# amdreallyfast/GpuRadixSort

Measured on AMD Instinct MI355X. Metric: Gkeys/s (uint32) at 1/2/4/8 MI355X; achieved HBM GB/s vs peak, higher is better.
Workload: dtype u32; 1 GPU; C4: 2^30 uint32 keys in total (strong scaling: 2^30 / N per GPU), 8-bit digits (MSD schedule at N = 1); N > 1: one RCCL exchange over xGMI (config.exchange); dist=uniform, keys_per_gpu=1073741824, total_keys=1073741824, key_bits=32, radix_bits=8, passes=4, parallelism=range-shard x1

## Files before the change

### gpuradixsort_amd/_lib.py

```python
from __future__ import annotations

import ctypes
import os
from ctypes import POINTER, c_char_p, c_float, c_int, c_size_t, c_uint32, c_uint64, c_ulonglong, c_void_p

PKG_DIR = os.path.dirname(os.path.abspath(__file__))
LIB_PATH = os.path.join(PKG_DIR, "libgrs.so")

GRS_OK, GRS_EINVAL, GRS_ENOMEM, GRS_EHIP, GRS_ECAPACITY, GRS_ENODEV, GRS_ETIMEOUT, GRS_ERCCL = range(8)
GRS_KEY_U32, GRS_KEY_U64 = 0, 1
GRS_RCCL_ID_BYTES = 128
GRS_MAX_N = (1 << 32) - (1 << 16)


class GrsError(RuntimeError):
    def __init__(self, status: int, what: str, detail: str = ""):
        self.status = status
        names = ["GRS_OK", "GRS_EINVAL", "GRS_ENOMEM", "GRS_EHIP", "GRS_ECAPACITY", "GRS_ENODEV",
                 "GRS_ETIMEOUT", "GRS_ERCCL"]
        name = names[status] if 0 <= status < len(names) else str(status)
        super().__init__(f"{what}: {name}" + (f" ({detail})" if detail else ""))


class grs_timing(ctypes.Structure):
    _fields_ = [("passes", c_int), ("total_ms", c_float), ("hist_ms", c_float),
                ("pass_ms", c_float * 16), ("copy_ms", c_float), ("kind", c_int)]


class grs_sharded_timing(ctypes.Structure):
    _fields_ = [("total_ms", c_float), ("before_ms", c_float), ("exchange_ms", c_float),
                ("after_ms", c_float), ("bytes_sent", c_uint64), ("bytes_received", c_uint64),
                ("presorted", c_int)]


class grs_key_extract(ctypes.Structure):
    _fields_ = [("kind", c_int), ("offset", c_uint32), ("transform", c_int),
                ("lo", c_float * 3), ("hi", c_float * 3)]


GRS_EXTRACT_FIELD, GRS_EXTRACT_MORTON3 = 0, 1

OPTIONS = {
    "tile": (1, {"size": -1, "small": 0, "big": 1}),
    "xl": (2, {"size": -1, "never": 0, "always": 1}),
    "pass": (3, {"auto": 0, "v4": 4, "v6": 6, "fused": 8}),
    "records": (4, {"arrays": 0, "scratch": 1, "split": 2}),
    "rank": (5, {"probe": 0, "match": 1}),
    "sharded_path": (6, {"auto": 0, "general": 1}),
    "sharded_send": (7, {"regions": 0, "contig": 1, "shrunk": 2}),
    "exchange": (8, {"auto": 0, "partition": 1, "presorted": 2, "chunked": 3}),
    "merge": (9, {"rounds": 0, "kway": 1}),
    "fault_tile": (10, {"off": -1}),
    "msd": (11, {"size": -1, "never": 0, "always": 1, "exact_p2": 2}),
    "seg_route": (12, {"shape": 0, "passes": 1, "composite": 2}),
    "h2_chunk": (13, {"size": 0}),
    "h2_piece": (14, {"default": 0}),
    "p3": (15, {"per_segment": 0, "persistent": 1, "whole_keys": 2}),
    "x_chunks": (16, {"default": 0}),
    "p3_shape": (17, {"size": 0, "S": 4, "M": 5, "A": 1, "W": 1, "B": 2, "C2": 7, "C": 3, "D": 6}),
}

SIGNATURES = [
    ("grs_version", c_int, []),
    ("grs_status_string", c_char_p, [c_int]),
    ("grs_last_error", c_char_p, []),
    ("grs_create", c_int, [POINTER(c_void_p), c_size_t, c_int, c_int, c_int, c_int]),
    ("grs_destroy", None, [c_void_p]),
    ("grs_scratch_bytes", c_size_t, [c_void_p]),
    ("grs_debug_check_guards", c_int, [c_void_p, POINTER(c_uint64)]),
    ("grs_debug_msd_flags", c_int, [c_void_p, POINTER(c_uint32)]),
    ("grs_debug_p3_kernel", c_char_p, [c_int, c_int, c_size_t, c_int, c_int]),
    ("grs_rank_mode", c_int, [c_void_p]),
    ("grs_lds_order_check", c_int, [c_int, c_int, c_int, POINTER(c_ulonglong)]),
    ("grs_set_option", c_int, [c_void_p, c_int, c_int]),
    ("grs_get_option", c_int, [c_void_p, c_int, POINTER(c_int)]),
    ("grs_pass_kernel", c_char_p, [c_void_p, c_size_t]),
    ("grs_sort", c_int, [c_void_p, c_void_p, c_void_p, c_size_t, c_void_p]),
    ("grs_sort_bits", c_int, [c_void_p, c_void_p, c_void_p, c_size_t, c_int, c_int, c_void_p]),
    ("grs_set_profiling", c_int, [c_void_p, c_int]),
    ("grs_last_timing", c_int, [c_void_p, POINTER(grs_timing)]),
    ("grs_timing_history", c_int, [c_void_p, c_int, POINTER(grs_timing)]),
    ("grs_check_error", c_int, [c_void_p]),
    ("grs_stream_check_error", c_int, [c_void_p, c_void_p]),
    ("grs_partition", c_int, [c_void_p, c_void_p, c_void_p, c_void_p, c_void_p, c_size_t, c_void_p,
                              c_int, c_void_p, c_void_p]),
    ("grs_partition_ranges", c_int, [c_void_p, c_void_p, c_void_p, c_void_p, c_void_p, c_size_t,
                                     c_void_p, c_void_p, c_int, c_void_p, c_void_p]),
    ("grs_partition_regions", c_int, [c_void_p, c_void_p, c_void_p, c_void_p, c_void_p, c_size_t,
                                      c_void_p, c_void_p, c_int, c_size_t, c_void_p, c_void_p]),
    ("grs_sort_sharded", c_int, [c_void_p, c_void_p, c_void_p, c_size_t, c_void_p, c_void_p,
                                 c_size_t, POINTER(c_size_t), c_void_p, c_void_p]),
    ("grs_sharded_last_timing", c_int, [c_void_p, POINTER(grs_sharded_timing)]),
    ("grs_sharded_redo_count", c_int, [c_void_p, POINTER(c_uint64)]),
    ("grs_rccl_unique_id", c_int, [c_void_p]),
    ("grs_rccl_comm_init", c_int, [POINTER(c_void_p), c_void_p, c_int, c_int, c_int]),
    ("grs_rccl_comm_destroy", None, [c_void_p]),
    ("grs_shard_splitters_host", c_int, [c_void_p, c_void_p, c_void_p, c_int, c_int, c_int, c_int,
                                         c_void_p, c_void_p]),
    ("grs_shard_plan_host", c_int, [c_void_p, c_int, c_int, POINTER(c_uint64), POINTER(c_uint64),
                                    POINTER(c_uint64)]),
    ("grs_shard_bounds_host", c_int, [c_void_p, c_size_t, c_int, c_void_p, c_void_p, c_int,
                                      POINTER(c_uint64)]),
    ("grs_shard_chunk_plan_host", c_int, [c_void_p, c_int, c_int, c_int, c_uint64, POINTER(c_uint64),
                                          POINTER(c_uint64), POINTER(c_uint64)]),
    ("grs_shard_samples_per_rank", c_int, [c_int]),
    ("grs_shard_sample", c_int, [c_void_p, c_size_t, c_int, c_int, c_void_p, c_void_p, c_void_p]),
    ("grs_shard_encode_words_max", c_size_t, [c_size_t, c_int]),
    ("grs_shard_encode", c_int, [c_void_p, c_void_p, c_size_t, c_void_p, c_void_p, c_int, c_int,
                                 c_void_p, c_size_t, c_void_p, c_void_p]),
    ("grs_shard_decode_merge", c_int, [c_void_p, c_void_p, c_int, POINTER(c_uint64),
                                       POINTER(c_uint32), c_void_p, c_size_t, c_void_p]),
    ("grs_copy_u32", c_int, [c_void_p, c_void_p, c_size_t, c_void_p]),
    ("grs_iota_u32", c_int, [c_void_p, c_size_t, c_uint32, c_void_p]),
    ("grs_gather_records", c_int, [c_void_p, c_void_p, c_void_p, c_size_t, c_size_t, c_void_p]),
    ("grs_fill_splitmix", c_int, [c_void_p, c_size_t, c_int, c_uint64, c_uint64, c_void_p]),
    ("grs_fill_permutation", c_int, [c_void_p, c_size_t, c_int, c_uint64, c_uint64, c_uint64, c_void_p]),
    ("grs_count_inversions", c_int, [c_void_p, c_size_t, c_int, POINTER(c_uint64), c_void_p]),
    ("grs_sort_host", c_int, [c_void_p, c_void_p, c_void_p, c_void_p, c_void_p, c_size_t,
                              c_void_p]),
    ("grs_key_transform", c_int, [c_void_p, c_size_t, c_int, c_int, c_int, c_void_p]),
    ("grs_sort_records", c_int, [c_void_p, c_void_p, c_size_t, c_size_t, POINTER(grs_key_extract),
                                 c_void_p]),
    ("grs_records_key_buffers", c_int, [c_void_p, c_size_t, c_size_t, POINTER(c_void_p),
                                        POINTER(c_void_p)]),
    ("grs_sort_records_by_keys", c_int, [c_void_p, c_void_p, c_size_t, c_size_t, c_void_p, c_void_p,
                                         c_void_p]),
    ("grs_scan_scratch_bytes", c_size_t, [c_size_t]),
    ("grs_exclusive_scan_u32", c_int, [c_void_p, c_void_p, c_size_t, c_void_p, c_void_p, c_size_t,
                                       c_void_p]),
    ("grs_scan_check_error", c_int, [c_void_p, c_void_p]),
    ("grs_sort_segmented", c_int, [c_void_p, c_void_p, c_void_p, c_size_t, c_void_p, c_int,
                                   c_void_p]),
]

_LIB = None


def lib() -> ctypes.CDLL:
    global _LIB
    if _LIB is not None:
        return _LIB
    import torch

    if not os.path.exists(LIB_PATH):
        raise ImportError(
            f"{LIB_PATH} is missing: build it with `make -C gpuradixsort_amd/csrc` or "
            "`python -c 'import __graft_entry__ as g; g.build()'` (no CPU fallback exists)")
    L = ctypes.CDLL(LIB_PATH)
    for name, res, args in SIGNATURES:
        f = getattr(L, name)
        f.restype = res
        f.argtypes = args
    _LIB = L
    return L


def check(status: int, what: str) -> None:
    if status != GRS_OK:
        detail = lib().grs_last_error()
        raise GrsError(status, what, detail.decode() if detail else "")
```

### gpuradixsort_amd/csrc/grs_capi.hip

```cpp
#include <hip/hip_runtime.h>

#include <algorithm>
#include <cmath>
#include <cstdio>
#include <cstdlib>
#include <cstring>
#include <mutex>
#include <set>
#include <string>
#include <type_traits>
#include <vector>

#include "../../include/grs.h"
#include "grs_config.h"
#include "grs_kernels.hpp"
#include "grs_pass.hpp"
#include "grs_msd.hpp"
#include "grs_shard.hpp"
#include "grs_codec.hpp"

#include <rccl/rccl.h>

namespace {

// ... 76 lines not shown
        case 1: d = lane % 3; break;
        case 2: d = (lane * 37u + round * 11u) & 255u; break;
        case 3: d = (lane & 1) ? 5u : 37u; break;
        case 4: d = (grs::splitmix64(lane * 131u + round) >> 7) & 15u; break;
        default: d = 255u - lane / 4; break;
      }
      const uint32_t before = cnt[d];
      __syncthreads();
      uint32_t below = 0;
      for (uint32_t l2 = 0; l2 < 64; ++l2) {
        const uint32_t d2 = __shfl(d, l2, 64);
        below += (l2 < lane && d2 == d) ? 1u : 0u;
      }
      const uint32_t old = atomicAdd(&cnt[d], 1u);
      bad += old != before + below;
      __syncthreads();
    }
  }
  if (bad) atomicAdd(out, bad);
}

template <int RB, int PACK>
__global__ __launch_bounds__(512) void grs_lds_order_scale(uint32_t pattern, uint32_t items,
                                                           unsigned long long* bad) {
  constexpr int RADIX = 1 << RB;
  __shared__ uint32_t cnt[8][RADIX / PACK];
  __shared__ uint32_t ref[8][RADIX];
  const uint32_t w = threadIdx.x >> 6, lane = threadIdx.x & 63;
  for (uint32_t i = threadIdx.x; i < 8u * RADIX / PACK; i += 512) (&cnt[0][0])[i] = 0;
  for (uint32_t i = threadIdx.x; i < 8u * RADIX; i += 512) (&ref[0][0])[i] = 0;
  __syncthreads();
  unsigned long long nbad = 0;
  const uint64_t seed = (static_cast<uint64_t>(blockIdx.x) * 8 + w) * 0x9E3779B97F4A7C15ull + pattern;
  for (uint32_t j = 0; j < items; ++j) {
    const uint64_t r = grs::splitmix64(seed ^ (static_cast<uint64_t>(j) * 64 + lane));
    uint32_t d;
    switch (pattern) {
      case 0: d = static_cast<uint32_t>(r) & (RADIX - 1); break;
      case 1: d = 7u & (RADIX - 1); break;
      case 2: d = (static_cast<uint32_t>(r) & 3u) * (RADIX / 4); break;
      case 3: d = lane < 32 ? 3u : static_cast<uint32_t>(r) & (RADIX - 1); break;
      default: d = ((static_cast<uint32_t>(r) & 15u) * 32u) & (RADIX - 1); break;
    }
    const uint64_t m = grs::match_digit<RB>(d);
    const uint32_t below = grs::mbcnt64(m);
    const uint32_t expect = ref[w][d] + below;
    uint32_t got;
    if constexpr (PACK == 2) {
      const uint32_t sh = (d & 1u) << 4;
      got = (atomicAdd(&cnt[w][d >> 1], 1u << sh) >> sh) & 0xFFFFu;
    } else {
      got = atomicAdd(&cnt[w][d], 1u);
    }
    nbad += got != expect;
    if (below == 0) ref[w][d] += static_cast<uint32_t>(__popcll(m));
  }
  if (nbad) atomicAdd(bad, nbad);
}

int device_rank_mode(int device) {
  static std::mutex mu;
  static int mode[64];
  static bool known[64];
  std::lock_guard<std::mutex> lock(mu);
  if (device >= 0 && device < 64 && known[device]) return mode[device];
  int m = 1;
  uint32_t* d = nullptr;
  if (hipMalloc(&d, 4) == hipSuccess) {
    uint32_t h = 1;
    if (hipMemset(d, 0, 4) == hipSuccess) {
      hipLaunchKernelGGL(grs_probe_lds_order, dim3(1), dim3(64), 0, 0, d);
      if (hipGetLastError() == hipSuccess && hipMemcpy(&h, d, 4, hipMemcpyDeviceToHost) == hipSuccess)
        m = h == 0 ? 0 : 1;
    }
    (void)hipFree(d);
  }
  (void)hipGetLastError();
  if (device >= 0 && device < 64) {
    mode[device] = m;
    known[device] = true;
  }
  return m;
}

}

struct grs_sorter {
  int device = 0;
  grs_key_type key_type = GRS_KEY_U32;
  int pairs = 0;
  int radix_bits = 8;
  int rank_mode = 0;
  int cus = 0;
  size_t capacity = 0;
  void* alt_keys = nullptr;
  uint32_t* alt_vals = nullptr;
  bool alt_joint = false;
  int rec_mode = 2;
  uint32_t* status = nullptr;
  size_t status_words = 0;
  size_t status_stride = 0;
  uint32_t* ctrl = nullptr;
  uint32_t* ctrl2 = nullptr;
  int cb_i = 0;
  bool cb_dirty = false;
  uint32_t* h_err = nullptr;
  size_t scratch_bytes = 0;
  static constexpr int EV_PER_CALL = GRS_MAX_PASSES + 3;
  int ring = 0;
  long long calls = 0;
  hipEvent_t* ev = nullptr;
  struct CallInfo { int ev_used; int passes; bool copy; int kind = 0; };
  CallInfo* info = nullptr;
  void* seg_buf = nullptr;
  size_t seg_bytes = 0;
  grs_sorter* seg64 = nullptr;
  void* host_stage = nullptr;
  size_t host_stage_bytes = 0;
  void* shard_buf = nullptr;
  size_t shard_bytes = 0;
  void* rec_buf = nullptr;
  size_t rec_bytes = 0;
  void* rec_kbuf = nullptr;
  uint32_t* shard_host = nullptr;
  void* xbuf = nullptr;
  size_t xbuf_bytes = 0;
  void* xrbuf = nullptr;
  size_t xrbuf_bytes = 0;
  void* codec_buf = nullptr;
  size_t codec_bytes = 0;
  int sharded_exchange = 0;
  int x_chunks = 0;
  hipStream_t xstream = nullptr;
  hipEvent_t xcev[17] = {};
  hipEvent_t xhev = nullptr;
  uint32_t* xchunk_host = nullptr;
  int merge_mode = 0;
  hipEvent_t xev[4] = {};
  bool xev_recorded = false;
  uint64_t x_sent = 0, x_recv = 0;
  int x_presorted = 0;
  uint64_t x_region_redo = 0;
  int tile_mode = -1;
  int pass_mode = 0;
  bool sharded_general = false;
  int sharded_send = 0;
  int xl_mode = 0;
  int probe_rank_mode = 0;
  int fault_tile = -1;
  uint32_t h2_chunk = 0;
  uint32_t h2_piece = 0;
  int p3_shape = 0;
  int p3_mode = 0;
  int seg_route = 0;
  int msd_mode = -1;
  void* msd_buf = nullptr;
  void* alt2_keys = nullptr;
  uint32_t* alt2_vals = nullptr;
  size_t msd_bytes = 0;
  size_t alt_words = 0;
  struct ScratchBuf {
    void** owner;
    size_t bytes;
    std::vector<size_t> bands;
  };
  std::vector<ScratchBuf> bufs;
  int last_msd_cb = -1;
  uint32_t* last_msd_spill2 = nullptr;
  size_t alt_inner_band = 0;
  bool alt_band_dirty = false;
};

namespace {

constexpr size_t kGuardBytes = 16384;
constexpr uint32_t kGuardWord = 0x6A7DBA5Eu;

hipError_t fill_band(void* at) {
  static const std::vector<uint32_t> pattern(kGuardBytes / 4, kGuardWord);
  return hipMemcpy(at, pattern.data(), kGuardBytes, hipMemcpyHostToDevice);
}

void sbuf_free(grs_sorter* s, void** p) {
  for (size_t i = 0; i < s->bufs.size(); ++i)
    if (s->bufs[i].owner == p) {
      s->scratch_bytes -= s->bufs[i].bytes;
      s->bufs.erase(s->bufs.begin() + static_cast<long>(i));
      break;
    }
  if (*p) (void)hipFree(*p);
  *p = nullptr;
}

grs_status sbuf_alloc(grs_sorter* s, void** p, size_t bytes, const char* what,
                      std::vector<size_t> inner = {}) {
  sbuf_free(s, p);
  void* d = nullptr;
  if (hipMalloc(&d, bytes + kGuardBytes) != hipSuccess) {
    (void)hipGetLastError();
    return set_err(GRS_ENOMEM, std::string(what) + ": hipMalloc of " + std::to_string(bytes + kGuardBytes) +
                                   " bytes failed");
  }
  inner.push_back(bytes);
  for (size_t o : inner)
    if (fill_band(static_cast<char*>(d) + o) != hipSuccess) {
      (void)hipFree(d);
      return set_err(GRS_EHIP, std::string(what) + ": guard band fill failed");
    }
  *p = d;
  s->bufs.push_back({p, bytes + kGuardBytes, inner});
  s->scratch_bytes += bytes + kGuardBytes;
  return GRS_OK;
}

grs_status grow_buf(grs_sorter* s, void** p, size_t* have, size_t need, const char* what) {
  if (*have >= need && *p) return GRS_OK;
  *have = 0;
  const grs_status r = sbuf_alloc(s, p, need, what);
  if (r == GRS_OK) *have = need;
  return r;
}

}

extern "C" {

int grs_version(void) { return GRS_VERSION; }

const char* grs_status_string(grs_status s) {
  switch (s) {
    case GRS_OK: return "GRS_OK";
    case GRS_EINVAL: return "GRS_EINVAL";
    case GRS_ENOMEM: return "GRS_ENOMEM";
    case GRS_EHIP: return "GRS_EHIP";
    case GRS_ECAPACITY: return "GRS_ECAPACITY";
    case GRS_ENODEV: return "GRS_ENODEV";
    case GRS_ETIMEOUT: return "GRS_ETIMEOUT";
    case GRS_ERCCL: return "GRS_ERCCL";
  }
  return "GRS_UNKNOWN";
}

const char* grs_last_error(void) { return g_last_error.c_str(); }

void grs_destroy(grs_sorter* s) {
  if (!s) return;
  int prev = 0;
  (void)hipGetDevice(&prev);
  (void)hipSetDevice(s->device);
  for (grs_sorter::ScratchBuf& b : s->bufs)
    if (*b.owner) {
      (void)hipFree(*b.owner);
      *b.owner = nullptr;
    }
  s->bufs.clear();
  if (s->h_err) (void)hipHostFree(s->h_err);
  if (s->seg64) grs_destroy(s->seg64);
  if (s->shard_host) (void)hipHostFree(s->shard_host);
  for (int i = 0; s->ev && i < s->ring * grs_sorter::EV_PER_CALL; ++i)
    if (s->ev[i]) (void)hipEventDestroy(s->ev[i]);
  for (hipEvent_t e : s->xev)
    if (e) (void)hipEventDestroy(e);
  for (hipEvent_t e : s->xcev)
    if (e) (void)hipEventDestroy(e);
  if (s->xhev) (void)hipEventDestroy(s->xhev);
  if (s->xstream) (void)hipStreamDestroy(s->xstream);
  if (s->xchunk_host) (void)hipHostFree(s->xchunk_host);
  delete[] s->ev;
  delete[] s->info;
  (void)hipSetDevice(prev);
  delete s;
}

}

namespace {

bool use_big_tiles(const grs_sorter* s, size_t n, size_t big_tile) {
  if (s->tile_mode >= 0) return s->tile_mode == 1;
  return (n + big_tile - 1) / big_tile >= static_cast<size_t>(std::max(1, s->cus));
}

bool use_persistent(const grs_sorter* s, size_t tiles, int rb) {
  if (s->pass_mode != 0) return s->pass_mode == 6 || s->pass_mode == 8;
  return rb == 4 || tiles <= 4u * static_cast<size_t>(std::max(1, s->cus));
}

bool use_xl(const grs_sorter* s, size_t n, size_t xl_tile) {
  if (s->rank_mode != 0 || s->xl_mode == 2) return false;
  return s->xl_mode == 1 ||
         (n + xl_tile - 1) / xl_tile >= 32u * static_cast<size_t>(std::max(1, s->cus));
}

template <int B, int I_, bool C> struct MsdLocal {
  static constexpr int BLOCK = B, I = I_;
  static constexpr bool C16 = C;
  static constexpr uint32_t SMAX = B * I_;
};
using MsdLocalS = MsdLocal<256, 8, false>;
using MsdLocalM = MsdLocal<256, 12, false>;
using MsdLocalA = MsdLocal<256, 20, false>;
using MsdLocalB = MsdLocal<512, 20, false>;
using MsdLocalW = MsdLocal<1024, 5, false>;
using MsdLocalC2 = MsdLocal<768, 23, true>;
using MsdLocalC = MsdLocal<768, 24, true>;
using MsdLocalD = MsdLocal<1024, 36, true>;
constexpr uint32_t kMsdSmaxMin = MsdLocalS::SMAX;
template <typename K, bool PAIRS, typename F>
bool with_msd_shape(int code, F&& f) {
  constexpr bool kKeys32 = sizeof(K) == 4 && !PAIRS;
  switch (code) {
    case 4: f(MsdLocalS{}); return true;
    case 5: f(MsdLocalM{}); return true;
    case 1:
      if constexpr (sizeof(K) == 8) f(MsdLocalW{});
      else f(MsdLocalA{});
      return true;
    case 2: f(MsdLocalB{}); return true;
    case 7:
      if constexpr (kKeys32) f(MsdLocalC2{});
      return kKeys32;
    case 3:
      if constexpr (kKeys32) f(MsdLocalC{});
      return kKeys32;
    case 6:
      if constexpr (kKeys32) f(MsdLocalD{});
      return kKeys32;
    default: return false;
  }
}
constexpr uint32_t kMsdTileMin = 17408;
static_assert(BigTile<uint32_t, true>::TILE == kMsdTileMin && BigTile<uint64_t, false>::TILE == kMsdTileMin &&
              BigTile<uint32_t, false>::TILE > kMsdTileMin, "MSD table sizing");

struct MsdLayout {
  size_t h2, h2x, h2s, big, spill2, mid, clear, dstart, reg, room, len2, in2, out2, tab, hdr2, rec2, hdr2r, rec2r,
      hdrf, recf, bin, bstart, blen, brow, rows, spill, words;
  size_t r2, rf, bl, mr;
  std::vector<size_t> bands;
  static MsdLayout of(size_t cap, size_t nd) {
    MsdLayout L{};
    cap = std::max<size_t>(cap, 1);
    L.r2 = cap / kMsdTileMin + 257;
    L.bl = std::min<size_t>(65536, cap / (kMsdSmaxMin + 1) + 2);
    L.mr = cap / (kMsdTileMin + 1) + 2;
    L.rf = cap / kMsdTileMin + L.bl + 1;
    size_t o = 0;
    auto take = [&](size_t w) {
      if (o != 0) {
        L.bands.push_back(o * 4);
        o += kGuardBytes / 4;
      }
      const size_t at = o;
      o += (w + 63) & ~static_cast<size_t>(63);
      return at;
    };
    L.h2 = take(3 * 65536 + 64 + 2 + 3 * 65536);
    L.h2x = L.h2 + 65536;
    L.h2s = L.h2 + 2 * 65536;
    L.big = L.h2 + 3 * 65536;
    L.spill2 = L.big + 8;
    L.mid = L.big + 64;
    L.clear = 3 * 65536 + 64 + 2;
    L.dstart = take(65536);
    L.reg = take(65536);
    L.room = take(256);
    L.len2 = take(65536);
    L.in2 = take(65536);
    L.out2 = take(65536);
    L.tab = take(4 * 257);
    L.hdr2 = take(4);
    L.rec2 = take(L.r2 * 8);
    L.hdr2r = take(4);
    L.rec2r = take(L.r2 * 8);
    L.hdrf = take(4);
    L.recf = take(L.rf * 8);
    L.bin = take(L.bl);
    L.bstart = take(L.bl);
    L.blen = take(L.bl);
    L.brow = take(L.bl);
    L.rows = take(L.mr * nd * 256);
    L.spill = take(6 * (L.bl + 1));
    L.words = o;
    return L;
  }
  static size_t status_words(size_t cap) {
    cap = std::max<size_t>(cap, 1);
    const size_t t2 = cap / kMsdTileMin + 257;
    const size_t w2 = (t2 + 2 * (t2 / GRS_LB_GROUP + 257)) * 256;
    const size_t tf = 2 * (cap / kMsdTileMin) + 2;
    const size_t gf = tf / GRS_LB_GROUP + cap / (kMsdTileMin + 1) + 2;
    return std::max(w2, (tf + 2 * gf) * 256);
  }
};

size_t msd_alt_words(size_t cap) { return std::max<size_t>(cap, 1) + cap / 8 + 256 * 4096 + 1024; }
size_t msd_alt2_words(size_t cap) { return std::max<size_t>(cap, 1) + cap / 10 * 3 + 65536 * 64 + 1024; }

bool msd_type(const grs_sorter* s) {
  return s->radix_bits == 8 && !(s->key_type == GRS_KEY_U64 && s->pairs);
}
constexpr size_t kMsdMinN = size_t(3) << 24;
size_t msd_digits(const grs_sorter* s) { return s->key_type == GRS_KEY_U64 ? 6 : 2; }

template <typename K, bool PAIRS>
size_t max_status_words(const grs_sorter* s, size_t cap, size_t radix) {
  const size_t big = std::min(BigTile<K, PAIRS>::TILE, BigTile4<K, PAIRS>::TILE);
  const size_t small = SmallTile<K, PAIRS>::TILE;
  size_t w0 = 0;
  const size_t big_max = std::max(BigTile<K, PAIRS>::TILE, BigTile4<K, PAIRS>::TILE);
  const size_t small_cap = s->tile_mode == 0 ? cap : std::min(cap, big_max * std::max(1, s->cus));
  const size_t match = MatchTile<K, PAIRS>::TILE;
  w0 = status_words_for((cap + match - 1) / match, radix);
  size_t w = std::max(std::max(w0, status_words_for((cap + big - 1) / big, radix)),
                      status_words_for((small_cap + small - 1) / small, radix));
  const size_t part = PartTile<K, PAIRS>::TILE;
  return std::max(w, status_words_for((cap + part - 1) / part, 16));
}

size_t needed_status_words(const grs_sorter* s) {
  const size_t cap = std::max<size_t>(s->capacity, 1);
  const size_t radix = std::max<size_t>(size_t(1) << s->radix_bits, 16);
  size_t w;
  if (s->key_type == GRS_KEY_U32)
    w = s->pairs ? max_status_words<uint32_t, true>(s, cap, radix)
                 : max_status_words<uint32_t, false>(s, cap, radix);
  else
    w = s->pairs ? max_status_words<uint64_t, true>(s, cap, radix)
                 : max_status_words<uint64_t, false>(s, cap, radix);
  return msd_type(s) ? std::max(w, MsdLayout::status_words(cap)) : w;
}

grs_status alloc_status(grs_sorter* s, size_t words) {
  const size_t stride = words + kGuardBytes / 4;
  const grs_status r = sbuf_alloc(s, reinterpret_cast<void**>(&s->status), (stride + words) * 4,
                                  "look-back status buffers", {words * 4});
  if (r != GRS_OK) return r;
  s->status_words = words;
  s->status_stride = stride;
  return GRS_OK;
}

grs_status alloc_alt(grs_sorter* s, size_t words) {
  const size_t kb = s->key_type == GRS_KEY_U64 ? 8 : 4;
  grs_status r;
  if (s->pairs && s->key_type == GRS_KEY_U32) {
    r = sbuf_alloc(s, &s->alt_keys, (2 * words) * 4 + kGuardBytes, "second buffer", {words * 4});
    if (r != GRS_OK) return r;
    s->alt_vals = reinterpret_cast<uint32_t*>(static_cast<char*>(s->alt_keys) + words * 4 + kGuardBytes);
    s->alt_joint = true;
    s->alt_inner_band = words * 4;
    s->alt_band_dirty = false;
  } else {
    r = sbuf_alloc(s, &s->alt_keys, words * kb, "second buffer");
    if (r == GRS_OK && s->pairs) r = sbuf_alloc(s, reinterpret_cast<void**>(&s->alt_vals), words * 4, "second buffer");
    if (r != GRS_OK) return r;
  }
  s->alt_words = words;
  return GRS_OK;
}

grs_status msd_scratch(grs_sorter* s, bool on) {
  const size_t cap = std::max<size_t>(s->capacity, 1);
  const size_t kb = s->key_type == GRS_KEY_U64 ? 8 : 4;
  const size_t altw = on ? msd_alt_words(cap) : cap;
  const bool change = (s->msd_buf != nullptr) != on || s->alt_words != altw;
  if (!change) return GRS_OK;
  (void)hipDeviceSynchronize();
  if (!on) {
    sbuf_free(s, &s->msd_buf);
    sbuf_free(s, &s->alt2_keys);
    s->alt2_vals = nullptr;
    s->msd_bytes = 0;
    return s->alt_words == cap && s->alt_keys ? GRS_OK : alloc_alt(s, cap);
  }
  grs_status r = alloc_alt(s, altw);
  if (r != GRS_OK) return r;
  const MsdLayout L = MsdLayout::of(cap, msd_digits(s));
  s->msd_bytes = L.words * 4;
  r = sbuf_alloc(s, &s->msd_buf, s->msd_bytes, "MSD tables", L.bands);
  if (r != GRS_OK) return r;
  const size_t w2 = msd_alt2_words(cap);
  r = sbuf_alloc(s, &s->alt2_keys, w2 * kb + kGuardBytes + (s->pairs ? w2 * 4 : 0), "MSD region buffer",
                 {w2 * kb});
  if (r != GRS_OK) return r;
  if (s->pairs) s->alt2_vals = reinterpret_cast<uint32_t*>(static_cast<char*>(s->alt2_keys) + w2 * kb + kGuardBytes);
  return GRS_OK;
}

}

extern "C" {

grs_status grs_set_option(grs_sorter* s, grs_option opt, int value) {
  if (!s) return set_err(GRS_EINVAL, "grs_set_option: NULL sorter");
  auto bad = [&]() { return set_err(GRS_EINVAL, "grs_set_option: value out of range for option " +
                                                    std::to_string(static_cast<int>(opt))); };
  switch (opt) {
    case GRS_OPT_TILE:
      if (value < -1 || value > 1) return bad();
      s->tile_mode = value;
      break;
    case GRS_OPT_XL:
      if (value < -1 || value > 1) return bad();
      s->xl_mode = value == -1 ? 0 : value == 1 ? 1 : 2;
      break;
    case GRS_OPT_PASS:
      if (value != 0 && value != 4 && value != 6 && value != 8) return bad();
      s->pass_mode = value;
      break;
    case GRS_OPT_RECORDS:
      if (value < 0 || value > 2) return bad();
      s->rec_mode = value;
      break;
    case GRS_OPT_RANK:
      if (value < 0 || value > 1) return bad();
      s->rank_mode = value == 1 ? 1 : s->probe_rank_mode;
      break;
    case GRS_OPT_SHARDED_PATH:
      if (value < 0 || value > 1) return bad();
      s->sharded_general = value == 1;
      break;
    case GRS_OPT_SHARDED_SEND:
      if (value < 0 || value > 2) return bad();
      s->sharded_send = value;
      break;
    case GRS_OPT_EXCHANGE:
      if (value < 0 || value > 3) return bad();
      s->sharded_exchange = value;
      break;
    case GRS_OPT_X_CHUNKS:
      if (value < 0 || value > 16) return bad();
      s->x_chunks = value;
      break;
    case GRS_OPT_FAULT_TILE: {
      if (value < -1) return bad();
      const uint32_t w[2] = {static_cast<uint32_t>(value + 1), value >= 0 ? (1u << 12) : 0u};
      int prev = 0;
      GRS_HIP(hipGetDevice(&prev));
      GRS_HIP(hipSetDevice(s->device));
      const hipError_t e = hipMemcpy(s->ctrl + GRS_CTRL_ERROR + 1, w, sizeof(w), hipMemcpyHostToDevice);
      (void)hipSetDevice(prev);
      if (e != hipSuccess) return set_err(GRS_EHIP, "grs_set_option: hipMemcpy failed");
      s->fault_tile = value;
      break;
    }
    case GRS_OPT_MERGE:
      if (value < 0 || value > 1) return bad();
      s->merge_mode = value;
      break;
    case GRS_OPT_MSD:
      if (value < -1 || value > 2) return bad();
      s->msd_mode = value;
      break;
    case GRS_OPT_SEG_ROUTE:
      if (value < 0 || value > 2) return bad();
      s->seg_route = value;
      break;
    case GRS_OPT_H2_CHUNK:
      if (value != 0 && (value < 4096 || value > (1 << 20) || (value & (value - 1)) != 0)) return bad();
      s->h2_chunk = static_cast<uint32_t>(value);
      break;
    case GRS_OPT_H2_PIECE:
      if (value != 0 && (value < 64 || value > 4096 || (value & (value - 1)) != 0)) return bad();
      s->h2_piece = static_cast<uint32_t>(value);
      break;
    case GRS_OPT_P3:
      if (value < 0 || value > 2) return bad();
      s->p3_mode = value;
      break;
    case GRS_OPT_P3_SHAPE: {
      const auto none = [](auto) {};
      const bool ok = value == 0 || (s->key_type == GRS_KEY_U32
                                         ? (s->pairs ? with_msd_shape<uint32_t, true>(value, none)
                                                     : with_msd_shape<uint32_t, false>(value, none))
                                         : !s->pairs && with_msd_shape<uint64_t, false>(value, none));
      if (!ok) return bad();
      s->p3_shape = value;
      break;
    }
    default:
      return set_err(GRS_EINVAL, "grs_set_option: unknown option");
  }
  const size_t words = needed_status_words(s);
  if (words > s->status_words) {
    int prev = 0;
    GRS_HIP(hipGetDevice(&prev));
    GRS_HIP(hipSetDevice(s->device));
    (void)hipDeviceSynchronize();
    const grs_status r = alloc_status(s, words);
    (void)hipSetDevice(prev);
    if (r != GRS_OK) return r;
  }
  if (opt == GRS_OPT_MSD) {
    int prev = 0;
    GRS_HIP(hipGetDevice(&prev));
    GRS_HIP(hipSetDevice(s->device));
    const grs_status r = msd_scratch(s, value != 0 && msd_type(s) && (value != -1 || s->capacity >= kMsdMinN));
    (void)hipSetDevice(prev);
    if (r != GRS_OK) return r;
  }
  return GRS_OK;
}

grs_status grs_get_option(const grs_sorter* s, grs_option opt, int* value) {
  if (!s || !value) return set_err(GRS_EINVAL, "grs_get_option: NULL argument");
  switch (opt) {
    case GRS_OPT_TILE: *value = s->tile_mode; break;
    case GRS_OPT_XL: *value = s->xl_mode == 0 ? -1 : s->xl_mode == 1 ? 1 : 0; break;
    case GRS_OPT_PASS: *value = s->pass_mode; break;
    case GRS_OPT_RECORDS: *value = s->rec_mode; break;
    case GRS_OPT_RANK: *value = s->rank_mode; break;
    case GRS_OPT_SHARDED_PATH: *value = s->sharded_general ? 1 : 0; break;
    case GRS_OPT_SHARDED_SEND: *value = s->sharded_send; break;
    case GRS_OPT_EXCHANGE: *value = s->sharded_exchange; break;
    case GRS_OPT_X_CHUNKS: *value = s->x_chunks; break;
    case GRS_OPT_MERGE: *value = s->merge_mode; break;
    case GRS_OPT_FAULT_TILE: *value = s->fault_tile; break;
    case GRS_OPT_MSD: *value = s->msd_mode; break;
    case GRS_OPT_SEG_ROUTE: *value = s->seg_route; break;
    case GRS_OPT_H2_CHUNK: *value = static_cast<int>(s->h2_chunk); break;
    case GRS_OPT_H2_PIECE: *value = static_cast<int>(s->h2_piece); break;
    case GRS_OPT_P3: *value = s->p3_mode; break;
    case GRS_OPT_P3_SHAPE: *value = s->p3_shape; break;
    default: return set_err(GRS_EINVAL, "grs_get_option: unknown option");
  }
  return GRS_OK;
}

grs_status grs_create(grs_sorter** out, size_t capacity, grs_key_type key_type,
                      int with_u32_payload, int radix_bits, int device) {
  if (!out) return set_err(GRS_EINVAL, "grs_create: out is NULL");
  *out = nullptr;
  if (key_type != GRS_KEY_U32 && key_type != GRS_KEY_U64)
    return set_err(GRS_EINVAL, "grs_create: bad key type");
  if (radix_bits == 0) radix_bits = 8;
  if (radix_bits != 4 && radix_bits != 8)
    return set_err(GRS_EINVAL, "grs_create: radix_bits must be 4, 8 or 0");
  if (capacity > GRS_MAX_N)
    return set_err(GRS_ECAPACITY, "grs_create: capacity exceeds GRS_MAX_N (2^32 - 2^16) items per device call");
  int ndev = 0;
  if (hipGetDeviceCount(&ndev) != hipSuccess || ndev <= 0)
    return set_err(GRS_ENODEV, "grs_create: no HIP device");
  if (device < 0 || device >= ndev) return set_err(GRS_ENODEV, "grs_create: bad device ordinal");

  int prev = 0;
  GRS_HIP(hipGetDevice(&prev));
  GRS_HIP(hipSetDevice(device));
  grs_sorter* s = new grs_sorter();
  s->device = device;
  s->key_type = key_type;
  s->pairs = with_u32_payload ? 1 : 0;
  s->radix_bits = radix_bits;
  s->capacity = capacity;
  s->rank_mode = s->probe_rank_mode = device_rank_mode(device);
  (void)hipDeviceGetAttribute(&s->cus, hipDeviceAttributeMultiprocessorCount, device);
  const size_t kb = key_type == GRS_KEY_U64 ? 8 : 4;
  const size_t cap = std::max<size_t>(capacity, 1);
  (void)kb;
  grs_status st = alloc_status(s, needed_status_words(s));
  if (st == GRS_OK) st = sbuf_alloc(s, reinterpret_cast<void**>(&s->ctrl), GRS_CTRL_WORDS * 4, "grs_create: control block");
  if (st == GRS_OK) st = sbuf_alloc(s, reinterpret_cast<void**>(&s->ctrl2), GRS_CTRL_ERROR * 4, "grs_create: control block");
  if (st == GRS_OK && (hipMemset(s->ctrl, 0, GRS_CTRL_WORDS * 4) != hipSuccess ||
                       hipMemset(s->ctrl2, 0, GRS_CTRL_ERROR * 4) != hipSuccess))
    st = set_err(GRS_EHIP, "grs_create: hipMemset failed");
  if (st == GRS_OK) {
    if (msd_type(s) && cap >= kMsdMinN && msd_scratch(s, true) != GRS_OK) (void)msd_scratch(s, false);
    if (!s->alt_keys) st = alloc_alt(s, cap);
  }
  if (st == GRS_OK && hipHostMalloc(reinterpret_cast<void**>(&s->h_err), 4, hipHostMallocDefault) != hipSuccess) {
    (void)hipGetLastError();
    st = set_err(GRS_ENOMEM, "grs_create: hipHostMalloc failed");
  }
  (void)hipSetDevice(prev);
  if (st != GRS_OK) {
    grs_destroy(s);
    return st;
  }
  *out = s;
  return GRS_OK;
}

size_t grs_scratch_bytes(const grs_sorter* s) { return s ? s->scratch_bytes : 0; }

grs_status grs_debug_check_guards(grs_sorter* s, uint64_t* bad_words) {
  if (!s || !bad_words) return set_err(GRS_EINVAL, "grs_debug_check_guards: NULL argument");
  *bad_words = 0;
  int prev = 0;
  GRS_HIP(hipGetDevice(&prev));
  GRS_HIP(hipSetDevice(s->device));
  grs_status r = GRS_OK;
  if (hipDeviceSynchronize() != hipSuccess) r = set_err(GRS_EHIP, "grs_debug_check_guards: synchronise");
  std::vector<uint32_t> h(kGuardBytes / 4);
  uint64_t bad = 0;
  for (const grs_sorter::ScratchBuf& b : s->bufs) {
    if (r != GRS_OK || !*b.owner) continue;
    for (size_t o : b.bands) {
      char* at = static_cast<char*>(*b.owner) + o;
      const bool records = b.owner == &s->alt_keys && o == s->alt_inner_band && s->alt_band_dirty;
      if (hipMemcpy(h.data(), at, kGuardBytes, hipMemcpyDeviceToHost) != hipSuccess) {
        r = set_err(GRS_EHIP, "grs_debug_check_guards: read-back");
        break;
      }
      uint64_t c = 0;
      for (uint32_t w : h) c += w != kGuardWord;
      if (!records) bad += c;
      if (c != 0 && fill_band(at) != hipSuccess) r = set_err(GRS_EHIP, "grs_debug_check_guards: restore");
    }
  }
  if (r == GRS_OK) s->alt_band_dirty = false;
  *bad_words = bad;
  (void)hipSetDevice(prev);
  return r;
}

grs_status grs_debug_msd_flags(grs_sorter* s, uint32_t* flags) {
  if (!s || !flags) return set_err(GRS_EINVAL, "grs_debug_msd_flags: NULL argument");
  if (s->last_msd_cb < 0) return set_err(GRS_EINVAL, "grs_debug_msd_flags: the last sort did not run the MSD schedule");
  int prev = 0;
  GRS_HIP(hipGetDevice(&prev));
  GRS_HIP(hipSetDevice(s->device));
  grs_status r = GRS_OK;
  const uint32_t* hist = s->last_msd_cb == 0 ? s->ctrl : s->ctrl2;
  uint32_t w[3] = {};
  if (hipDeviceSynchronize() != hipSuccess ||
      hipMemcpy(&w[0], hist + 512 + 256, 4, hipMemcpyDeviceToHost) != hipSuccess ||
      hipMemcpy(&w[1], s->last_msd_spill2, 4, hipMemcpyDeviceToHost) != hipSuccess ||
      hipMemcpy(&w[2], hist + GRS_MSD_SPAN + 4, 4, hipMemcpyDeviceToHost) != hipSuccess)
    r = set_err(GRS_EHIP, "grs_debug_msd_flags: read-back");
  flags[0] = w[0] != 0u;
  flags[1] = w[1] != 0u;
  flags[2] = w[2];
  (void)hipSetDevice(prev);
  return r;
}

int grs_rank_mode(const grs_sorter* s) { return s ? s->rank_mode : -1; }

grs_status grs_set_profiling(grs_sorter* s, int ring) {
  if (!s) return set_err(GRS_EINVAL, "grs_set_profiling: NULL sorter");
  if (ring < 0 || ring > 4096) return set_err(GRS_EINVAL, "grs_set_profiling: ring out of range");
  int prev = 0;
  GRS_HIP(hipGetDevice(&prev));
  GRS_HIP(hipSetDevice(s->device));
  for (int i = 0; s->ev && i < s->ring * grs_sorter::EV_PER_CALL; ++i)
    if (s->ev[i]) (void)hipEventDestroy(s->ev[i]);
  delete[] s->ev;
  delete[] s->info;
  s->ev = nullptr;
  s->info = nullptr;
  s->ring = 0;
  s->calls = 0;
  grs_status st = GRS_OK;
  if (ring > 0) {
    s->ev = new hipEvent_t[ring * grs_sorter::EV_PER_CALL]();
    s->info = new grs_sorter::CallInfo[ring]();
    s->ring = ring;
    for (int i = 0; i < ring * grs_sorter::EV_PER_CALL && st == GRS_OK; ++i)
      if (hipEventCreate(&s->ev[i]) != hipSuccess)
        st = set_err(GRS_EHIP, "grs_set_profiling: hipEventCreate failed");
    for (hipEvent_t& e : s->xev)
      if (st == GRS_OK && !e && hipEventCreate(&e) != hipSuccess)
        st = set_err(GRS_EHIP, "grs_set_profiling: hipEventCreate failed");
  }
  s->xev_recorded = false;
  (void)hipSetDevice(prev);
  return st;
}

}

namespace {

template <typename K, bool PAIRS, int RB, typename Tile, uint32_t OPT, bool PERSIST = false,
          typename DigitF>
grs_status launch_pass(grs_sorter* s, const K* src, K* dst, const uint32_t* vsrc, uint32_t* vdst,
                       uint32_t n, const DigitF& dig, const DigitF* dig_dev, const uint32_t* hist,
                       uint32_t* ticket, uint32_t* st_cur, uint32_t* st_nxt, hipStream_t stream,
                       uint32_t expect_tile = 0, const uint32_t* plan = nullptr) {
  const uint32_t tiles = (n + Tile::TILE - 1) / Tile::TILE;
  if (status_words_for(tiles, 1u << RB) > s->status_words)
    return set_err(GRS_ECAPACITY, "status buffer too small (pass: " + std::to_string(tiles) + " tiles, have " +
                                      std::to_string(s->status_words) + " words)");
  if (expect_tile != 0 && expect_tile != static_cast<uint32_t>(Tile::TILE))
    return set_err(GRS_EINVAL, "internal: pass tile differs from the zeroed status layout");
  if constexpr (PERSIST) {
    const uint32_t grid = std::min<uint32_t>(tiles, static_cast<uint32_t>(s->cus * Tile::MINW));
    hipLaunchKernelGGL((grs::grs_onesweep_v6<K, PAIRS, RB, Tile::BLOCK, Tile::ITEMS, Tile::MINW,
                                             OPT, DigitF>),
                       dim3(grid), dim3(Tile::BLOCK), 0, stream, src, dst, vsrc, vdst, n, dig, hist,
                       ticket, st_cur, st_nxt, s->ctrl + GRS_CTRL_ERROR, dig_dev, plan);
  } else {
    hipLaunchKernelGGL((grs::grs_onesweep_v4<K, PAIRS, RB, Tile::BLOCK, Tile::ITEMS, Tile::MINW,
                                             OPT, DigitF>),
                       dim3(tiles), dim3(Tile::BLOCK), 0, stream, src, dst, vsrc, vdst, n, dig, hist,
                       ticket, st_cur, st_nxt, s->ctrl + GRS_CTRL_ERROR, dig_dev, plan);
  }
  GRS_HIP(hipGetLastError());
  return GRS_OK;
}

template <typename K, bool PAIRS, int RB, typename Tile, uint32_t OPT, bool PERSIST>
grs_status launch_rec(int kind, grs_sorter* s, const K* src, K* dst, const uint32_t* vsrc,
                      uint32_t* vdst, uint32_t n, const grs::RadixDigit<K>& dig,
                      const uint32_t* hist, uint32_t* ticket, uint32_t* st_cur, uint32_t* st_nxt,
                      hipStream_t stream, uint32_t expect_tile, const uint32_t* plan = nullptr) {
  using Dig = grs::RadixDigit<K>;
  constexpr bool R = sizeof(K) == 4 && PAIRS && RB == 8;
  constexpr uint32_t W = R ? 8192u : 0u, Rd = R ? 4096u : 0u, RS = R ? 16384u : 0u, WS = R ? 32768u : 0u;
  switch (R ? kind : 0) {
    case 1: return launch_pass<K, PAIRS, RB, Tile, OPT | W, PERSIST>(s, src, dst, vsrc, vdst, n, dig, (const Dig*)nullptr, hist, ticket, st_cur, st_nxt, stream, expect_tile);
    case 2: return launch_pass<K, PAIRS, RB, Tile, OPT | Rd, PERSIST>(s, src, dst, vsrc, vdst, n, dig, (const Dig*)nullptr, hist, ticket, st_cur, st_nxt, stream, expect_tile);
    case 3: return launch_pass<K, PAIRS, RB, Tile, OPT | Rd | RS | W, PERSIST>(s, src, dst, vsrc, vdst, n, dig, (const Dig*)nullptr, hist, ticket, st_cur, st_nxt, stream, expect_tile);
    case 4: return launch_pass<K, PAIRS, RB, Tile, OPT | Rd | W | WS, PERSIST>(s, src, dst, vsrc, vdst, n, dig, (const Dig*)nullptr, hist, ticket, st_cur, st_nxt, stream, expect_tile);
    default: return launch_pass<K, PAIRS, RB, Tile, OPT, PERSIST>(s, src, dst, vsrc, vdst, n, dig, (const Dig*)nullptr, hist, ticket, st_cur, st_nxt, stream, expect_tile, plan);
  }
}

template <typename K, bool PAIRS, int RB>
grs_status run_sort(grs_sorter* s, K* keys, uint32_t* vals, uint32_t n, int begin_bit,
                    int end_bit, hipStream_t stream, const K* src_in = nullptr,
                    const uint32_t* vsrc_in = nullptr) {
  using Big = std::conditional_t<RB == 8, BigTile<K, PAIRS>, BigTile4<K, PAIRS>>;
  using Small = SmallTile<K, PAIRS>;
  constexpr uint32_t kBig = RB == 8 ? BigTile<K, PAIRS>::OPT : kBig4Opt;
  constexpr int RADIX = 1 << RB;
  const bool big = use_big_tiles(s, n, Big::TILE);
  const int passes = (end_bit - begin_bit + RB - 1) / RB;
  uint32_t tile = big ? Big::TILE : Small::TILE;
  if (s->rank_mode != 0 && big) tile = MatchTile<K, PAIRS>::TILE;
  using XL = XLTile<K, PAIRS>;
  constexpr bool kXlType = RB == 8 && !(sizeof(K) == 8 && PAIRS);
  const bool xl = kXlType && big && use_xl(s, n, XL::TILE);
  if (xl) tile = XL::TILE;
  const uint32_t tiles = (n + tile - 1) / tile;
  const bool persist = !xl && !Big::TWO_ROUNDS && use_persistent(s, tiles, RB);
  const size_t words = status_words_for(tiles, RADIX);
  if (words > s->status_words)
    return set_err(GRS_ECAPACITY, "status buffer too small (LSD: n " + std::to_string(n) + ", " +
                                      std::to_string(words) + " words, have " + std::to_string(s->status_words) + ")");
  uint32_t* st0 = s->status;
  uint32_t* st1 = s->status + s->status_stride;
  uint32_t* const cb[2] = {s->ctrl, s->ctrl2};
  uint32_t* hist = cb[s->cb_i];
  uint32_t* tickets = hist + GRS_CTRL_TICKETS;
  uint32_t* hist_next = cb[s->cb_i ^ 1];
  int ev = 0;
  hipEvent_t* evs = s->ring ? s->ev + (s->calls % s->ring) * grs_sorter::EV_PER_CALL : nullptr;
  auto mark = [&]() -> grs_status {
    if (evs) GRS_HIP(hipEventRecord(evs[ev++], stream));
    return GRS_OK;
  };

  grs_status r;
  if ((r = mark()) != GRS_OK) return r;
  if (s->cb_dirty && s->cb_i == 0) GRS_HIP(hipMemsetAsync(hist, 0, GRS_CTRL_ERROR * 4, stream));
  s->cb_dirty = false;
  {
    const int slots = grs::Hist2Layout<K>::PER_CU * s->cus;
    const int need = static_cast<int>(n >> grs::kHist2GridShift<K>) + 1;
    int grid = n <= (1u << 25) ? s->cus : slots;
    if (grid < need) grid = (need + slots - 1) / slots * slots;
    const bool full = begin_bit == 0 && end_bit == static_cast<int>(8 * sizeof(K));
    auto kern = full ? grs::grs_upfront_hist2<K, RB, true> : grs::grs_upfront_hist2<K, RB, false>;
    hipLaunchKernelGGL(kern, dim3(grid), dim3(grs::Hist2Layout<K>::BLOCK), 0, stream,
                       src_in ? src_in : keys, n, begin_bit, end_bit, passes, hist, st0,
                       static_cast<uint32_t>(words), hist_next, (uint32_t*)nullptr, 0u);
    GRS_HIP(hipGetLastError());
  }
  s->cb_i ^= 1;
  if ((r = mark()) != GRS_OK) return r;

  K* src = keys;
  K* dst = static_cast<K*>(s->alt_keys);
  uint32_t* vsrc = vals;
  uint32_t* vdst = s->alt_vals;
  if (src_in) {
    src = const_cast<K*>(src_in);
    vsrc = const_cast<uint32_t*>(vsrc_in);
    if ((passes & 1) != 0) {
      dst = keys;
      vdst = vals;
    }
  }
  constexpr bool kRecType = sizeof(K) == 4 && PAIRS && RB == 8;
// ... 109 lines not shown
  if (need <= MsdLocalM::SMAX) return 5;
  if (need <= MsdLocalA::SMAX) return 1;
  if (need <= MsdLocalB::SMAX) return 2;
  if (elem == 4 && need <= MsdLocalC2::SMAX) return 7;
  if (elem == 4 && need <= MsdLocalC::SMAX) return 3;
  if (elem == 4 && need <= MsdLocalD::SMAX) return 6;
  return 0;
}

struct MsdP3Kernel {
  enum Family { kLocal, kLocalPf, kLocal16 } family;
  int block, items;
  uint32_t smax;
  uint32_t mid_max;
  bool list;
};
template <typename K, bool PAIRS, typename P3C>
MsdP3Kernel msd_p3_kernel(size_t n, int p3_mode) {
  using P3L = std::conditional_t<sizeof(K) == 4 && !PAIRS, MsdLocalC, MsdLocalB>;
  const uint32_t mid_max = P3L::SMAX > P3C::SMAX ? P3L::SMAX : P3C::SMAX;
  const bool list = P3L::SMAX > P3C::SMAX;
  const MsdP3Kernel whole{MsdP3Kernel::kLocal, P3C::BLOCK, P3C::I, P3C::SMAX, mid_max, list};
  if constexpr (sizeof(K) == 4) {
    if (p3_mode == 1) return {MsdP3Kernel::kLocalPf, P3C::BLOCK, P3C::I, P3C::SMAX, mid_max, list};
    if constexpr (!PAIRS && P3C::SMAX == MsdLocalC2::SMAX) {
      if (p3_mode == 0) return {MsdP3Kernel::kLocal16, 512, 34, 512u * 34u, mid_max, list};
    }
    if constexpr (!PAIRS && P3C::SMAX == MsdLocalD::SMAX) {
      if (p3_mode == 0 && msd_segment_need(n) <= 1024 * 34)
        return {MsdP3Kernel::kLocal16, 1024, 34, 1024u * 34u, 1024u * 34u, list};
    }
  }
  return whole;
}

const char* msd_p3_kernel_name(const MsdP3Kernel& k) {
  static const char* const family[] = {"grs_msd_local", "grs_msd_local_pf", "grs_msd_local16"};
  static std::mutex mu;
  static std::set<std::string> names;
  const std::string name =
      std::string(family[k.family]) + "<" + std::to_string(k.block) + "," + std::to_string(k.items) + ">";
  std::lock_guard<std::mutex> lock(mu);
  return names.insert(name).first->c_str();
}

int msd_shape_code(int pinned, size_t n, size_t elem) { return pinned != 0 ? pinned : msd_local_shape(n, elem); }

bool use_msd(const grs_sorter* s, size_t n, int begin_bit, int end_bit) {
  if (!msd_type(s) || s->msd_mode == 0 || s->msd_buf == nullptr || s->rank_mode != 0) return false;
  const int kbits = s->key_type == GRS_KEY_U64 ? 64 : 32;
  const size_t elem = kbits / 8 + (s->pairs ? 4 : 0);
  if (begin_bit != 0 || end_bit != kbits || msd_local_shape(n, elem) == 0) return false;
  return s->msd_mode >= 1 || n >= kMsdMinN;
}

template <typename K, bool PAIRS, typename P3C>
grs_status run_msd(grs_sorter* s, K* keys, uint32_t* vals, uint32_t n, hipStream_t stream,
                   const K* src_in, const uint32_t* vsrc_in) {
  using Big = BigTile<K, PAIRS>;
  using XL = XLTile<K, PAIRS>;
  using Small = SmallTile<K, PAIRS>;
  using FT = BigTile<K, PAIRS>;
  using Dig = grs::RadixDigit<K>;
  constexpr int KB = 8 * static_cast<int>(sizeof(K));
  constexpr int ND = (KB - 16) / 8;
  static_assert(!Big::TWO_ROUNDS, "u64 pairs take the LSD sort");
  constexpr uint32_t G = GRS_LB_GROUP;
  const bool big = use_big_tiles(s, n, Big::TILE);
  const bool xl = big && use_xl(s, n, XL::TILE);
  const uint32_t tile1 = xl ? XL::TILE : big ? Big::TILE : Small::TILE;
  const size_t words1 = status_words_for((n + tile1 - 1) / tile1, 256);
  const uint32_t tile2 = xl ? XL::TILE : Big::TILE;
  const size_t t2 = n / tile2 + 257;
  const size_t words2 = (t2 + 2 * (t2 / G + 257)) * 256;
  if (words1 > s->status_words || words2 > s->status_words)
    return set_err(GRS_ECAPACITY, "status buffer too small (MSD: n " + std::to_string(n) + ", P1 " +
                                      std::to_string(words1) + " / P2 " + std::to_string(words2) + " words, have " +
                                      std::to_string(s->status_words) + ")");
  const MsdLayout L = MsdLayout::of(s->capacity, ND);
  if (t2 > L.r2) return set_err(GRS_ECAPACITY, "internal: MSD plan capacity");
  uint32_t* const mb = static_cast<uint32_t*>(s->msd_buf);
  uint32_t* const h2 = mb + L.h2;
  uint32_t* const bigc = mb + L.big;
  uint32_t* const dstart = mb + L.dstart;
  uint32_t* const hdr2 = mb + L.hdr2;
  auto* const rec2 = reinterpret_cast<grs::SegTile*>(mb + L.rec2);
  uint32_t* const hdrf = mb + L.hdrf;
  auto* const recf = reinterpret_cast<grs::SegTile*>(mb + L.recf);
  uint32_t* const rows = mb + L.rows;
  uint32_t* const st[2] = {s->status, s->status + s->status_stride};
  uint32_t* const err = s->ctrl + GRS_CTRL_ERROR;
  uint32_t* const cb[2] = {s->ctrl, s->ctrl2};
  uint32_t* const hist = cb[s->cb_i];
  uint32_t* const tickets = hist + GRS_CTRL_TICKETS;
  uint32_t* const hist_next = cb[s->cb_i ^ 1];
  const K* src = src_in ? src_in : keys;
  const uint32_t* vsrc = src_in ? vsrc_in : vals;
  K* const alt = static_cast<K*>(s->alt_keys);
  uint32_t* const valt = PAIRS ? s->alt_vals : nullptr;
  int ev = 0;
  hipEvent_t* evs = s->ring ? s->ev + (s->calls % s->ring) * grs_sorter::EV_PER_CALL : nullptr;
  auto mark = [&]() -> grs_status {
    if (evs) GRS_HIP(hipEventRecord(evs[ev++], stream));
    return GRS_OK;
  };
  uint32_t* const samp = hist;
  uint32_t* const exact = hist + 256;
  uint32_t* const totals = hist + 512;
  uint32_t* const span = hist + GRS_MSD_SPAN;
  const uint32_t* const top = span + 4;
  const uint64_t sampled = std::min<uint64_t>(n, uint64_t(GRS_MSD_SAMPLE_CHUNKS) * GRS_WAVE);
  const unsigned long long mult =
      static_cast<unsigned long long>((static_cast<uint64_t>(n) * 9 * (uint64_t(1) << 20) + 8 * sampled - 1) /
                                      (8 * sampled));
  const uint32_t pad = n > sampled ? 4096u : 0u;
  const uint64_t region_len = static_cast<uint64_t>(n) + n / 8 + 256u * pad + 256u;
  if (region_len > msd_alt_words(s->capacity)) return set_err(GRS_ECAPACITY, "internal: MSD regions");
  grs_status r;
#ifdef GRS_DIAG
  auto diag_set = [&](uint64_t out_lim, uint64_t in_lim) -> grs_status {
    const uint32_t lim[4] = {static_cast<uint32_t>(std::min<uint64_t>(out_lim, 0xFFFFFFFFu)),
                             static_cast<uint32_t>(std::min<uint64_t>(in_lim, 0xFFFFFFFFu)),
                             static_cast<uint32_t>(std::min<size_t>(s->status_words, 0xFFFFFFFFu)), 0u};
    GRS_HIP(hipMemcpyToSymbolAsync(HIP_SYMBOL(grs::diag_lim), lim, sizeof(lim), 0, hipMemcpyHostToDevice, stream));
    return GRS_OK;
  };
  auto diag_check = [&](const char* what) -> grs_status {
    GRS_HIP(hipStreamSynchronize(stream));
    uint32_t hit[24];
    GRS_HIP(hipMemcpyFromSymbol(hit, HIP_SYMBOL(grs::diag_hit), sizeof(hit)));
    if (hit[8] != 0u)
      fprintf(stderr, "diag %-12s first run past the bound: tile %u digit %u start %u gstart %u prefix %u seg_start %u "
              "seg_len %u publish %u gh %u base %u valid %u lstart %u\n", what, hit[9], hit[10], hit[11], hit[12],
              hit[13], hit[14], hit[15], hit[16], hit[17], hit[18], hit[19], hit[20]);
    uint32_t host_err[4] = {};
    GRS_HIP(hipMemcpy(host_err, err, sizeof(host_err), hipMemcpyDeviceToHost));
    fprintf(stderr, "diag %-12s bad stores %u (max %u)  bad loads %u (max %u)  status %u (tile row %u)  error word %u\n",
            what, hit[0], hit[1], hit[2], hit[3], hit[4], hit[5], host_err[0]);
    const uint32_t zero[24] = {};
    GRS_HIP(hipMemcpyToSymbol(HIP_SYMBOL(grs::diag_hit), zero, sizeof(zero)));
    const char* stop = getenv("GRS_DIAG_STOP");
    if (stop != nullptr && strcmp(stop, what) == 0) return set_err(GRS_EINVAL, std::string("diag stop after ") + what);
    return GRS_OK;
  };
#define GRS_DIAG_SET(o, i) if ((r = diag_set(o, i)) != GRS_OK) return r
#define GRS_DIAG_CHECK(w) if ((r = diag_check(w)) != GRS_OK) return r
#else
#define GRS_DIAG_SET(o, i)
#define GRS_DIAG_CHECK(w)
#endif
  if ((r = mark()) != GRS_OK) return r;
  s->last_msd_cb = s->cb_i;
  s->last_msd_spill2 = mb + L.spill2;
  if (s->cb_dirty && s->cb_i == 0) GRS_HIP(hipMemsetAsync(hist, 0, GRS_CTRL_ERROR * 4, stream));
  s->cb_dirty = false;
  if (s->alt_band_dirty) {
    GRS_HIP(hipMemsetD32Async(reinterpret_cast<hipDeviceptr_t>(static_cast<char*>(s->alt_keys) + s->alt_inner_band),
                              static_cast<int>(kGuardWord), kGuardBytes / 4, stream));
    s->alt_band_dirty = false;
  }
  hipLaunchKernelGGL((grs::grs_msd_sample<K>), dim3(std::max(1, s->cus)), dim3(256), 0, stream, src, n, samp, st[0],
                     static_cast<uint32_t>(words1), hist_next, h2, static_cast<uint32_t>(L.clear), span);
  GRS_HIP(hipGetLastError());
  s->cb_i ^= 1;
  if ((r = mark()) != GRS_OK) return r;
  const Dig d1{0, 255u};
  GRS_DIAG_SET(region_len, n);
  {
    const uint32_t tiles = (n + tile1 - 1) / tile1;
    auto go = [&](auto tshape, auto optc) {
      using T = decltype(tshape);
      constexpr uint32_t opt = decltype(optc)::value;
      hipLaunchKernelGGL((grs::grs_onesweep_region<K, PAIRS, 8, T::BLOCK, T::ITEMS, T::MINW, opt>),
                         dim3(tiles), dim3(T::BLOCK), 0, stream, src, alt, vsrc, valt, n, d1, samp, mult,
                         pad, static_cast<uint32_t>(region_len), tickets, st[0], st[1], err, totals, span);
    };
    if (xl) go(XL{}, std::integral_constant<uint32_t, XL::OPT>{});
    else if (big) go(Big{}, std::integral_constant<uint32_t, Big::OPT>{});
    else go(Small{}, std::integral_constant<uint32_t, kSmallOpt>{});
    GRS_HIP(hipGetLastError());
  }
  if ((r = mark()) != GRS_OK) return r;
  hipLaunchKernelGGL((grs::grs_msd_span<K, FT::TILE>), dim3(1), dim3(256), 0, stream, n, span, totals, recf, hdrf);
  GRS_HIP(hipGetLastError());
  hipLaunchKernelGGL((grs::grs_seg_hist<K, 1, true>), dim3(2 * s->cus), dim3(256), 0, stream, src, recf, hdrf,
                     0, exact, st[0], 256u, top);
  GRS_HIP(hipGetLastError());
  hipLaunchKernelGGL((grs::grs_onesweep_seg<K, PAIRS, 8, FT::BLOCK, FT::ITEMS, FT::MINW, FT::OPT, true>),
                     dim3(s->cus), dim3(FT::BLOCK), 0, stream, src, alt, vsrc, valt, d1, recf, hdrf,
                     exact, 256u, tickets + 15 * GRS_XCDS, st[0], st[1], err, nullptr, nullptr, nullptr,
                     nullptr, top);
  GRS_HIP(hipGetLastError());
  GRS_DIAG_CHECK("P1");
  if ((r = mark()) != GRS_OK) return r;
  uint32_t* const tab = mb + L.tab;
  uint32_t* const spill2 = mb + L.spill2;
  uint32_t* const h2x = mb + L.h2x;
  uint32_t* const reg = mb + L.reg;
  uint32_t* const hdr2r = mb + L.hdr2r;
  auto* const rec2r = reinterpret_cast<grs::SegTile*>(mb + L.rec2r);
  K* const rk = static_cast<K*>(s->alt2_keys);
  uint32_t* const rv = PAIRS ? s->alt2_vals : nullptr;
  uint32_t chunk = GRS_H2_CHUNK;
  while (chunk > 32768u && static_cast<uint64_t>(n) / chunk < 16u * static_cast<uint64_t>(std::max(1, s->cus)))
    chunk >>= 1;
  uint32_t shift = 0;
  while (shift < 6 && (static_cast<uint64_t>(n) >> (shift + 1)) >= 65536ull * 512) ++shift;
  chunk = std::min<uint32_t>(chunk << shift, 1u << 20);
  if (s->h2_chunk != 0) chunk = s->h2_chunk;
  const uint32_t piece_log = s->h2_piece != 0 ? static_cast<uint32_t>(__builtin_ctz(s->h2_piece)) : GRS_H2_PIECE_LOG;
  const uint64_t cap2 = s->msd_mode == 2 ? 0 : static_cast<uint64_t>(msd_alt2_words(s->capacity));
  {
    if (xl)
      hipLaunchKernelGGL((grs::grs_msd_plan2<XL::TILE>), dim3(1), dim3(1024), 0, stream, samp, mult, pad,
                         totals, exact, chunk, tab, rec2, hdr2, shift == 0 ? 1u : 0u);
    else
      hipLaunchKernelGGL((grs::grs_msd_plan2<Big::TILE>), dim3(1), dim3(1024), 0, stream, samp, mult, pad,
                         totals, exact, chunk, tab, rec2, hdr2, shift == 0 ? 1u : 0u);
    GRS_HIP(hipGetLastError());
    hipLaunchKernelGGL((grs::grs_msd_hist2<K>), dim3(n / chunk + 257), dim3(1024), 0, stream, alt,
                       shift ? mb + L.h2s : h2x, st[1], static_cast<uint32_t>(words2), tab, chunk, shift,
                       (const uint32_t*)nullptr, top, piece_log);
    GRS_HIP(hipGetLastError());
    if (shift) {
      uint32_t* const room = mb + L.room;
      hipLaunchKernelGGL(grs::grs_msd_regions, dim3(256), dim3(256), 0, stream, tab, mb + L.h2s, reg, room);
      GRS_HIP(hipGetLastError());
      if (xl)
        hipLaunchKernelGGL((grs::grs_msd_plan3<XL::TILE>), dim3(1), dim3(1024), 0, stream, tab, room, cap2,
                           rec2r, hdr2r, spill2);
      else
        hipLaunchKernelGGL((grs::grs_msd_plan3<Big::TILE>), dim3(1), dim3(1024), 0, stream, tab, room, cap2,
                           rec2r, hdr2r, spill2);
      GRS_HIP(hipGetLastError());
    }
  }
  if ((r = mark()) != GRS_OK) return r;
  {
    const Dig d2{-8, 255u};
    const dim3 grid(static_cast<uint32_t>(t2));
    constexpr uint32_t RG = 131072;
    auto go = [&](auto tshape) -> grs_status {
      using T = decltype(tshape);
      if (shift) {
        GRS_DIAG_CHECK("plans");
        GRS_DIAG_SET(cap2, region_len);
        hipLaunchKernelGGL((grs::grs_onesweep_seg<K, PAIRS, 8, T::BLOCK, T::ITEMS, T::MINW, T::OPT | RG, false>),
                           grid, dim3(T::BLOCK), 0, stream, alt, rk, valt, rv, d2, rec2r, hdr2r, reg, 256u,
                           tickets + GRS_XCDS, st[1], st[0], err, dstart, h2, spill2, (const uint32_t*)nullptr, top);
        GRS_HIP(hipGetLastError());
        GRS_DIAG_CHECK("P2region");
        GRS_DIAG_SET(n, region_len);
        hipLaunchKernelGGL((grs::grs_msd_hist2<K, T::TILE>), dim3(n / chunk + 257), dim3(1024), 0, stream, alt,
                           h2x, st[0], static_cast<uint32_t>(words2), tab, chunk, 0u, spill2, top, 8u, rec2, hdr2);
        GRS_HIP(hipGetLastError());
        hipLaunchKernelGGL((grs::grs_onesweep_seg<K, PAIRS, 8, T::BLOCK, T::ITEMS, T::MINW, T::OPT, true>),
                           dim3(s->cus), dim3(T::BLOCK), 0, stream, alt, keys, valt, vals, d2, rec2, hdr2, h2x,
                           256u, tickets + 14 * GRS_XCDS, st[0], st[1], err, (uint32_t*)nullptr,
                           (uint32_t*)nullptr, (uint32_t*)nullptr, spill2, top);
        GRS_HIP(hipGetLastError());
      } else {
        GRS_HIP(hipMemsetD32Async(reinterpret_cast<hipDeviceptr_t>(spill2), 1, 1, stream));
        hipLaunchKernelGGL((grs::grs_onesweep_seg<K, PAIRS, 8, T::BLOCK, T::ITEMS, T::MINW, T::OPT, false>), grid,
                           dim3(T::BLOCK), 0, stream, alt, keys, valt, vals, d2, rec2, hdr2, h2x, 256u,
                           tickets + GRS_XCDS, st[1], st[0], err, (uint32_t*)nullptr, (uint32_t*)nullptr,
                           (uint32_t*)nullptr, (const uint32_t*)nullptr, top);
        GRS_HIP(hipGetLastError());
      }
      return GRS_OK;
    };
    if ((r = xl ? go(XL{}) : go(Big{})) != GRS_OK) return r;
    GRS_DIAG_CHECK("P2exact");
    hipLaunchKernelGGL(grs::grs_msd_starts, dim3(256), dim3(256), 0, stream, spill2, tab, h2, h2x, dstart,
                       mb + L.len2, mb + L.in2, mb + L.out2);
    GRS_HIP(hipGetLastError());
  }
  if ((r = mark()) != GRS_OK) return r;
  using P3L = std::conditional_t<sizeof(K) == 4 && !PAIRS, MsdLocalC, MsdLocalB>;
  const MsdP3Kernel pk = msd_p3_kernel<K, PAIRS, P3C>(n, s->p3_mode);
  const uint32_t mid_max = pk.mid_max;
  bool launched = false;
  if constexpr (sizeof(K) == 4) {
    if (pk.family == MsdP3Kernel::kLocalPf) {
      using LS = grs::LocalSort<K, PAIRS, P3C::BLOCK, P3C::I, P3C::C16>;
      constexpr int lds_per_cu = 160 * 1024 / static_cast<int>(sizeof(typename LS::Smem) + 16);
      constexpr int per_cu = std::min(std::min(lds_per_cu, 2048 / P3C::BLOCK), P3C::BLOCK == 512 && !PAIRS ? 2 : 8);
      constexpr int minw = std::max(1, per_cu * P3C::BLOCK / GRS_WAVE / 4);
      hipLaunchKernelGGL((grs::grs_msd_local_pf<K, PAIRS, P3C::BLOCK, P3C::I, P3C::C16, FT::TILE, minw>),
                         dim3(per_cu * std::max(1, s->cus)), dim3(P3C::BLOCK), 0, stream, keys, vals, rk, rv, spill2,
                         mb + L.len2, mb + L.in2, mb + L.out2, mid_max, mb + L.mid, bigc, mb + L.bin, mb + L.bstart,
                         mb + L.blen, mb + L.brow, rows, top, bigc + 16);
      launched = true;
    } else if (pk.family == MsdP3Kernel::kLocal16 && pk.block == 512) {
      hipLaunchKernelGGL((grs::grs_msd_local16<512, 34, 6, FT::TILE>), dim3(65536), dim3(512), 0, stream,
                         (uint32_t*)keys, vals, (const uint32_t*)rk, rv, spill2, mb + L.len2, mb + L.in2, mb + L.out2,
                         mid_max, mb + L.mid, bigc, mb + L.bin, mb + L.bstart, mb + L.blen, mb + L.brow, rows, top);
      launched = true;
    } else if (pk.family == MsdP3Kernel::kLocal16) {
      hipLaunchKernelGGL((grs::grs_msd_local16<1024, 34, 8, FT::TILE>), dim3(65536), dim3(1024), 0, stream,
                         (uint32_t*)keys, vals, (const uint32_t*)rk, rv, spill2, mb + L.len2, mb + L.in2, mb + L.out2,
                         mid_max, mb + L.mid, bigc, mb + L.bin, mb + L.bstart, mb + L.blen, mb + L.brow, rows, top);
      launched = true;
    }
  }
  if (!launched) {
    if (pk.family != MsdP3Kernel::kLocal) return set_err(GRS_EINVAL, "internal: no P3 kernel of that family for this type");
    hipLaunchKernelGGL((grs::grs_msd_local<K, PAIRS, P3C::BLOCK, P3C::I, P3C::C16, FT::TILE>), dim3(65536),
                       dim3(P3C::BLOCK), 0, stream, keys, vals, rk, rv, spill2, mb + L.len2, mb + L.in2, mb + L.out2,
                       mid_max, mb + L.mid, bigc, mb + L.bin, mb + L.bstart, mb + L.blen, mb + L.brow, rows, top);
  }
  GRS_HIP(hipGetLastError());
  if (pk.list) {
    constexpr int per_cu = P3L::SMAX * (sizeof(K) + (PAIRS ? 4 : 0)) <= 80 * 1024 ? 2 : 1;
    constexpr int minw = per_cu * P3L::BLOCK / GRS_WAVE / 4;
    hipLaunchKernelGGL((grs::grs_msd_local_list<K, PAIRS, P3L::BLOCK, P3L::I, P3L::C16, minw>),
                       dim3(per_cu * s->cus), dim3(P3L::BLOCK), 0, stream, keys, vals, rk, rv, spill2, mb + L.mid,
                       top, (const uint32_t*)bigc, (const uint32_t*)(mb + L.bin), (const uint32_t*)(mb + L.bstart),
                       (const uint32_t*)(mb + L.blen));
    GRS_HIP(hipGetLastError());
  } else {
    hipLaunchKernelGGL((grs::grs_msd_copy_big<K, PAIRS>), dim3(4 * s->cus), dim3(256), 0, stream, rk, rv, keys, vals,
                       spill2, bigc, mb + L.bin, mb + L.bstart, mb + L.blen);
    GRS_HIP(hipGetLastError());
  }
  GRS_DIAG_CHECK("P3");
  GRS_DIAG_SET(n, n);
  if ((r = mark()) != GRS_OK) return r;
  static_assert(ND % 2 == 0, "the fallback ends in keys");
  hipLaunchKernelGGL((grs::grs_seg_plan<FT::TILE, grs::kSegList>), dim3(1), dim3(1024), 0, stream,
                     mb + L.bstart, mb + L.blen, mb + L.brow, 0u, bigc, mb + L.spill, recf, hdrf);
  GRS_HIP(hipGetLastError());
  hipLaunchKernelGGL((grs::grs_seg_hist<K, ND>), dim3(2 * s->cus), dim3(256), 0, stream, keys, recf, hdrf,
                     0, rows, st[0], 256u);
  GRS_HIP(hipGetLastError());
  for (int p = 0; p < ND; ++p) {
    K* const ik = (p & 1) ? alt : keys;
    K* const ok = (p & 1) ? keys : alt;
    uint32_t* const iv = (p & 1) ? valt : vals;
    uint32_t* const ov = (p & 1) ? vals : valt;
    hipLaunchKernelGGL((grs::grs_onesweep_seg<K, PAIRS, 8, FT::BLOCK, FT::ITEMS, FT::MINW, FT::OPT, true>),
                       dim3(s->cus), dim3(FT::BLOCK), 0, stream, ik, ok, iv, ov, Dig{8 * p, 255u}, recf, hdrf,
                       rows + 256 * p, static_cast<uint32_t>(ND * 256), tickets + (2 + p) * GRS_XCDS,
                       st[p & 1], st[(p + 1) & 1], err, nullptr);
    GRS_HIP(hipGetLastError());
  }
  GRS_DIAG_CHECK("fallback");
  GRS_DIAG_SET(0, 0);
  if ((r = mark()) != GRS_OK) return r;
  if (evs) {
    s->info[s->calls % s->ring] = {ev, 6, false, 1};
    ++s->calls;
  }
  return GRS_OK;
}

template <typename K, bool PAIRS>
grs_status run_sort_msd(grs_sorter* s, K* keys, uint32_t* vals, uint32_t n, hipStream_t stream,
                        const K* src_in = nullptr, const uint32_t* vsrc_in = nullptr) {
  grs_status r = GRS_OK;
  const bool known = with_msd_shape<K, PAIRS>(msd_shape_code(s->p3_shape, n, sizeof(K) + (PAIRS ? 4 : 0)), [&](auto shape) {
    r = run_msd<K, PAIRS, decltype(shape)>(s, keys, vals, n, stream, src_in, vsrc_in);
  });
  return known ? r : set_err(GRS_EINVAL, "internal: no MSD shape for this n");
}

template <typename K, bool PAIRS, int N>
grs_status run_partition_n(grs_sorter* s, const K* keys, const uint32_t* vals, K* keys_out,
                           uint32_t* vals_out, uint32_t n, const grs::SplitterIdxDigit<K, N>& dig,
                           const grs::SplitterIdxDigit<K, N>* dig_dev, int count,
                           uint32_t* d_counts, hipStream_t stream, uint32_t region = 0) {
  using T = PartTile<K, PAIRS>;
  using Dig = grs::SplitterIdxDigit<K, N>;
  const uint32_t tiles = (n + T::TILE - 1) / T::TILE;
  const size_t words = status_words_for(tiles, 16);
  if (words > s->status_words) return set_err(GRS_ECAPACITY, "status buffer too small");
  uint32_t* hist = s->ctrl;
  s->cb_dirty = true;
  if (region) {
    hipLaunchKernelGGL(grs::grs_part_init, dim3(std::max<uint32_t>(1u, std::min<uint32_t>(256u, static_cast<uint32_t>(words / 1024 + 1)))),
                       dim3(256), 0, stream, hist, static_cast<uint32_t>(GRS_CTRL_ERROR), region,
                       static_cast<uint32_t>(count + 1), s->status, static_cast<uint32_t>(words));
    GRS_HIP(hipGetLastError());
  } else {
    GRS_HIP(hipMemsetAsync(s->ctrl, 0, GRS_CTRL_ERROR * 4, stream));
    static const int per_cu = [] {
      int b = 0;
      if (hipOccupancyMaxActiveBlocksPerMultiprocessor(&b, grs::grs_digit_hist<K, Dig>, GRS_HIST_BLOCK,
                                                       0) != hipSuccess || b < 1)
        b = 4;
      return b;
    }();
    const int grid = std::max(1, std::min<int>(per_cu * std::max(1, s->cus), (n + 4095) / 4096));
    hipLaunchKernelGGL((grs::grs_digit_hist<K, Dig>), dim3(grid), dim3(GRS_HIST_BLOCK), 0, stream,
                       keys, n, dig, dig_dev, hist, s->status, static_cast<uint32_t>(words));
    GRS_HIP(hipGetLastError());
  }
  grs_status r;
  if (s->rank_mode == 0)
    r = launch_pass<K, PAIRS, 4, T, kSmallOpt>(s, keys, keys_out, vals, vals_out, n, dig, dig_dev, hist,
                                             s->ctrl + GRS_CTRL_TICKETS, s->status,
                                             s->status + s->status_stride, stream);
  else
    r = launch_pass<K, PAIRS, 4, T, kMatchOpt>(s, keys, keys_out, vals, vals_out, n, dig, dig_dev, hist,
                                              s->ctrl + GRS_CTRL_TICKETS, s->status,
                                              s->status + s->status_stride, stream);
  if (r != GRS_OK) return r;
  if (region) {
    const uint32_t groups = (tiles + GRS_LB_GROUP - 1) / GRS_LB_GROUP;
    hipLaunchKernelGGL(grs::grs_lb_totals, dim3(1), dim3(256), 0, stream,
                       s->status + static_cast<size_t>(tiles) * 16, groups, 16u,
                       static_cast<uint32_t>(count + 1), d_counts);
    GRS_HIP(hipGetLastError());
  } else {
    GRS_HIP(hipMemcpyAsync(d_counts, hist, (count + 1) * 4, hipMemcpyDeviceToDevice, stream));
  }
  return GRS_OK;
}

template <typename K, bool PAIRS>
grs_status run_partition(grs_sorter* s, const K* keys, const uint32_t* vals, K* keys_out,
                         uint32_t* vals_out, uint32_t n, const K* splitters, const uint32_t* th,
                         int count, uint32_t* d_counts, hipStream_t stream, uint32_t region = 0) {
  auto go = [&](auto nconst) {
    constexpr int N = decltype(nconst)::value;
    grs::SplitterIdxDigit<K, N> d{};
    d.count = N;
    for (int i = 0; i < GRS_MAX_SPLITTERS; ++i) {
      d.s[i] = i < count ? splitters[i] : static_cast<K>(~static_cast<K>(0));
      d.th[i] = i < count ? (th ? th[i] : 0u) : 0xFFFFFFFFu;
    }
    return run_partition_n<K, PAIRS, N>(s, keys, vals, keys_out, vals_out, n, d, nullptr, count,
                                        d_counts, stream, region);
  };
  if (count <= 1) return go(std::integral_constant<int, 1>{});
  if (count <= 3) return go(std::integral_constant<int, 3>{});
  if (count <= 7) return go(std::integral_constant<int, 7>{});
  return go(std::integral_constant<int, 15>{});
}

}

extern "C" {

static grs_status partition_impl(grs_sorter* s, const void* d_keys, const uint32_t* d_vals,
                                 void* d_keys_out, uint32_t* d_vals_out, size_t n,
                                 const void* splitters, const uint32_t* thresholds,
                                 int n_splitters, uint32_t* d_counts, void* stream,
                                 uint32_t region = 0) {
  if (!s) return set_err(GRS_EINVAL, "grs_partition: NULL sorter");
  if (n_splitters < 0 || n_splitters > GRS_MAX_SPLITTERS || (n_splitters > 0 && !splitters))
    return set_err(GRS_EINVAL, "grs_partition: 0..15 splitters required");
  if (!d_counts) return set_err(GRS_EINVAL, "grs_partition: d_counts is NULL");
  if (n > s->capacity) return set_err(GRS_ECAPACITY, "grs_partition: n exceeds sorter capacity");
  hipStream_t st = static_cast<hipStream_t>(stream);
  if (n == 0) {
    GRS_HIP(hipMemsetAsync(d_counts, 0, (n_splitters + 1) * 4, st));
    return GRS_OK;
  }
  if (!d_keys || !d_keys_out) return set_err(GRS_EINVAL, "grs_partition: NULL keys");
  if (s->pairs && (!d_vals || !d_vals_out))
    return set_err(GRS_EINVAL, "grs_partition: payload sorter needs d_vals / d_vals_out");
  int prev = 0;
  GRS_HIP(hipGetDevice(&prev));
  if (prev != s->device) GRS_HIP(hipSetDevice(s->device));
  const uint32_t n32 = static_cast<uint32_t>(n);
  grs_status r;
  if (s->key_type == GRS_KEY_U32) {
    if (s->pairs)
      r = run_partition<uint32_t, true>(s, (const uint32_t*)d_keys, d_vals, (uint32_t*)d_keys_out,
                                        d_vals_out, n32, (const uint32_t*)splitters, thresholds,
                                        n_splitters, d_counts, st, region);
    else
      r = run_partition<uint32_t, false>(s, (const uint32_t*)d_keys, nullptr, (uint32_t*)d_keys_out,
                                         nullptr, n32, (const uint32_t*)splitters, thresholds,
                                         n_splitters, d_counts, st, region);
// ... 1648 lines not shown
  for (int c = 0; c < nchunks; ++c)
    base += grs::shard_chunk_plan(count_matrices + c * gg, nranks, rank, static_cast<uint64_t>(c) * chunk_len, base,
                                  send_off + static_cast<size_t>(c) * nranks, recv_off + static_cast<size_t>(c) * nranks);
  *n_out = base;
  return GRS_OK;
}

static grs_status records_key_scratch(grs_sorter* s, void** keys, uint32_t** idx) {
  const size_t kb = s->key_type == GRS_KEY_U64 ? 8 : 4;
  const size_t cap = std::max<size_t>(s->capacity, 1);
  const size_t koff = (cap * kb + 255) & ~static_cast<size_t>(255);
  if (!s->rec_kbuf) {
    const grs_status r = sbuf_alloc(s, &s->rec_kbuf, koff + cap * 4, "grs_records_key_buffers: scratch");
    if (r != GRS_OK) return r;
  }
  *keys = s->rec_kbuf;
  *idx = reinterpret_cast<uint32_t*>(static_cast<char*>(s->rec_kbuf) + koff);
  return GRS_OK;
}

static grs_status records_call_scratch(grs_sorter* s, size_t need) {
  return grow_buf(s, &s->rec_buf, &s->rec_bytes, need, "grs_sort_records: scratch");
}

grs_status grs_records_key_buffers(grs_sorter* s, size_t n, size_t record_bytes, void** d_keys,
                                   uint32_t** d_idx) {
  if (!s || !d_keys || !d_idx) return set_err(GRS_EINVAL, "grs_records_key_buffers: NULL argument");
  if (!s->pairs) return set_err(GRS_EINVAL, "grs_records_key_buffers: needs a sorter created with a payload");
  if (n > s->capacity) return set_err(GRS_ECAPACITY, "grs_records_key_buffers: n exceeds capacity");
  if (record_bytes == 0 || record_bytes > 0xFFFFFFFFull)
    return set_err(GRS_EINVAL, "grs_records_key_buffers: bad record size");
  int prev = 0;
  GRS_HIP(hipGetDevice(&prev));
  if (prev != s->device) GRS_HIP(hipSetDevice(s->device));
  const grs_status r = records_key_scratch(s, d_keys, d_idx);
  if (prev != s->device) (void)hipSetDevice(prev);
  return r;
}

grs_status grs_sort_records_by_keys(grs_sorter* s, void* d_records, size_t n, size_t record_bytes,
                                    void* d_keys, uint32_t* d_idx, void* stream) {
  if (!s) return set_err(GRS_EINVAL, "grs_sort_records_by_keys: NULL sorter");
  if (!s->pairs) return set_err(GRS_EINVAL, "grs_sort_records_by_keys: needs a sorter created with a payload");
  if (n > s->capacity) return set_err(GRS_ECAPACITY, "grs_sort_records_by_keys: n exceeds capacity");
  if (record_bytes == 0 || record_bytes > 0xFFFFFFFFull)
    return set_err(GRS_EINVAL, "grs_sort_records_by_keys: bad record size");
  if (n == 0) return GRS_OK;
  if (!d_records || !d_keys || !d_idx) return set_err(GRS_EINVAL, "grs_sort_records_by_keys: NULL buffer");
  int prev = 0;
  GRS_HIP(hipGetDevice(&prev));
  if (prev != s->device) GRS_HIP(hipSetDevice(s->device));
  hipStream_t st = static_cast<hipStream_t>(stream);
  grs_status r = records_call_scratch(s, n * record_bytes);
  void* copy = s->rec_buf;
  if (r == GRS_OK) r = grs_sort(s, d_keys, d_idx, n, stream);
  if (r == GRS_OK) r = gather_records(d_records, copy, d_idx, n, record_bytes, stream,
                                      static_cast<uint32_t>(n - 1));
  if (r == GRS_OK && hipMemcpyAsync(d_records, copy, n * record_bytes, hipMemcpyDeviceToDevice, st) != hipSuccess)
    r = set_err(GRS_EHIP, "grs_sort_records_by_keys: copy back");
  if (prev != s->device) (void)hipSetDevice(prev);
  return r;
}

grs_status grs_sort_records(grs_sorter* s, void* d_records, size_t n, size_t record_bytes,
                            const grs_key_extract* key, void* stream) {
  if (!s || !key) return set_err(GRS_EINVAL, "grs_sort_records: NULL argument");
  if (!s->pairs) return set_err(GRS_EINVAL, "grs_sort_records: needs a sorter created with a payload");
  if (n > s->capacity) return set_err(GRS_ECAPACITY, "grs_sort_records: n exceeds capacity");
  const size_t kb = s->key_type == GRS_KEY_U64 ? 8 : 4;
  if (record_bytes == 0 || record_bytes > 0xFFFFFFFFull ||
      (key->kind != GRS_EXTRACT_FIELD && key->kind != GRS_EXTRACT_MORTON3) ||
      (key->kind == GRS_EXTRACT_FIELD && (key->offset + kb > record_bytes || key->transform < 0 ||
                                          key->transform > 2)) ||
      (key->kind == GRS_EXTRACT_MORTON3 && static_cast<size_t>(key->offset) + 12 > record_bytes))
    return set_err(GRS_EINVAL, "grs_sort_records: key field outside the record or bad kind");
  if (n == 0) return GRS_OK;
  if (!d_records) return set_err(GRS_EINVAL, "grs_sort_records: NULL records");
  int prev = 0;
  GRS_HIP(hipGetDevice(&prev));
  if (prev != s->device) GRS_HIP(hipSetDevice(s->device));
  hipStream_t st = static_cast<hipStream_t>(stream);
  auto al = [](size_t b) { return (b + 255) & ~static_cast<size_t>(255); };
  grs_status r = records_call_scratch(s, al(n * kb) + al(n * 4) + n * record_bytes);
  char* rb = static_cast<char*>(s->rec_buf);
  void* keys = rb;
  uint32_t* idx = reinterpret_cast<uint32_t*>(rb + al(n * kb));
  void* copy = rb + al(n * kb) + al(n * 4);
  const grs::KeyExtract kx{key->kind, key->offset, key->transform,
                           {key->lo[0], key->lo[1], key->lo[2]}, {key->hi[0], key->hi[1], key->hi[2]}};
  if (r == GRS_OK) {
    if (kb == 4)
      hipLaunchKernelGGL(grs::grs_extract_keys<uint32_t>, dim3(grid_for(n, 256)), dim3(256), 0, st,
                         static_cast<const uint8_t*>(d_records), static_cast<uint64_t>(n),
                         static_cast<uint32_t>(record_bytes), kx, static_cast<uint32_t*>(keys), idx);
    else
      hipLaunchKernelGGL(grs::grs_extract_keys<uint64_t>, dim3(grid_for(n, 256)), dim3(256), 0, st,
                         static_cast<const uint8_t*>(d_records), static_cast<uint64_t>(n),
                         static_cast<uint32_t>(record_bytes), kx, static_cast<uint64_t*>(keys), idx);
    if (hipGetLastError() != hipSuccess) r = set_err(GRS_EHIP, "grs_sort_records: launch");
  }
  if (r == GRS_OK) r = grs_sort(s, keys, idx, n, stream);
  if (r == GRS_OK) r = gather_records(d_records, copy, idx, n, record_bytes, stream,
                                      static_cast<uint32_t>(n - 1));
  if (r == GRS_OK && hipMemcpyAsync(d_records, copy, n * record_bytes, hipMemcpyDeviceToDevice, st) != hipSuccess)
    r = set_err(GRS_EHIP, "grs_sort_records: copy back");
  if (prev != s->device) (void)hipSetDevice(prev);
  return r;
}

grs_status grs_lds_order_check(int device, int blocks, int items, unsigned long long* mismatches) {
  if (!mismatches || blocks < 1 || items < 1 || items > 512)
    return set_err(GRS_EINVAL, "grs_lds_order_check: blocks >= 1, 1 <= items <= 512, non-NULL out");
  int prev = 0;
  GRS_HIP(hipGetDevice(&prev));
  if (prev != device) GRS_HIP(hipSetDevice(device));
  unsigned long long* d = nullptr;
  grs_status r = GRS_OK;
  if (hipMalloc(&d, 8) != hipSuccess) {
    (void)hipGetLastError();
    r = set_err(GRS_ENOMEM, "grs_lds_order_check: allocation");
  }
  if (r == GRS_OK && hipMemset(d, 0, 8) != hipSuccess) r = set_err(GRS_EHIP, "grs_lds_order_check: memset");
  for (uint32_t p = 0; r == GRS_OK && p < 5; ++p) {
    const uint32_t it = static_cast<uint32_t>(items);
    hipLaunchKernelGGL((grs_lds_order_scale<4, 1>), dim3(blocks), dim3(512), 0, 0, p, it, d);
    hipLaunchKernelGGL((grs_lds_order_scale<8, 1>), dim3(blocks), dim3(512), 0, 0, p, it, d);
    hipLaunchKernelGGL((grs_lds_order_scale<8, 2>), dim3(blocks), dim3(512), 0, 0, p, it, d);
    hipLaunchKernelGGL((grs_lds_order_scale<11, 1>), dim3(blocks), dim3(512), 0, 0, p, it, d);
    if (hipGetLastError() != hipSuccess) r = set_err(GRS_EHIP, "grs_lds_order_check: launch");
  }
  if (r == GRS_OK && hipMemcpy(mismatches, d, 8, hipMemcpyDeviceToHost) != hipSuccess)
    r = set_err(GRS_EHIP, "grs_lds_order_check: copy");
  if (d) (void)hipFree(d);
  if (prev != device) (void)hipSetDevice(prev);
  return r;
}

const char* grs_debug_p3_kernel(grs_key_type key_type, int pairs, size_t n, int p3_mode, int p3_shape) {
  if (n == 0 || n > GRS_MAX_N || p3_mode < 0 || p3_mode > 2) return nullptr;
  const char* name = nullptr;
  auto pick = [&](auto key, auto with_payload) {
    using K = decltype(key);
    constexpr bool PAIRS = decltype(with_payload)::value;
    (void)with_msd_shape<K, PAIRS>(msd_shape_code(p3_shape, n, sizeof(K) + (PAIRS ? 4 : 0)), [&](auto shape) {
      name = msd_p3_kernel_name(msd_p3_kernel<K, PAIRS, decltype(shape)>(n, p3_mode));
    });
  };
  if (key_type == GRS_KEY_U32 && pairs) pick(uint32_t{}, std::true_type{});
  else if (key_type == GRS_KEY_U32) pick(uint32_t{}, std::false_type{});
  else if (key_type == GRS_KEY_U64 && !pairs) pick(uint64_t{}, std::false_type{});
  return name;
}

const char* grs_pass_kernel(const grs_sorter* s, size_t n) {
  if (!s || n == 0) return "";
  if (use_msd(s, n, 0, s->key_type == GRS_KEY_U64 ? 64 : 32)) return "grs_onesweep_region";
  auto pick = [&](size_t big_tile, bool two_rounds = false) -> const char* {
    if (s->rank_mode != 0 || !use_big_tiles(s, n, big_tile) || two_rounds) return "grs_onesweep_v4";
    if (!use_persistent(s, (n + big_tile - 1) / big_tile, s->radix_bits)) return "grs_onesweep_v4";
    const bool rec = s->key_type == GRS_KEY_U32 && s->pairs && s->radix_bits == 8 && s->rec_mode != 0;
    const bool fused = !rec && s->pass_mode == 8;
    return fused ? "grs_onesweep_fused" : "grs_onesweep_v6";
  };
  const bool u32 = s->key_type == GRS_KEY_U32;
  if (s->radix_bits == 4)
    return u32 ? (s->pairs ? pick(BigTile4<uint32_t, true>::TILE) : pick(BigTile4<uint32_t, false>::TILE))
               : (s->pairs ? pick(BigTile4<uint64_t, true>::TILE) : pick(BigTile4<uint64_t, false>::TILE));
  return u32 ? (s->pairs ? pick(BigTile<uint32_t, true>::TILE, use_xl(s, n, XLTile<uint32_t, true>::TILE))
                         : pick(BigTile<uint32_t, false>::TILE, use_xl(s, n, XLTile<uint32_t, false>::TILE)))
             : (s->pairs ? pick(BigTile<uint64_t, true>::TILE, BigTile<uint64_t, true>::TWO_ROUNDS)
                         : pick(BigTile<uint64_t, false>::TILE, use_xl(s, n, XLTile<uint64_t, false>::TILE)));
}

}
```

### gpuradixsort_amd/csrc/grs_msd.hpp

```cpp
#pragma once

#include "grs_kernels.hpp"
#include "grs_pass.hpp"

namespace grs {

enum SegSource : int { kSegSizes = 0, kSegList = 1, kSegOffsets = 2, kSegMoved = 3, kSegOffsetsAll = 4 };

#define GRS_PLAN_LDS_SEGS 2048
#define GRS_H2_PIECE_LOG 8
#ifndef GRS_P3_LDS_LAYOUT
#define GRS_P3_LDS_LAYOUT 1
#endif
#define GRS_PLAN_LDS_WORDS (6 * GRS_PLAN_LDS_SEGS + 5 * 16)

template <int BLOCK, int NV>
__device__ __forceinline__ void block_scan(uint32_t (&v)[NV], uint32_t* wsum, uint32_t (&tot)[NV]) {
  constexpr int W = BLOCK / GRS_WAVE;
  const uint32_t t = threadIdx.x, lane = t & (GRS_WAVE - 1), w = t >> 6;
  uint32_t inc[NV];
#pragma unroll
  for (int q = 0; q < NV; ++q) {
    inc[q] = wave_scan_dpp(v[q]);
    if (lane == GRS_WAVE - 1) wsum[q * W + w] = inc[q];
// ... 22 lines not shown
                               const uint32_t* __restrict__ room = nullptr) {
  constexpr uint32_t G = GRS_LB_GROUP;
  const uint32_t t = threadIdx.x;
  const bool in_lds = nseg < GRS_PLAN_LDS_SEGS;
  uint32_t* const tpre = in_lds ? lds : spill;
  const uint32_t cap = in_lds ? GRS_PLAN_LDS_SEGS : nseg + 1;
  uint32_t* const rpre = tpre + cap;
  uint32_t* const gpre = rpre + cap;
  uint32_t* const sst = gpre + cap;
  uint32_t* const sln = sst + cap;
  uint32_t* const shr = sln + cap;
  uint32_t* const wsum = lds + 6 * GRS_PLAN_LDS_SEGS;
  uint32_t carry[5] = {0, 0, 0, 0, 0};
  for (uint32_t c0 = 0; c0 < nseg; c0 += BLOCK) {
    const uint32_t i = c0 + t;
    uint32_t len = 0, st = 0, hr = i;
    if (i < nseg) {
      if constexpr (SRC == kSegSizes) {
        len = a[i];
      } else if constexpr (SRC == kSegList || SRC == kSegMoved) {
        st = a[i];
        len = b[i];
        hr = c[i];
      } else {
        st = a[i];
        len = a[i + 1] - st;
      }
    }
    const uint32_t tl = len / TILE + (len % TILE != 0u ? 1u : 0u);
    const uint32_t multi = tl > 1 ? tl : 0u;
    uint32_t v[5] = {tl, multi, (multi + G - 1) / G, len, multi ? 1u : 0u}, tot[5];
    block_scan<BLOCK, 5>(v, wsum, tot);
    if (i < nseg) {
      tpre[i] = carry[0] + v[0];
      rpre[i] = carry[1] + v[1];
      gpre[i] = carry[2] + v[2];
      sst[i] = SRC == kSegSizes ? carry[3] + v[3] : st;
      sln[i] = len;
      shr[i] = SRC == kSegOffsets ? carry[4] + v[4] : hr;
    }
#pragma unroll
    for (int q = 0; q < 5; ++q) carry[q] += tot[q];
  }
  if (t == 0) tpre[nseg] = carry[0];
  __syncthreads();
  const uint32_t tiles = carry[0];
  for (uint32_t tk = t; tk < tiles; tk += BLOCK) {
    uint32_t lo = 0, hi = nseg;
    while (hi - lo > 1) {
      const uint32_t mid = (lo + hi) >> 1;
      if (tpre[mid] <= tk) lo = mid; else hi = mid;
    }
    const uint32_t j = tk - tpre[lo];
    const uint32_t tl = tpre[lo + 1] - tpre[lo];
    const uint32_t len = sln[lo];
    const uint32_t q = j / G;
    const uint32_t flags = (j % G) | (min(G, tl - q * G) << 4) | ((tl == 1 ? 1u : 0u) << 8) | (q << 9) |
                           (j + 1 == tl ? 0x80000000u : 0u);
    const uint32_t out = SRC == kSegMoved ? shr[lo] : sst[lo];
    rec[tk] = SegTile{rpre[lo] + j, gpre[lo] + q, flags, sst[lo] + j * TILE, min(TILE, len - j * TILE),
                      out, room != nullptr ? room[lo] : len, SRC == kSegMoved ? lo : shr[lo]};
  }
  if (t == 0) {
    hdr[0] = tiles;
    hdr[1] = carry[2];
    hdr[2] = carry[1];
  }
}

template <uint32_t TILE, int SRC>
__global__ __launch_bounds__(1024) void grs_seg_plan(const uint32_t* __restrict__ a,
                                                     const uint32_t* __restrict__ b,
                                                     const uint32_t* __restrict__ c,
                                                     uint32_t nseg_host,
                                                     const uint32_t* __restrict__ nseg_dev,
                                                     uint32_t* __restrict__ spill,
                                                     SegTile* __restrict__ rec,
                                                     uint32_t* __restrict__ hdr) {
  __shared__ uint32_t lds[GRS_PLAN_LDS_WORDS];
  const uint32_t nseg = nseg_dev != nullptr ? *nseg_dev : nseg_host;
  seg_plan_block<TILE, 1024, SRC>(a, b, c, nseg, spill, rec, hdr, lds);
}

template <typename K, int ND, bool SOLO = false>
__global__ __launch_bounds__(256) void grs_seg_hist(const K* __restrict__ keys,
                                                    const SegTile* __restrict__ rec,
                                                    const uint32_t* __restrict__ hdr, int shift0,
                                                    uint32_t* __restrict__ rows,
                                                    uint32_t* __restrict__ zero, uint32_t radix,
                                                    const uint32_t* __restrict__ shift_dev = nullptr) {
  __shared__ uint32_t h[ND * 256];
  const uint32_t t = threadIdx.x;
  const uint32_t tiles = hdr[0];
  if (shift_dev != nullptr) shift0 += static_cast<int>(__builtin_amdgcn_readfirstlane(*shift_dev));
  const size_t zw = static_cast<size_t>(hdr[2] + 2 * hdr[1]) * radix;
  for (size_t i = static_cast<size_t>(blockIdx.x) * 256 + t; i < zw; i += static_cast<size_t>(gridDim.x) * 256)
    zero[i] = 0;
  for (uint32_t k = blockIdx.x; k < tiles; k += gridDim.x) {
    const SegTile r = rec[k];
    if (!SOLO && ((r.flags >> 8) & 1u)) continue;
    for (uint32_t i = t; i < ND * 256; i += 256) h[i] = 0;
    __syncthreads();
    constexpr uint32_t U = 8;
    for (uint32_t i0 = t; i0 < r.valid; i0 += 256 * U) {
      K x[U];
#pragma unroll
      for (uint32_t u = 0; u < U; ++u) {
        const uint32_t i = i0 + u * 256;
        x[u] = i < r.valid ? keys[r.base + i] : K(0);
      }
#pragma unroll
      for (uint32_t u = 0; u < U; ++u) {
        if (i0 + u * 256 < r.valid) {
#pragma unroll
          for (int p = 0; p < ND; ++p)
            atomicAdd(&h[p * 256 + static_cast<uint32_t>((x[u] >> (shift0 + 8 * p)) & 255u)], 1u);
        }
      }
    }
    __syncthreads();
    for (uint32_t i = t; i < ND * 256; i += 256)
      if (h[i] != 0u) atomicAdd(&rows[static_cast<size_t>(r.seg) * ND * 256 + i], h[i]);
    __syncthreads();
  }
}

#define GRS_H2_CHUNK 262144
#define GRS_H2_COPIES 32
#ifndef GRS_H2_INFLIGHT
#define GRS_H2_INFLIGHT 8
#endif
#define GRS_MSD_SAMPLE_CHUNKS 16384
#define GRS_MSD_GUESS_CHUNKS 64

#define GRS_MSD_SPAN 1024

template <typename K>
__host__ __device__ inline uint32_t msd_top_shift(K varying) {
  constexpr int KB = 8 * static_cast<int>(sizeof(K));
  int hb = -1;
  for (int b = KB - 1; b >= 0; --b)
    if ((varying >> b) & K(1)) {
      hb = b;
      break;
    }
  const int s = hb - 7;
  return static_cast<uint32_t>(s < 8 ? 8 : s > KB - 8 ? KB - 8 : s);
}
template <typename K>
__device__ __forceinline__ K span_join(uint32_t lo, uint32_t hi) {
  if constexpr (sizeof(K) == 8) return (static_cast<K>(hi) << 32) | lo;
  else return static_cast<K>(lo);
}
template <int RMAX>
__device__ __forceinline__ int msd_p3_rounds(uint32_t s) {
  const int r = (static_cast<int>(s) - 8 + 7) / 8;
  return r < 1 ? 1 : r > RMAX ? RMAX : r;
}

template <typename K>
__global__ __launch_bounds__(256) void grs_msd_sample(const K* __restrict__ keys, uint32_t n,
                                                      uint32_t* __restrict__ samp,
                                                      uint32_t* __restrict__ clear, uint32_t clear_words,
                                                      uint32_t* __restrict__ clear_ctrl,
                                                      uint32_t* __restrict__ clear2, uint32_t clear2_words,
                                                      uint32_t* __restrict__ span) {
  __shared__ uint32_t h[256];
  __shared__ uint32_t sv[4];
  const uint32_t t = threadIdx.x, lane = t & (GRS_WAVE - 1);
  h[t] = 0;
  if (t < 4) sv[t] = 0;
  constexpr uint32_t GC = GRS_MSD_GUESS_CHUNKS, GK = GC * GRS_WAVE / 256;
  K g[GK];
#pragma unroll
  for (uint32_t u = 0; u < GK; ++u) {
    const uint32_t i = u * 256 + t;
    const uint32_t pos = n <= GC * GRS_WAVE
                             ? i
                             : static_cast<uint32_t>(static_cast<uint64_t>(i >> 6) * (n - GRS_WAVE) / (GC - 1)) + (i & 63u);
    g[u] = i < n ? keys[pos] : K(0);
  }
  const uint32_t gs = gridDim.x * 256;
  auto zero16 = [&](uint32_t* p, uint32_t words) {
    uint4* const q = reinterpret_cast<uint4*>(p);
    const uint32_t nv = words / 4;
    for (uint32_t i = blockIdx.x * 256 + t; i < nv; i += gs) q[i] = make_uint4(0u, 0u, 0u, 0u);
    for (uint32_t i = nv * 4 + blockIdx.x * 256 + t; i < words; i += gs) p[i] = 0;
  };
  zero16(clear, clear_words);
  zero16(clear2, clear2_words);
  constexpr uint32_t H = GRS_CTRL_HIST_WORDS, TK = GRS_MAX_PASSES * GRS_XCDS;
  zero16(clear_ctrl, H + TK);
  K o = 0, no = 0;
#pragma unroll
  for (uint32_t u = 0; u < GK; ++u)
    if (u * 256 + t < n) {
      o |= g[u];
      no |= static_cast<K>(~g[u]);
    }
  uint32_t v[4] = {static_cast<uint32_t>(o), static_cast<uint32_t>(static_cast<uint64_t>(o) >> 32),
                   static_cast<uint32_t>(no), static_cast<uint32_t>(static_cast<uint64_t>(no) >> 32)};
#pragma unroll
  for (int q = 0; q < 4; ++q) {
#pragma unroll
    for (int s = 32; s > 0; s >>= 1) v[q] |= __shfl_xor(v[q], s);
  }
  __syncthreads();
  if (lane == 0)
    for (int q = 0; q < 4; ++q) atomicOr(&sv[q], v[q]);
  __syncthreads();
  const uint32_t top = msd_top_shift<K>(span_join<K>(sv[0], sv[1]) & span_join<K>(sv[2], sv[3]));
  if (blockIdx.x == 0 && t == 0) span[4] = top;
  auto bin = [&](K k) { return static_cast<uint32_t>(k >> top) & 255u; };
  constexpr uint32_t C = GRS_MSD_SAMPLE_CHUNKS;
  if (n <= C * GRS_WAVE) {
    for (uint32_t i0 = blockIdx.x * 256 + t; i0 < n; i0 += 4 * gs) {
      K x[4];
#pragma unroll
      for (uint32_t u = 0; u < 4; ++u) x[u] = i0 + u * gs < n ? keys[i0 + u * gs] : K(0);
#pragma unroll
      for (uint32_t u = 0; u < 4; ++u)
        if (i0 + u * gs < n) atomicAdd(&h[bin(x[u])], 1u);
    }
  } else {
    constexpr uint32_t U = 16;
    const uint32_t waves = gridDim.x * 4;
    for (uint32_t c0 = blockIdx.x * 4 + (t >> 6); c0 < C; c0 += U * waves) {
      K k[U];
#pragma unroll
      for (uint32_t u = 0; u < U; ++u) {
        const uint32_t c = c0 + u * waves;
        const uint32_t pos = static_cast<uint32_t>(static_cast<uint64_t>(c) * (n - GRS_WAVE) / (C - 1));
        k[u] = c < C ? keys[pos + lane] : K(0);
      }
#pragma unroll
      for (uint32_t u = 0; u < U; ++u)
        if (c0 + u * waves < C) atomicAdd(&h[bin(k[u])], 1u);
    }
  }
  __syncthreads();
  if (h[t] != 0u) atomicAdd(&samp[t], h[t]);
}

template <typename K, uint32_t TILEF>
__global__ __launch_bounds__(256) void grs_msd_span(uint32_t n, uint32_t* __restrict__ span,
                                                    uint32_t* __restrict__ totals,
                                                    SegTile* __restrict__ rec, uint32_t* __restrict__ hdr) {
  __shared__ uint32_t tiles;
  const uint32_t t = threadIdx.x;
  if (t == 0) {
    const uint32_t sx = msd_top_shift<K>(span_join<K>(span[0], span[1]) & span_join<K>(span[2], span[3]));
    bool redo = totals[256] != 0u;
    if (sx != span[4]) {
      span[4] = sx;
      totals[256] = 1u;
      redo = true;
    }
    tiles = redo ? n / TILEF + (n % TILEF != 0u ? 1u : 0u) : 0u;
  }
  __syncthreads();
  constexpr uint32_t G = GRS_LB_GROUP;
  const uint32_t T = tiles;
  for (uint32_t k = t; k < T; k += 256) {
    const uint32_t q = k / G;
    const uint32_t flags = (k % G) | (min(G, T - q * G) << 4) | ((T == 1 ? 1u : 0u) << 8) | (q << 9) |
                           (k + 1 == T ? 0x80000000u : 0u);
    rec[k] = SegTile{k, q, flags, k * TILEF, min(TILEF, n - k * TILEF), 0u, n, 0u};
  }
  if (t == 0) {
    hdr[0] = T;
    hdr[1] = T > 1 ? (T + G - 1) / G : 0u;
    hdr[2] = T > 1 ? T : 0u;
  }
}

__device__ void msd_bucket_table(const uint32_t* __restrict__ samp, unsigned long long mult,
                                 uint32_t pad, const uint32_t* __restrict__ totals,
                                 const uint32_t* __restrict__ exact, uint32_t chunk, uint32_t* in,
                                 uint32_t* len, uint32_t* out, uint32_t* cpre, uint32_t* wsum) {
  const uint32_t t = threadIdx.x;
  const bool redo = totals[256] != 0u;
  uint32_t v[3] = {0, 0, 0}, tot[3];
  if (t < 256) {
    const uint32_t l = redo ? exact[t] : totals[t];
    const uint32_t r = redo ? l : static_cast<uint32_t>((static_cast<unsigned long long>(samp[t]) * mult) >> 20) + pad;
    v[0] = l;
    v[1] = r;
    v[2] = (l + chunk - 1) / chunk;
    len[t] = l;
  }
  block_scan<1024, 3>(v, wsum, tot);
  if (t < 256) {
    out[t] = v[0];
    in[t] = v[1];
    cpre[t] = v[2];
  }
  if (t == 0) cpre[256] = tot[2];
  __syncthreads();
}

template <uint32_t TILE2>
__global__ __launch_bounds__(1024) void grs_msd_plan2(const uint32_t* __restrict__ samp,
                                                      unsigned long long mult, uint32_t pad,
                                                      const uint32_t* __restrict__ totals,
                                                      const uint32_t* __restrict__ exact,
                                                      uint32_t chunk, uint32_t* __restrict__ tab,
// ... 71 lines not shown
  const uint32_t head = min(cl, (VEC - mis) % VEC);
  const uint32_t nv = (cl - head) / VEC;
  const uint4* kv = reinterpret_cast<const uint4*>(kc + head);
  auto count4 = [&](const uint4& x) {
    const K* e = reinterpret_cast<const K*>(&x);
#pragma unroll
    for (uint32_t q = 0; q < VEC; ++q) count(e[q]);
  };
  if (sample_shift != 0) {
    constexpr uint32_t VL = VEC == 4 ? 2 : 1;
    const uint32_t pul = piece_log - VL, PU = 1u << pul;
    const uint32_t np = (nv + PU - 1) >> pul;
    const uint32_t ns = ((np + (1u << sample_shift) - 1) >> sample_shift) << pul;
    auto at = [&](uint32_t m) { return ((m >> pul) << (sample_shift + pul)) + (m & (PU - 1u)); };
    uint32_t m = t;
    constexpr int U = GRS_H2_INFLIGHT;
    for (; m + (U - 1) * B < ns; m += U * B) {
      uint4 x[U];
      bool ok[U];
#pragma unroll
      for (int u = 0; u < U; ++u) {
        const uint32_t v = at(m + u * B);
        ok[u] = v < nv;
        x[u] = kv[ok[u] ? v : 0u];
      }
#pragma unroll
      for (int u = 0; u < U; ++u) asm volatile("" ::"v"(x[u].x), "v"(x[u].y), "v"(x[u].z), "v"(x[u].w));
#pragma unroll
      for (int u = 0; u < U; ++u) {
        const K* e = reinterpret_cast<const K*>(&x[u]);
        const uint32_t one = ok[u] ? 1u : 0u;
#pragma unroll
        for (uint32_t q = 0; q < VEC; ++q)
          atomicAdd(base + (static_cast<uint32_t>(e[q] >> SH) & 255u) * GRS_H2_COPIES, one);
      }
    }
    for (; m < ns; m += B) {
      const uint32_t v = at(m);
      if (v < nv) count4(kv[v]);
    }
    flush();
    return;
  }
  if (t < head) count(kc[t]);
  uint32_t i = t;
  constexpr int U = GRS_H2_INFLIGHT;
  for (; i + (U - 1) * B < nv; i += U * B) {
    uint4 x[U];
#pragma unroll
    for (int u = 0; u < U; ++u) x[u] = kv[i + u * B];
#pragma unroll
    for (int u = 0; u < U; ++u) asm volatile("" ::"v"(x[u].x), "v"(x[u].y), "v"(x[u].z), "v"(x[u].w));
#pragma unroll
    for (int u = 0; u < U; ++u) count4(x[u]);
  }
  for (; i < nv; i += B) count4(kv[i]);
  for (uint32_t r = head + nv * VEC + t; r < cl; r += B) count(kc[r]);
  flush();
}

__global__ __launch_bounds__(256) void grs_msd_regions(const uint32_t* __restrict__ tab,
                                                       const uint32_t* __restrict__ hs,
                                                       uint32_t* __restrict__ reg, uint32_t* __restrict__ room) {
  __shared__ uint32_t wsum[4];
  const uint32_t s = blockIdx.x, t = threadIdx.x;
  const uint32_t c = hs[s * 256 + t];
  uint32_t v[1] = {c}, ts[1];
  block_scan<256, 1>(v, wsum, ts);
  const uint32_t L = tab[257 + s];
  uint32_t r = L;
  if (ts[0] != 0u) {
    const float scale = static_cast<float>(L) / static_cast<float>(ts[0]);
    const float e = static_cast<float>(c) * scale + 6.0f * scale * sqrtf(static_cast<float>(c) + 1.0f) + 64.0f;
    r = e < static_cast<float>(L) ? static_cast<uint32_t>(e) : L;
  }
  reg[s * 256 + t] = r;
  __shared__ uint64_t part[4];
  uint64_t r64 = r;
  for (int o = 32; o > 0; o >>= 1) r64 += __shfl_xor(r64, o);
  if ((t & 63u) == 0) part[t >> 6] = r64;
  __syncthreads();
  if (t == 0) {
    const uint64_t all = part[0] + part[1] + part[2] + part[3];
    room[s] = all >= (uint64_t(1) << 31) ? 0xFFFFFFFFu : static_cast<uint32_t>(all);
  }
}

template <uint32_t TILE2>
__global__ __launch_bounds__(1024) void grs_msd_plan3(const uint32_t* __restrict__ tab,
                                                      const uint32_t* __restrict__ room_g, uint64_t cap2,
                                                      SegTile* __restrict__ rec, uint32_t* __restrict__ hdr,
                                                      uint32_t* __restrict__ spill) {
  __shared__ uint32_t lds[GRS_PLAN_LDS_WORDS + 4 * 257 + 64];
  uint32_t* const in = lds + GRS_PLAN_LDS_WORDS;
  uint32_t* const len = in + 257;
  uint32_t* const out = len + 257;
  uint32_t* const room = out + 257;
  uint32_t* const wsum = room + 257;
  const uint32_t t = threadIdx.x;
  uint64_t r64 = 0;
  if (t < 256) {
    in[t] = tab[t];
    len[t] = tab[257 + t];
    room[t] = room_g[t];
    r64 = room[t];
  }
  for (int o = 32; o > 0; o >>= 1) r64 += __shfl_xor(r64, o);
  __shared__ uint64_t wtot[16];
  if ((t & 63u) == 0) wtot[t >> 6] = r64;
  uint32_t v[1] = {t < 256 ? room[t] : 0u}, tot[1];
  block_scan<1024, 1>(v, wsum, tot);
  if (t < 256) out[t] = v[0];
  uint64_t all = 0;
  for (int k = 0; k < 16; ++k) all += wtot[k];
  __syncthreads();
  if (all > cap2 || all >= (uint64_t(1) << 32)) {
    if (t == 0) {
      hdr[0] = 0;
      hdr[1] = 0;
      hdr[2] = 0;
      *spill = 1u;
    }
    return;
  }
  seg_plan_block<TILE2, 1024, kSegMoved>(in, len, out, 256u, nullptr, rec, hdr, lds, room);
}

__global__ __launch_bounds__(256) void grs_msd_starts(const uint32_t* __restrict__ spill,
                                                      const uint32_t* __restrict__ tab,
                                                      const uint32_t* __restrict__ rtot,
                                                      const uint32_t* __restrict__ xcnt,
                                                      const uint32_t* __restrict__ rstart,
                                                      uint32_t* __restrict__ len2, uint32_t* __restrict__ in2,
                                                      uint32_t* __restrict__ out2) {
  __shared__ uint32_t wsum[4];
  const bool sp = *spill != 0u;
  const uint32_t s = blockIdx.x, t = threadIdx.x, b = s * 256 + t;
  const uint32_t l = sp ? xcnt[b] : rtot[b];
  uint32_t v[1] = {l}, tot[1];
  block_scan<256, 1>(v, wsum, tot);
  const uint32_t o = tab[2 * 257 + s] + v[0];
  len2[b] = l;
  out2[b] = o;
  in2[b] = sp ? o : rstart[b];
}

template <typename K, bool PAIRS>
__global__ __launch_bounds__(256) void grs_msd_copy_big(const K* __restrict__ rk, const uint32_t* __restrict__ rv,
                                                        K* __restrict__ keys, uint32_t* __restrict__ vals,
                                                        const uint32_t* __restrict__ spill,
                                                        const uint32_t* __restrict__ big,
                                                        const uint32_t* __restrict__ big_in,
                                                        const uint32_t* __restrict__ big_out,
                                                        const uint32_t* __restrict__ big_len) {
  if (*spill != 0u) return;
  const uint32_t count = big[0];
  for (uint32_t e = 0; e < count; ++e) {
    const uint32_t a = big_in[e], o = big_out[e], n = big_len[e];
    for (uint32_t i = blockIdx.x * 256 + threadIdx.x; i < n; i += gridDim.x * 256) {
      keys[o + i] = rk[a + i];
      if constexpr (PAIRS) vals[o + i] = rv[a + i];
    }
  }
}

template <typename K, bool PAIRS, int BLOCK, int I, bool C16, int RMAX = (8 * static_cast<int>(sizeof(K)) - 16) / 8>
struct LocalSort {
  static constexpr uint32_t W = BLOCK / GRS_WAVE, SMAX = BLOCK * I;
  static constexpr int ROUNDS = RMAX;
  static_assert(W <= 16 && BLOCK >= 256, "digit threads: waves 0..3");
  static_assert(!C16 || SMAX < 65536, "16-bit positions");
  static constexpr uint32_t KV = 16 / sizeof(K), VV = 4;
  template <uint32_t V>
  __device__ __forceinline__ static uint32_t swz_t(uint32_t x) {
#if GRS_P3_LDS_LAYOUT == 0
    return x;
#elif GRS_P3_LDS_LAYOUT == 2
    return x + ((x >> 8) * V);
#else
    return x ^ (((x >> 8) & 15u) << (V == 4 ? 2 : V == 2 ? 1 : 0));
#endif
  }
  __device__ __forceinline__ static uint32_t swz(uint32_t x) { return swz_t<KV>(x); }
  __device__ __forceinline__ static uint32_t swzv(uint32_t x) { return swz_t<VV>(x); }
  template <uint32_t V>
  __device__ __forceinline__ static uint32_t swz_row(uint32_t base, uint32_t lane) {
#if GRS_P3_LDS_LAYOUT == 0
    return base + lane;
#elif GRS_P3_LDS_LAYOUT == 2
    return base + (base >> 8) * V + lane;
#else
    return base + (lane ^ (((base >> 8) & 15u) << (V == 4 ? 2 : V == 2 ? 1 : 0)));
#endif
  }
  template <uint32_t V>
  static constexpr uint32_t lds_len(uint32_t n) {
    return GRS_P3_LDS_LAYOUT == 2 ? (n + (n >> 8) * V + 63) / 64 * 64 : (n + 63) / 64 * 64;
  }
  static constexpr uint32_t SK = lds_len<KV>(SMAX + KV);
  struct Smem {
    alignas(16) K sk[SK];
    alignas(16) uint32_t sv[PAIRS ? lds_len<VV>(SMAX + VV) : 4];
    uint32_t cnt[W * 256 / (C16 ? 2 : 1)];
    uint32_t wtot[4];
    uint32_t slot;
  };
  using Vals = uint32_t[PAIRS ? I : 1];
  __device__ __forceinline__ static void run(Smem& sm, K* __restrict__ keys, uint32_t* __restrict__ vals,
                                             uint32_t lo, uint32_t len) {
    run(sm, keys, vals, keys, vals, lo, len, ROUNDS);
  }
  __device__ __forceinline__ static void run(Smem& sm, const K* kin, const uint32_t* vin, K* kout,
                                             uint32_t* vout, uint32_t lo, uint32_t len, int rounds) {
    K k[I];
    Vals v;
    load(k, v, kin, vin, lo, len);
    sort_rounds(sm, k, v, len, rounds);
    store(sm, kout, vout, lo, len);
  }
  __device__ __forceinline__ static void load(K (&k)[I], Vals& v, const K* kin, const uint32_t* vin,
                                              uint32_t lo, uint32_t len, uint32_t t = threadIdx.x) {
    const uint32_t lane = t & (GRS_WAVE - 1), w = t >> 6;
#pragma unroll
    for (uint32_t j = 0; j < I; ++j) {
      const uint32_t i = w * GRS_WAVE * I + j * GRS_WAVE + lane;
      k[j] = i < len ? kin[lo + i] : K(0);
      if constexpr (PAIRS) v[j] = i < len ? vin[lo + i] : 0u;
    }
  }
  __device__ __forceinline__ static void sort_rounds(Smem& sm, K (&k)[I], Vals& v, uint32_t len, int rounds,
                                                     uint32_t ak = 0, uint32_t av = 0, int shift0 = 0,
                                                     uint32_t t = threadIdx.x) {
    uint16_t* const c16 = reinterpret_cast<uint16_t*>(sm.cnt);
    auto cld = [&](uint32_t a) -> uint32_t { if constexpr (C16) return c16[a]; else return sm.cnt[a]; };
    auto cst = [&](uint32_t a, uint32_t x) {
      if constexpr (C16) c16[a] = static_cast<uint16_t>(x); else sm.cnt[a] = x;
    };
    const uint32_t lane = t & (GRS_WAVE - 1), w = t >> 6;
#pragma unroll
    for (int pass = 0; pass < ROUNDS; ++pass) {
      if (pass >= rounds) break;
      const int shift = shift0 + 8 * pass;
      auto digit = [&](K x) { return static_cast<uint32_t>(x >> shift) & 255u; };
      for (uint32_t c = t; c < W * 256 / (C16 ? 2 : 1); c += BLOCK) sm.cnt[c] = 0;
      __syncthreads();
      uint32_t r[I];
#pragma unroll
      for (uint32_t j = 0; j < I; ++j) {
        const uint32_t i = w * GRS_WAVE * I + j * GRS_WAVE + lane;
        const uint32_t d = digit(k[j]);
        if constexpr (C16) {
          const uint32_t sh = (d & 1u) << 4;
          r[j] = i < len ? (atomicAdd(&sm.cnt[(w * 256 + d) >> 1], 1u << sh) >> sh) & 0xFFFFu : 0u;
        } else {
          r[j] = i < len ? atomicAdd(&sm.cnt[w * 256 + d], 1u) : 0u;
        }
      }
      __syncthreads();
      uint32_t c[W], tot = 0, incl = 0;
      if (t < 256) {
#pragma unroll
        for (uint32_t ww = 0; ww < W; ++ww) {
          c[ww] = cld(ww * 256 + t);
          tot += c[ww];
        }
        incl = wave_scan_dpp(tot);
        if (lane == GRS_WAVE - 1) sm.wtot[w] = incl;
      }
      __syncthreads();
      if (t < 256) {
        uint32_t b = incl - tot;
#pragma unroll
        for (uint32_t ww = 0; ww < 4; ++ww) b += ww < w ? sm.wtot[ww] : 0u;
#pragma unroll
        for (uint32_t ww = 0; ww < W; ++ww) {
          cst(ww * 256 + t, b);
          b += c[ww];
        }
      }
      __syncthreads();
      const bool last = pass + 1 >= rounds;
      const uint32_t sk_off = last ? ak : 0u, sv_off = last ? av : 0u;
#pragma unroll
      for (uint32_t j = 0; j < I; ++j) {
        const uint32_t i = w * GRS_WAVE * I + j * GRS_WAVE + lane;
        if (i < len) {
          const uint32_t dst = cld(w * 256 + digit(k[j])) + r[j];
          sm.sk[swz(dst + sk_off)] = k[j];
          if constexpr (PAIRS) sm.sv[swzv(dst + sv_off)] = v[j];
        }
      }
      __syncthreads();
      if (pass + 1 < rounds) {
        const uint32_t ws = __builtin_amdgcn_readfirstlane(w);
#pragma unroll
        for (uint32_t j = 0; j < I; ++j) {
          const uint32_t base = ws * GRS_WAVE * I + j * GRS_WAVE;
          if (base + lane < len) {
            k[j] = sm.sk[swz_row<KV>(base, lane)];
            if constexpr (PAIRS) v[j] = sm.sv[swz_row<VV>(base, lane)];
          }
        }
      }
    }
  }
  __device__ __forceinline__ static void store(Smem& sm, K* kout, uint32_t* vout, uint32_t lo, uint32_t len) {
    for (uint32_t i = threadIdx.x; i < len; i += BLOCK) {
      kout[lo + i] = sm.sk[swz(i)];
      if constexpr (PAIRS) vout[lo + i] = sm.sv[swzv(i)];
    }
  }

  template <typename T, uint32_t V>
  __device__ __forceinline__ static uint32_t mis(const T* at) {
    return static_cast<uint32_t>(reinterpret_cast<uintptr_t>(at) / sizeof(T)) % V;
  }
  template <typename T, uint32_t V, bool ROT = true>
  __device__ __forceinline__ static void copy_out(T* run, const T* lds, uint32_t len, uint32_t seed = blockIdx.x) {
    const uint32_t t = threadIdx.x, a = mis<T, V>(run);
    const uint32_t head = min(len, (V - a) % V);
    const uint32_t nv = (len - head) / V;
    if (t < head) run[t] = lds[swz_t<V>(a + t)];
    uint4* dst = reinterpret_cast<uint4*>(run + head);
    const uint32_t rot = ROT && nv != 0u ? ((seed * 97u & 255u) * 16u) % nv : 0u;
    for (uint32_t c = t; c < nv; c += BLOCK) {
      uint32_t r = c + rot;
      if (r >= nv) r -= nv;
      dst[r] = *reinterpret_cast<const uint4*>(lds + swz_t<V>(a + head + r * V));
    }
    const uint32_t r = head + nv * V + t;
    if (r < len) run[r] = lds[swz_t<V>(a + r)];
  }
  template <bool ROT = true>
  __device__ __forceinline__ static void run_vec(Smem& sm, const K* kin, const uint32_t* vin, K* kout,
                                                 uint32_t* vout, uint32_t len, int rounds) {
    K k[I];
    Vals v;
    auto ld = [&]() { load(k, v, kin, vin, 0u, len); };
    ld();
    const uint32_t ak = mis<K, KV>(kout), av = PAIRS ? mis<uint32_t, VV>(vout) : 0u;
    if (ROUNDS > 2 && rounds > 2) {
      if constexpr (ROUNDS > 2) {
        sort_rounds(sm, k, v, len, 2, ak, av, 8 * rounds - 16);
        if (finish_runs(sm, len, 8 * rounds - 16, ak, av)) {
          ld();
          sort_rounds(sm, k, v, len, rounds, ak, av);
        }
      }
    } else {
      sort_rounds(sm, k, v, len, rounds, ak, av);
    }
    copy_out<K, KV, ROT>(kout, sm.sk, len);
    if constexpr (PAIRS) copy_out<uint32_t, VV, ROT>(vout, sm.sv, len);
  }
  static constexpr uint32_t kRunMax = 48;
  __device__ __forceinline__ static bool finish_runs(Smem& sm, uint32_t len, int hb, uint32_t ak, uint32_t av) {
    __syncthreads();
    if (threadIdx.x == 0) sm.slot = 0;
    __syncthreads();
    auto A = [&](uint32_t p) -> K& { return sm.sk[swz(ak + p)]; };
    auto B = [&](uint32_t p) -> uint32_t& { return sm.sv[swzv(av + p)]; };
    for (uint32_t p = threadIdx.x; p < len; p += BLOCK) {
      const K hi = A(p) >> hb;
      if (p != 0 && (A(p - 1) >> hb) == hi) continue;
      uint32_t e = p + 1;
      while (e < len && (A(e) >> hb) == hi && e - p <= kRunMax) ++e;
      if (e - p > kRunMax) {
        sm.slot = 1;
        continue;
      }
      for (uint32_t q = p + 1; q < e; ++q) {
        const K x = A(q);
        uint32_t y = 0;
        if constexpr (PAIRS) y = B(q);
        uint32_t r = q;
        while (r > p && A(r - 1) > x) {
          A(r) = A(r - 1);
          if constexpr (PAIRS) B(r) = B(r - 1);
          --r;
        }
        A(r) = x;
        if constexpr (PAIRS) B(r) = y;
      }
    }
    __syncthreads();
    return sm.slot != 0u;
  }
};

#ifndef GRS_P3H_GROUP
#define GRS_P3H_GROUP 8
#endif
template <int BLOCK, int I>
struct LocalSort16 {
  static_assert(I % 2 == 0, "two keys a register");
  static constexpr uint32_t W = BLOCK / GRS_WAVE, SMAX = BLOCK * I, IP = I / 2;
  static constexpr uint32_t G = GRS_P3H_GROUP;
  static_assert(W <= 16 && BLOCK >= 256 && SMAX < 65536, "digit threads: waves 0..3; 16-bit counters");
  __device__ __forceinline__ static uint32_t swz(uint32_t x) { return x ^ (((x >> 8) & 15u) << 2); }
  __device__ __forceinline__ static uint32_t swz_row(uint32_t base, uint32_t lane) {
    return base + (lane ^ (((base >> 8) & 15u) << 2));
  }
  static constexpr uint32_t SK = (SMAX + 4 + 63) / 64 * 64;
  struct Smem {
    alignas(16) uint16_t sk[SK];
    uint32_t cnt[W * 128];
    uint32_t spare[GRS_WAVE];
    uint32_t wtot[4];
    uint32_t slot;
  };
  __device__ __forceinline__ static uint32_t half(const uint32_t (&p)[IP], uint32_t j) {
    return (p[j >> 1] >> (16 * (j & 1))) & 0xFFFFu;
  }
  __device__ __forceinline__ static void run(Smem& sm, const uint32_t* kin, uint32_t* kout, uint32_t len,
                                             int rounds) {
    const uint32_t t = threadIdx.x, lane = t & (GRS_WAVE - 1), w = t >> 6;
    const uint32_t hi = __builtin_amdgcn_readfirstlane(kin[0]) & 0xFFFF0000u;
    const auto rsrc = __builtin_amdgcn_make_buffer_rsrc(const_cast<uint32_t*>(kin), 0, static_cast<int>(4u * len),
                                                        0x00020000);
    const uint32_t ws = __builtin_amdgcn_readfirstlane(w), wbase = ws * GRS_WAVE * I;
    const uint32_t wlen = len > wbase ? len - wbase : 0u;
    uint32_t kp[IP];
#pragma unroll
    for (uint32_t j = 0; j < IP; ++j) {
      const uint32_t a = __builtin_amdgcn_raw_buffer_load_b16(rsrc, 4u * lane, 4u * (wbase + 2u * j * GRS_WAVE), 0);
      const uint32_t b = __builtin_amdgcn_raw_buffer_load_b16(rsrc, 4u * lane, 4u * (wbase + (2u * j + 1u) * GRS_WAVE), 0);
      kp[j] = (a & 0xFFFFu) | (b << 16);
    }
    const uint32_t ak = static_cast<uint32_t>(reinterpret_cast<uintptr_t>(kout) / 4u) % 4u;
    uint16_t* const c16 = reinterpret_cast<uint16_t*>(sm.cnt);
#pragma unroll
    for (int pass = 0; pass < 2; ++pass) {
      if (pass >= rounds) break;
      const uint32_t shift = 8u * static_cast<uint32_t>(pass);
      for (uint32_t c = t; c < W * 128; c += BLOCK) sm.cnt[c] = 0;
      __syncthreads();
      uint32_t rp[IP];
#pragma unroll
      for (uint32_t j = 0; j < I; ++j) {
        const uint32_t d = (half(kp, j) >> shift) & 255u, sh = (d & 1u) << 4;
        const bool ok = lane + j * GRS_WAVE < wlen;
        const uint32_t r = (atomicAdd(ok ? &sm.cnt[(w * 256 + d) >> 1] : &sm.spare[lane], 1u << sh) >> sh) & 0xFFFFu;
        if (j & 1) rp[j >> 1] |= r << 16;
        else rp[j >> 1] = r;
        if (j % G == G - 1) __builtin_amdgcn_sched_barrier(0);
      }
#pragma unroll
      for (uint32_t j = 0; j < IP; ++j) asm volatile("" : "+v"(kp[j]), "+v"(rp[j]));
      __syncthreads();
      uint32_t c[W], tot = 0, incl = 0;
      if (t < 256) {
#pragma unroll
        for (uint32_t ww = 0; ww < W; ++ww) {
          c[ww] = c16[ww * 256 + t];
          tot += c[ww];
        }
        incl = wave_scan_dpp(tot);
        if (lane == GRS_WAVE - 1) sm.wtot[w] = incl;
      }
      __syncthreads();
      if (t < 256) {
        uint32_t b = incl - tot;
#pragma unroll
        for (uint32_t ww = 0; ww < 4; ++ww) b += ww < w ? sm.wtot[ww] : 0u;
#pragma unroll
        for (uint32_t ww = 0; ww < W; ++ww) {
          c16[ww * 256 + t] = static_cast<uint16_t>(b);
          b += c[ww];
        }
      }
      __syncthreads();
      const uint32_t off = pass + 1 >= rounds ? ak : 0u;
#pragma unroll
      for (uint32_t j = 0; j < I; ++j) {
        const uint32_t x = half(kp, j);
        const uint32_t dst = lane + j * GRS_WAVE < wlen ? c16[w * 256 + ((x >> shift) & 255u)] + half(rp, j)
                                                        : wbase + j * GRS_WAVE + lane;
        sm.sk[swz(dst + off)] = static_cast<uint16_t>(x);
        if (j % G == G - 1) __builtin_amdgcn_sched_barrier(0);
      }
      __syncthreads();
      if (pass + 1 < rounds) {
#pragma unroll
        for (uint32_t j = 0; j < IP; ++j) {
          const uint32_t b0 = wbase + 2u * j * GRS_WAVE, b1 = b0 + GRS_WAVE;
          kp[j] = static_cast<uint32_t>(sm.sk[swz_row(b0, lane)]) | (static_cast<uint32_t>(sm.sk[swz_row(b1, lane)]) << 16);
        }
      }
    }
    const uint32_t head = min(len, (4u - ak) % 4u), nv = (len - head) / 4u;
    if (t < head) kout[t] = hi | sm.sk[swz(ak + t)];
    uint4* const dst = reinterpret_cast<uint4*>(kout + head);
    const uint32_t rot = nv != 0u ? ((blockIdx.x * 97u & 255u) * 16u) % nv : 0u;
    for (uint32_t c = t; c < nv; c += BLOCK) {
      uint32_t r = c + rot;
      if (r >= nv) r -= nv;
      const uint2 g = *reinterpret_cast<const uint2*>(sm.sk + swz(ak + head + r * 4u));
      dst[r] = make_uint4(hi | (g.x & 0xFFFFu), hi | (g.x >> 16), hi | (g.y & 0xFFFFu), hi | (g.y >> 16));
    }
    const uint32_t r = head + nv * 4u + t;
    if (r < len) kout[r] = hi | sm.sk[swz(ak + r)];
  }
};

template <typename K, bool PAIRS, int BLOCK, uint32_t SMAX, uint32_t ND, uint32_t TILEF>
__device__ __forceinline__ void msd_local_other(uint32_t len, uint32_t lo, uint32_t o, bool inplace, const K* kin,
                                                const uint32_t* vin, K* keys, uint32_t* vals, uint32_t mid_max,
                                                uint32_t* mid, uint32_t* big, uint32_t* big_in,
                                                uint32_t* big_start, uint32_t* big_len, uint32_t* big_row,
                                                uint32_t* rows, uint32_t& slot) {
  const uint32_t t = threadIdx.x;
  if (len == 1u) {
    if (!inplace && t == 0) {
      keys[o] = kin[lo];
      if constexpr (PAIRS) vals[o] = vin[lo];
    }
    return;
  }
  if (len <= SMAX) return;
  if (len <= mid_max) {
    if (t == 0) {
      const uint32_t e = atomicAdd(&mid[0], 1u);
      mid[2 + 3 * e] = lo;
      mid[3 + 3 * e] = o;
      mid[4 + 3 * e] = len;
    }
    return;
  }
  if (t == 0) {
    const uint32_t e = atomicAdd(&big[0], 1u);
    const uint32_t row = len > TILEF ? atomicAdd(&big[1], 1u) : 0xFFFFFFFFu;
    big_in[e] = lo;
    big_start[e] = o;
    big_len[e] = len;
    big_row[e] = row;
    slot = row;
  }
  __syncthreads();
  const uint32_t row = slot;
  if (row != 0xFFFFFFFFu)
    for (uint32_t i = t; i < ND * 256; i += BLOCK) rows[static_cast<size_t>(row) * ND * 256 + i] = 0;
}

template <typename K, bool PAIRS, int BLOCK, int I, bool C16, uint32_t TILEF>
__global__ __launch_bounds__(BLOCK) void grs_msd_local(K* __restrict__ keys, uint32_t* __restrict__ vals,
                                                       const K* __restrict__ rk, const uint32_t* __restrict__ rv,
                                                       const uint32_t* __restrict__ spill,
                                                       const uint32_t* __restrict__ len2,
                                                       const uint32_t* __restrict__ in2,
                                                       const uint32_t* __restrict__ out2,
                                                       uint32_t mid_max, uint32_t* __restrict__ mid,
                                                       uint32_t* __restrict__ big,
                                                       uint32_t* __restrict__ big_in,
                                                       uint32_t* __restrict__ big_start,
                                                       uint32_t* __restrict__ big_len,
                                                       uint32_t* __restrict__ big_row,
                                                       uint32_t* __restrict__ rows,
                                                       const uint32_t* __restrict__ top_shift) {
  using LS = LocalSort<K, PAIRS, BLOCK, I, C16>;
  constexpr uint32_t ND = LS::ROUNDS;
  __shared__ typename LS::Smem sm;
  const uint32_t len = len2[blockIdx.x];
  if (len == 0u) return;
  const bool inplace = __builtin_amdgcn_readfirstlane(*spill) != 0u;
  const uint32_t lo = in2[blockIdx.x], o = out2[blockIdx.x];
  const K* const kin = inplace ? keys : rk;
  const uint32_t* const vin = inplace ? vals : rv;
  if (len == 1u || len > LS::SMAX) {
    msd_local_other<K, PAIRS, BLOCK, LS::SMAX, ND, TILEF>(len, lo, o, inplace, kin, vin, keys, vals, mid_max, mid,
                                                          big, big_in, big_start, big_len, big_row, rows, sm.slot);
    return;
  }
  const int rounds = msd_p3_rounds<LS::ROUNDS>(__builtin_amdgcn_readfirstlane(*top_shift));
  LS::template run_vec<>(sm, kin + lo, PAIRS ? vin + lo : nullptr, keys + o, PAIRS ? vals + o : nullptr, len,
                         rounds);
}

template <int BLOCK, int I, int MINW, uint32_t TILEF>
__global__ __launch_bounds__(BLOCK, MINW) void grs_msd_local16(
    uint32_t* __restrict__ keys, uint32_t* __restrict__ vals, const uint32_t* __restrict__ rk,
    const uint32_t* __restrict__ rv, const uint32_t* __restrict__ spill, const uint32_t* __restrict__ len2,
    const uint32_t* __restrict__ in2, const uint32_t* __restrict__ out2, uint32_t mid_max, uint32_t* __restrict__ mid,
    uint32_t* __restrict__ big, uint32_t* __restrict__ big_in, uint32_t* __restrict__ big_start,
    uint32_t* __restrict__ big_len, uint32_t* __restrict__ big_row, uint32_t* __restrict__ rows,
    const uint32_t* __restrict__ top_shift) {
  using LS = LocalSort16<BLOCK, I>;
  __shared__ typename LS::Smem sm;
  const uint32_t len = len2[blockIdx.x];
  if (len == 0u) return;
  const bool inplace = __builtin_amdgcn_readfirstlane(*spill) != 0u;
  const uint32_t lo = in2[blockIdx.x], o = out2[blockIdx.x];
  const uint32_t* const kin = inplace ? keys : rk;
  if (len == 1u || len > LS::SMAX) {
    msd_local_other<uint32_t, false, BLOCK, LS::SMAX, 2, TILEF>(len, lo, o, inplace, kin, nullptr, keys, vals, mid_max,
                                                                mid, big, big_in, big_start, big_len, big_row, rows,
                                                                sm.slot);
    return;
  }
  LS::run(sm, kin + lo, keys + o, len, msd_p3_rounds<2>(__builtin_amdgcn_readfirstlane(*top_shift)));
}

template <typename K, bool PAIRS, int BLOCK, int I, bool C16, uint32_t TILEF, int MINW>
__global__ __launch_bounds__(BLOCK, MINW) void grs_msd_local_pf(
    K* __restrict__ keys, uint32_t* __restrict__ vals, const K* __restrict__ rk, const uint32_t* __restrict__ rv,
    const uint32_t* __restrict__ spill, const uint32_t* __restrict__ len2, const uint32_t* __restrict__ in2,
    const uint32_t* __restrict__ out2, uint32_t mid_max, uint32_t* __restrict__ mid, uint32_t* __restrict__ big,
    uint32_t* __restrict__ big_in, uint32_t* __restrict__ big_start, uint32_t* __restrict__ big_len,
    uint32_t* __restrict__ big_row, uint32_t* __restrict__ rows, const uint32_t* __restrict__ top_shift,
    uint32_t* __restrict__ ticket) {
  using LS = LocalSort<K, PAIRS, BLOCK, I, C16>;
  static_assert(LS::ROUNDS <= 2, "u64 keys: grs_msd_local (its run finish may reload the keys)");
  constexpr uint32_t ND = LS::ROUNDS, NSEG = 65536;
  __shared__ typename LS::Smem sm;
  __shared__ uint32_t nxt;
  const uint32_t t = threadIdx.x;
  const bool inplace = __builtin_amdgcn_readfirstlane(*spill) != 0u;
  const K* const kin = inplace ? keys : rk;
  const uint32_t* const vin = inplace ? vals : rv;
  const int rounds = msd_p3_rounds<LS::ROUNDS>(__builtin_amdgcn_readfirstlane(*top_shift));
  auto sorted_here = [](uint32_t l) { return l >= 2u && l <= LS::SMAX; };
  if (t == 0) nxt = atomicAdd(ticket, 1u);
  __syncthreads();
  uint32_t b = __builtin_amdgcn_readfirstlane(nxt);
  K k[I];
  typename LS::Vals v;
  uint32_t len = b < NSEG ? len2[b] : 0u;
  if (b < NSEG && sorted_here(len)) LS::load(k, v, kin, vin, in2[b], len);
  while (b < NSEG) {
    __syncthreads();
    if (t == 0) nxt = atomicAdd(ticket, 1u);
    const uint32_t lo = in2[b], o = out2[b];
    const bool here = sorted_here(len);
    if (here) {
      const uint32_t ak = LS::template mis<K, LS::KV>(keys + o);
      const uint32_t av = PAIRS ? LS::template mis<uint32_t, LS::VV>(vals + o) : 0u;
      uint32_t tt = t;
      asm volatile("" : "+v"(tt));
      LS::sort_rounds(sm, k, v, len, rounds, ak, av, 0, tt);
    } else {
      if (len != 0u)
        msd_local_other<K, PAIRS, BLOCK, LS::SMAX, ND, TILEF>(len, lo, o, inplace, kin, vin, keys, vals, mid_max,
                                                              mid, big, big_in, big_start, big_len, big_row, rows,
                                                              sm.slot);
      __syncthreads();
    }
    const uint32_t nb = __builtin_amdgcn_readfirstlane(nxt);
    const uint32_t nlen = nb < NSEG ? len2[nb] : 0u;
    if (nb < NSEG && sorted_here(nlen)) {
      uint32_t tt = t;
      asm volatile("" : "+v"(tt));
      LS::load(k, v, kin, vin, in2[nb], nlen, tt);
    }
    if (here) {
      LS::template copy_out<K, LS::KV>(keys + o, sm.sk, len, b);
      if constexpr (PAIRS) LS::template copy_out<uint32_t, LS::VV>(vals + o, sm.sv, len, b);
    }
    b = nb;
    len = nlen;
  }
}

template <typename K, bool PAIRS, int BLOCK, int I, bool C16, int MINW>
__global__ __launch_bounds__(BLOCK, MINW) void grs_msd_local_list(K* __restrict__ keys,
                                                            uint32_t* __restrict__ vals,
                                                            const K* __restrict__ rk,
                                                            const uint32_t* __restrict__ rv,
                                                            const uint32_t* __restrict__ spill,
                                                            const uint32_t* __restrict__ mid,
                                                            const uint32_t* __restrict__ top_shift,
                                                            const uint32_t* __restrict__ big = nullptr,
                                                            const uint32_t* __restrict__ big_in = nullptr,
                                                            const uint32_t* __restrict__ big_out = nullptr,
                                                            const uint32_t* __restrict__ big_len = nullptr) {
  using LS = LocalSort<K, PAIRS, BLOCK, I, C16>;
  __shared__ typename LS::Smem sm;
  const bool inplace = *spill != 0u;
  if (big != nullptr && !inplace) {
    const uint32_t nb = big[0];
    for (uint32_t e = 0; e < nb; ++e) {
      const uint32_t a = big_in[e], o = big_out[e], n = big_len[e];
      for (uint32_t i = blockIdx.x * BLOCK + threadIdx.x; i < n; i += gridDim.x * BLOCK) {
        keys[o + i] = rk[a + i];
        if constexpr (PAIRS) vals[o + i] = rv[a + i];
      }
    }
  }
  const uint32_t count = mid[0];
  if (count == 0u) return;
  const K* const kin = inplace ? keys : rk;
  const uint32_t* const vin = inplace ? vals : rv;
  const int rounds = msd_p3_rounds<LS::ROUNDS>(__builtin_amdgcn_readfirstlane(*top_shift));
  for (uint32_t e = blockIdx.x; e < count; e += gridDim.x) {
    const uint32_t lo = mid[2 + 3 * e], o = mid[3 + 3 * e], len = mid[4 + 3 * e];
    LS::template run_vec<>(sm, kin + lo, PAIRS ? vin + lo : nullptr, keys + o, PAIRS ? vals + o : nullptr,
                           len, rounds);
    __syncthreads();
  }
}

template <uint32_t CP, uint32_t CL, uint32_t TILEF, int ND>
__global__ __launch_bounds__(256) void grs_seg_runs(const uint32_t* __restrict__ off,
                                                    const uint32_t* __restrict__ ds, uint32_t* __restrict__ cnt,
                                                    uint32_t* __restrict__ prim, uint32_t* __restrict__ mid,
                                                    uint32_t* __restrict__ bstart,
                                                    uint32_t* __restrict__ blen, uint32_t* __restrict__ brow,
                                                    uint32_t* __restrict__ rows) {
  constexpr uint32_t NONE = 0xFFFFFFFFu;
  __shared__ uint32_t es[257], eb[257], rl[256], wsum[3 * 4], base[3];
  const uint32_t s = blockIdx.x, t = threadIdx.x;
  const uint32_t lo = off[s], hi = off[s + 1];
  if (hi <= lo) return;
  const uint32_t st = ds[static_cast<size_t>(s) * 256 + t];
  const uint32_t en = t < 255u ? ds[static_cast<size_t>(s) * 256 + t + 1] : hi;
  rl[t] = en - st;
  __syncthreads();
  if (t < GRS_WAVE) {
    uint32_t cur = CP + 1;
    uint32_t q4[4];
#pragma unroll
    for (int q = 0; q < 4; ++q) q4[q] = rl[q * GRS_WAVE + t];
#pragma unroll
    for (int q = 0; q < 4; ++q) {
      uint64_t m = 0;
#pragma unroll
      for (int j = 0; j < GRS_WAVE; ++j) {
        const uint32_t l = __builtin_amdgcn_readlane(q4[q], j);
        const bool open = cur > CP || l > CP - cur;
        cur = open ? l : cur + l;
        if (l > CP) cur = CP + 1;
        m |= static_cast<uint64_t>(open) << j;
      }
      rl[q * GRS_WAVE + t] = static_cast<uint32_t>(m >> t) & 1u;
    }
  }
  __syncthreads();
  uint32_t f[1] = {rl[t]}, ne[1];
  const uint32_t is_first = f[0];
  block_scan<256, 1>(f, wsum, ne);
  const uint32_t E = ne[0];
  if (is_first) {
    es[f[0]] = st;
    eb[f[0]] = t;
  }
  if (t == 0) {
    es[E] = hi;
    eb[E] = 256;
  }
  __syncthreads();
  uint32_t s0 = 0, l = 0, nb = 0;
  if (t < E) {
    s0 = es[t];
    l = es[t + 1] - s0;
    nb = eb[t + 1] - eb[t];
  }
  uint32_t cls[3] = {l != 0u && l <= CP ? 1u : 0u, l > CP && l <= CL ? 1u : 0u, l > CL ? 1u : 0u}, tot[3];
  const uint32_t k0 = cls[0], k1 = cls[1], k2 = cls[2];
  block_scan<256, 3>(cls, wsum, tot);
  if (t == 0) {
    base[0] = tot[0] ? atomicAdd(&cnt[0], tot[0]) : 0u;
    base[1] = tot[1] ? atomicAdd(&cnt[1], tot[1]) : 0u;
    base[2] = tot[2] ? atomicAdd(&cnt[2], tot[2]) : 0u;
  }
  __syncthreads();
  const uint32_t lw = l | (nb > 1u ? 0x80000000u : 0u);
  if (k0) {
    const uint32_t e = base[0] + cls[0];
    prim[2 * e] = s0;
    prim[2 * e + 1] = lw;
  } else if (k1) {
    const uint32_t e = base[1] + cls[1];
    mid[2 * e] = s0;
    mid[2 * e + 1] = lw;
  } else if (k2) {
    const uint32_t e = base[2] + cls[2];
    const uint32_t row = l > TILEF ? atomicAdd(&cnt[3], 1u) : NONE;
    bstart[e] = s0;
    blen[e] = l;
    brow[e] = row;
    if (row != NONE)
      for (uint32_t i = 0; i < ND * 256; ++i) rows[static_cast<size_t>(row) * ND * 256 + i] = 0;
  }
}

template <typename K, bool PAIRS, int BLOCK, int I, bool C16, int MINW>
__global__ __launch_bounds__(BLOCK, MINW) void grs_seg_local_list(const K* __restrict__ kin,
                                                                  const uint32_t* __restrict__ vin,
                                                                  K* __restrict__ kout,
                                                                  uint32_t* __restrict__ vout,
                                                                  const uint32_t* __restrict__ count_p,
                                                                  const uint32_t* __restrict__ list) {
  constexpr int KR = static_cast<int>(sizeof(K));
  using LS = LocalSort<K, PAIRS, BLOCK, I, C16, KR>;
  __shared__ typename LS::Smem sm;
  const uint32_t count = *count_p;
  for (uint32_t e = blockIdx.x; e < count; e += gridDim.x) {
    const uint32_t lw = list[2 * e + 1];
    LS::run(sm, kin, vin, kout, vout, list[2 * e], lw & 0x7FFFFFFFu, (lw >> 31) ? KR : KR - 1);
    __syncthreads();
  }
}

}
```

### gpuradixsort_amd/csrc/grs_pass.hpp

```cpp
#pragma once

#include <type_traits>

#include "grs_kernels.hpp"

namespace grs {

__host__ __device__ constexpr size_t lb3_status_words(size_t tiles, size_t radix) {
  return (tiles + 2 * ((tiles + GRS_LB_GROUP - 1) / GRS_LB_GROUP)) * radix;
}

struct PassDebug {
  uint32_t fault_tile1;
  uint32_t spin_limit;
  __device__ __forceinline__ static PassDebug read(const uint32_t* error_word) {
    const uint32_t lim = error_word[2];
    return PassDebug{error_word[1], lim != 0u ? lim : static_cast<uint32_t>(GRS_SPIN_LIMIT)};
  }
};

template <int RADIX, int GW = GRS_LB_GWIN>
struct Lb3 {
  static constexpr int G = GRS_LB_GROUP;
  uint32_t tw[G - 1];
// ... 325 lines not shown
      const uint32_t c = cnt_ld(ww * RADIX + t);
      cnt_st(ww * RADIX + t, tile_cnt);
      tile_cnt += c;
    }
    publish = (t == dmask) ? tile_cnt - pad : tile_cnt;
    if (solo) {
      gh = publish;
    } else {
      if (tile + 1u != dbg.fault_tile1)
        st_status(status + static_cast<size_t>(tile) * RADIX + t, publish + 1u);
      gold = __hip_atomic_fetch_add(gacc + static_cast<size_t>(sp.group) * RADIX + t,
                                    (1u << 24) | publish, __ATOMIC_RELAXED, __HIP_MEMORY_SCOPE_AGENT);
    }
  }
  if (w < static_cast<uint32_t>(DW)) {
    const uint32_t li = wave_scan_dpp(tile_cnt);
    const uint32_t gi = wave_scan_dpp(gh);
    if (lane == GRS_WAVE - 1) {
      sm.wsum[w] = li;
      sm.wsum[WAVES + w] = gi;
    }
    lstart = li - tile_cnt;
    gstart = gi - gh;
  }
  lds_barrier();

  Lb3<RADIX, (ROUNDS > 1 ? GRS_LB_GWIN_XL : GRS_LB_GWIN)> lb;
  if (t < static_cast<uint32_t>(RADIX)) {
    for (uint32_t ww = 0; ww < w; ++ww) {
      lstart += sm.wsum[ww];
      gstart += sm.wsum[WAVES + ww];
    }
    if (digit_starts != nullptr) digit_starts[t] = sp.seg_start + gstart;
#pragma unroll
    for (int ww = 0; ww < WAVES; ++ww) cnt_st(ww * RADIX + t, cnt_ld(ww * RADIX + t) + lstart);
    if constexpr (IDX) {
      sm.lstart[t] = lstart;
      if (t == static_cast<uint32_t>(RADIX - 1)) sm.lstart[RADIX] = TILE;
    }
    if constexpr (!LATE_LB) {
      if (!solo) lb.issue(status, gacc, ginc, tile, t, sp.jg, sp.group, sp.g0);
    }
  }
  lds_barrier();

  if constexpr (IDX) {
    for (uint32_t c = t; c < static_cast<uint32_t>(TILE / GRS_WAVE); c += BLOCK) {
      uint32_t d0 = 0, d1 = 0;
#pragma unroll
      for (int b = 1; b < RADIX; ++b) {
        const uint32_t ls = sm.lstart[b];
        d0 += ls <= c * GRS_WAVE;
        d1 += ls <= c * GRS_WAVE + GRS_WAVE - 1;
      }
      sm.cdig[c] = static_cast<uint16_t>(d0 | (d1 << 8));
    }
  }
#pragma unroll
  for (int j = 0; j < ITEMS; ++j) asm volatile("" : "+v"(key[j]));
#pragma unroll
  for (int j = 0; j < ITEMS; ++j) {
    uint32_t r = (j & 1) ? rank[j / 2] >> 16 : rank[j / 2] & 0xFFFFu;
    uint32_t d;
    if constexpr (IDX) {
      d = r >> 12;
      r &= 0xFFFu;
    } else {
      d = dig_of(j);
    }
    const uint32_t pos = cnt_ld(w * RADIX + d) + r;
    if (ROUNDS == 1 || pos < static_cast<uint32_t>(LTILE)) {
      sm.keys[pos] = key[j];
      if constexpr (PAIRS) sm.vals[pos] = val[j];
    }
    if constexpr (ROUNDS > 1) {
      if (j & 1)
        rank[j / 2] = (rank[j / 2] & 0xFFFFu) | (pos << 16);
      else
        rank[j / 2] = (rank[j / 2] & 0xFFFF0000u) | pos;
    }
  }
  if constexpr (LATE_LB) {
    if (t < static_cast<uint32_t>(RADIX) && !solo) lb.issue(status, gacc, ginc, tile, t, sp.jg, sp.group, sp.g0);
  }
  uint32_t next = tiles;
  if constexpr (PF && ROUNDS == 1) {
    next = __builtin_amdgcn_readfirstlane(sm.next);
    if (next < tiles) tile_load<K, PAIRS, BLOCK, ITEMS, OPT>(key, val, keys_in, vals_in, n, next, t);
  }
  if (t < static_cast<uint32_t>(RADIX)) {
    const uint32_t prefix =
        solo ? 0u
             : lb.finish(status, gacc, ginc, tile, sp.jg, sp.group, sp.in_group, t, gold, publish,
                         error_word, dbg.spin_limit);
    if constexpr ((OPT & 131072) != 0) {
      if (sp.last) {
        const uint32_t tot = prefix + publish;
        region_totals[t] = tot;
        if (tot > gh) atomicOr(spill_flag != nullptr ? spill_flag : &region_totals[RADIX], 1u);
      }
    }
    uint32_t start = gstart + prefix;
    if constexpr (!IDX) {
      const uint64_t last = sp.seg_len >= publish ? static_cast<uint64_t>(sp.seg_len - publish) : 0u;
      const uint64_t want = static_cast<uint64_t>(gstart) + static_cast<uint64_t>(prefix);
#ifndef GRS_TEST_NO_CLAMP
      start = sp.seg_start + static_cast<uint32_t>(want < last ? want : last);
#else
      (void)last;
      start = sp.seg_start + static_cast<uint32_t>(want);
#endif
    }
#ifdef GRS_DIAG
    if (diag_lim[0] != 0u && publish != 0u && start + publish > diag_lim[0] &&
        atomicCAS(&diag_hit[8], 0u, 1u) == 0u) {
      diag_hit[9] = tile;
      diag_hit[10] = t;
      diag_hit[11] = start;
      diag_hit[12] = gstart;
      diag_hit[13] = prefix;
      diag_hit[14] = sp.seg_start;
      diag_hit[15] = sp.seg_len;
      diag_hit[16] = publish;
      diag_hit[17] = gh;
      diag_hit[18] = sp.base;
      diag_hit[19] = sp.valid;
      diag_hit[20] = lstart;
    }
#endif
    sm.base[t] = start - lstart;
  }
  lds_barrier();

  constexpr bool SPAN = (OPT & 262144) != 0;
  K s_or = 0, s_nor = 0;
  auto put = [&](uint32_t dst, K kk, uint32_t i) {
#ifdef GRS_DIAG
    if (diag_lim[0] != 0u && dst >= diag_lim[0]) {
      atomicAdd(&diag_hit[0], 1u);
      atomicMax(&diag_hit[1], dst);
      return;
    }
#endif
    if constexpr ((OPT & 8192) != 0) {
      static_assert(PAIRS && sizeof(K) == 4, "records: u32 key + u32 value");
      const uint2 r = make_uint2(static_cast<uint32_t>(kk), sm.vals[i]);
      const unsigned long long x = (static_cast<unsigned long long>(r.y) << 32) | r.x;
      if constexpr ((OPT & 32768) != 0) {
        if (dst >= n / 2) reinterpret_cast<unsigned long long*>(vals_out)[dst - n / 2] = x;
        else reinterpret_cast<unsigned long long*>(keys_out)[dst] = x;
      } else {
        reinterpret_cast<unsigned long long*>(keys_out)[dst] = x;
      }
    } else {
      keys_out[dst] = kk;
      if constexpr (PAIRS) vals_out[dst] = sm.vals[i];
    }
  };
  auto dig_at = [&](uint32_t i, K kk) -> uint32_t {
    if constexpr (IDX) {
      const uint32_t c = sm.cdig[i >> 6];
      uint32_t d = c & 255u;
      if (d != (c >> 8))
        while (i >= sm.lstart[d + 1]) ++d;
      return d;
    } else {
      return dig(kk);
    }
  };
#pragma unroll
  for (int rr = 0; rr < ROUNDS; ++rr) {
    if (rr > 0) {
      lds_barrier();
#pragma unroll
      for (int j = 0; j < ITEMS; ++j) {
        const uint32_t pos = (j & 1) ? rank[j / 2] >> 16 : rank[j / 2] & 0xFFFFu;
        const uint32_t lp = pos - static_cast<uint32_t>(rr * LTILE);
        if (lp < static_cast<uint32_t>(LTILE)) {
          sm.keys[lp] = key[j];
          if constexpr (PAIRS) sm.vals[lp] = val[j];
        }
      }
      lds_barrier();
      if constexpr (PF) {
        if (rr == ROUNDS - 1) {
          next = __builtin_amdgcn_readfirstlane(sm.next);
          if (next < tiles) tile_load<K, PAIRS, BLOCK, ITEMS, OPT>(key, val, keys_in, vals_in, n, next, t);
        }
      }
    }
    const uint32_t roff = static_cast<uint32_t>(rr * LTILE);
    if (valid == static_cast<uint32_t>(TILE)) {
#pragma unroll
      for (int k = 0; k < LITEMS; ++k) {
        const uint32_t i = k * BLOCK + t;
        const K kk = sm.keys[i];
        const uint32_t d = dig_at(roff + i, kk);
        put(sm.base[d] + roff + i, kk, i);
        if constexpr (SPAN) {
          s_or |= kk;
          s_nor |= static_cast<K>(~kk);
        }
      }
    } else {
#pragma unroll
      for (int k = 0; k < LITEMS; ++k) {
        const uint32_t i = k * BLOCK + t;
        if (roff + i < valid) {
          const K kk = sm.keys[i];
          const uint32_t d = dig_at(roff + i, kk);
          put(sm.base[d] + roff + i, kk, i);
          if constexpr (SPAN) {
            s_or |= kk;
            s_nor |= static_cast<K>(~kk);
          }
        }
      }
    }
  }
  if constexpr (SPAN) {
    uint32_t v[4] = {static_cast<uint32_t>(s_or), static_cast<uint32_t>(static_cast<uint64_t>(s_or) >> 32),
                     static_cast<uint32_t>(s_nor), static_cast<uint32_t>(static_cast<uint64_t>(s_nor) >> 32)};
#pragma unroll
    for (int q = 0; q < 4; ++q) {
      if (sizeof(K) == 4 && (q & 1)) continue;
#pragma unroll
      for (int o = 32; o > 0; o >>= 1) v[q] |= __shfl_xor(v[q], o);
      if (lane == 0 && v[q] != 0u) atomicOr(&sm.span[q], v[q]);
    }
  }
  return next;
}

template <typename K, bool PAIRS, int RADIX, int BLOCK>
__device__ __forceinline__ void elided_tile(uint32_t mode, const TileSpan& sp, const K* __restrict__ keys_in,
                                            K* __restrict__ keys_out, const uint32_t* __restrict__ vals_in,
                                            uint32_t* __restrict__ vals_out, uint32_t* __restrict__ status_next) {
  const uint32_t t = threadIdx.x;
  if (t < static_cast<uint32_t>(RADIX)) {
    status_next[static_cast<size_t>(sp.tile) * RADIX + t] = 0;
    if (sp.jg == 0) {
      status_next[static_cast<size_t>(sp.tiles + sp.group) * RADIX + t] = 0;
      status_next[static_cast<size_t>(sp.tiles + sp.groups + sp.group) * RADIX + t] = 0;
    }
  }
  if (mode == kPassCopy) {
    for (uint32_t i = t; i < sp.valid; i += BLOCK) {
      keys_out[sp.base + i] = keys_in[sp.base + i];
      if constexpr (PAIRS) vals_out[sp.base + i] = vals_in[sp.base + i];
    }
  }
}

template <typename K, bool PAIRS, int RB, int BLOCK, int ITEMS, int MINW, int OPT = 0,
          typename DigitF = RadixDigit<K>>
__global__ __launch_bounds__(BLOCK, MINW) void grs_onesweep_v4(
    const K* __restrict__ keys_in, K* __restrict__ keys_out, const uint32_t* __restrict__ vals_in,
    uint32_t* __restrict__ vals_out, uint32_t n, const DigitF dig,
    const uint32_t* __restrict__ pass_hist, uint32_t* __restrict__ ticket,
    uint32_t* __restrict__ status, uint32_t* __restrict__ status_next,
    uint32_t* __restrict__ error_word, const DigitF* __restrict__ dig_dev,
    const uint32_t* __restrict__ plan = nullptr) {
  using SM = V4SmemFor<K, PAIRS, RB, BLOCK, ITEMS, OPT, DigitF>;
  __shared__ SM sm;
  const uint32_t t = threadIdx.x;
  uint32_t tt = t;
  asm volatile("" : "+v"(tt));
  K key[ITEMS];
  uint32_t val[ITEMS];
  const uint32_t mode = plan != nullptr ? __builtin_amdgcn_readfirstlane(*plan) : 0u;
  if (t == 0) sm.ticket = atomicAdd(ticket, 1u);
  for (uint32_t i = t; i < sizeof(sm.cnt) / 4; i += BLOCK) sm.cnt[i] = 0;
  const DigitF dg = dig_dev != nullptr ? *dig_dev : dig;
  __syncthreads();
  const uint32_t tile = __builtin_amdgcn_readfirstlane(sm.ticket);
  if (mode != 0u) {
    elided_tile<K, PAIRS, SM::RADIX, BLOCK>(mode, TileSpan::whole(tile, n, SM::TILE), keys_in, keys_out, vals_in,
                                            vals_out, status_next);
    return;
  }
  tile_load<K, PAIRS, BLOCK, ITEMS, OPT>(key, val, keys_in, vals_in, n, tile, tt);
  const uint32_t gh = t < static_cast<uint32_t>(SM::RADIX) ? pass_hist[t] : 0u;
  onesweep_tile<K, PAIRS, RB, BLOCK, ITEMS, OPT>(sm, TileSpan::whole(tile, n, SM::TILE), key, val,
                                                 keys_in, keys_out, vals_in,
                                                 vals_out, n, dg, gh, ticket, status, status_next,
                                                 error_word, PassDebug::read(error_word));
}

template <typename K, bool PAIRS, int RB, int BLOCK, int ITEMS, int MINW, int OPT>
__global__ __launch_bounds__(BLOCK, MINW) void grs_onesweep_region(
    const K* __restrict__ keys_in, K* __restrict__ keys_out, const uint32_t* __restrict__ vals_in,
    uint32_t* __restrict__ vals_out, uint32_t n, const RadixDigit<K> dig,
    const uint32_t* __restrict__ sample, unsigned long long mult, uint32_t pad,
    uint32_t region_len, uint32_t* __restrict__ ticket, uint32_t* __restrict__ status,
    uint32_t* __restrict__ status_next, uint32_t* __restrict__ error_word,
    uint32_t* __restrict__ totals, uint32_t* __restrict__ span) {
  constexpr int ROPT = OPT | 131072 | 262144;
  using SM = V4SmemFor<K, PAIRS, RB, BLOCK, ITEMS, ROPT, RadixDigit<K>>;
  __shared__ SM sm;
  const uint32_t t = threadIdx.x;
  uint32_t tt = t;
  asm volatile("" : "+v"(tt));
  K key[ITEMS];
  uint32_t val[ITEMS];
  if (t == 0) sm.ticket = atomicAdd(ticket, 1u);
  if (t < 4) sm.span[t] = 0;
// ... 177 lines not shown
```

### gpuradixsort_amd/sorter.py

```python
from __future__ import annotations

import ctypes
from typing import Optional

import torch

from ._lib import GRS_KEY_U32, GRS_KEY_U64, OPTIONS, check, grs_timing, lib

_KEY_TYPES = {torch.int32: GRS_KEY_U32, torch.uint32: GRS_KEY_U32,
              torch.int64: GRS_KEY_U64, torch.uint64: GRS_KEY_U64}


def _stream_ptr(stream: Optional[torch.cuda.Stream]) -> ctypes.c_void_p:
    s = stream if stream is not None else torch.cuda.current_stream()
    return ctypes.c_void_p(s.cuda_stream)


def _ptr(t: torch.Tensor) -> ctypes.c_void_p:
    return ctypes.c_void_p(t.data_ptr())


class RadixSorter:

    def __init__(self, capacity: int, key_bits: int = 32, pairs: bool = False,
                 radix_bits: int = 8, device: Optional[int] = None,
                 options: Optional[dict] = None):
        L = lib()
        if device is None:
            device = torch.cuda.current_device()
        self.capacity = int(capacity)
        self.key_bits = int(key_bits)
        self.pairs = bool(pairs)
        self.radix_bits = int(radix_bits)
        self.device = int(device)
        kt = GRS_KEY_U32 if key_bits == 32 else GRS_KEY_U64
        if key_bits not in (32, 64):
            raise ValueError("key_bits must be 32 or 64")
        h = ctypes.c_void_p()
        check(L.grs_create(ctypes.byref(h), self.capacity, kt, int(self.pairs), self.radix_bits,
                           self.device), "grs_create")
        self._h = h
        for name, value in (options or {}).items():
            self.set_option(name, value)

    def set_option(self, name: str, value) -> None:
        opt, names = OPTIONS[name]
        v = names[value] if isinstance(value, str) else int(value)
        check(lib().grs_set_option(self._h, opt, v), f"grs_set_option({name}={value})")

    def get_option(self, name: str) -> int:
        v = ctypes.c_int()
        check(lib().grs_get_option(self._h, OPTIONS[name][0], ctypes.byref(v)), "grs_get_option")
        return v.value

    def close(self) -> None:
        if getattr(self, "_h", None):
            lib().grs_destroy(self._h)
            self._h = None

    def __del__(self):
        try:
            self.close()
        except Exception:
            pass

    @property
    def scratch_bytes(self) -> int:
        return int(lib().grs_scratch_bytes(self._h))

    def check_guards(self) -> int:
        bad = ctypes.c_uint64()
        check(lib().grs_debug_check_guards(self._h, ctypes.byref(bad)), "grs_debug_check_guards")
        return int(bad.value)

    def msd_flags(self) -> dict:
        f = (ctypes.c_uint32 * 3)()
        check(lib().grs_debug_msd_flags(self._h, f), "grs_debug_msd_flags")
        return {"p1_redo": bool(f[0]), "p2_exact": bool(f[1]), "top_shift": int(f[2])}

    def p3_kernel(self, n: int) -> Optional[str]:
        kt = GRS_KEY_U32 if self.key_bits == 32 else GRS_KEY_U64
        name = lib().grs_debug_p3_kernel(kt, int(self.pairs), int(n), self.get_option("p3"),
                                         self.get_option("p3_shape"))
        return name.decode() if name else None

    @property
    def rank_mode(self) -> str:
        return {0: "atomic", 1: "match"}[int(lib().grs_rank_mode(self._h))]

    @property
    def pass_kernel(self) -> str:
        return self.pass_kernel_for(self.capacity)

    def pass_kernel_for(self, n: int) -> str:
        return lib().grs_pass_kernel(self._h, int(n)).decode()

    def _check_keys(self, keys: torch.Tensor, vals: Optional[torch.Tensor]) -> None:
        if not keys.is_cuda or not keys.is_contiguous():
            raise ValueError("keys must be a contiguous device tensor")
        if keys.element_size() * 8 != self.key_bits:
            raise ValueError(f"keys must be {self.key_bits}-bit")
        if self.pairs:
            if vals is None or vals.numel() < keys.numel() or vals.element_size() != 4 \
                    or not vals.is_contiguous() or not vals.is_cuda:
                raise ValueError("pairs sorter needs a contiguous 32-bit device payload tensor")
        elif vals is not None:
            raise ValueError("this sorter was created without a payload")

    @staticmethod
    def _check_n(n: Optional[int], *tensors: Optional[torch.Tensor]) -> int:
        n = tensors[0].numel() if n is None else int(n)
        if n < 0:
            raise ValueError("n must be >= 0")
        for t in tensors:
            if t is not None and t.numel() < n:
                raise ValueError(f"n = {n} exceeds a tensor of {t.numel()} items")
        return n

    def sort(self, keys: torch.Tensor, vals: Optional[torch.Tensor] = None, n: Optional[int] = None,
             begin_bit: int = 0, end_bit: Optional[int] = None,
             stream: Optional[torch.cuda.Stream] = None) -> None:
        self._check_keys(keys, vals)
        n = self._check_n(n, keys, vals)
        end_bit = self.key_bits if end_bit is None else int(end_bit)
        vp = _ptr(vals) if vals is not None else ctypes.c_void_p(0)
        check(lib().grs_sort_bits(self._h, _ptr(keys), vp, n, int(begin_bit), end_bit,
                                  _stream_ptr(stream)), "grs_sort")

    def partition(self, keys: torch.Tensor, keys_out: torch.Tensor, splitters, counts: torch.Tensor,
                  vals: Optional[torch.Tensor] = None, vals_out: Optional[torch.Tensor] = None,
                  n: Optional[int] = None, stream: Optional[torch.cuda.Stream] = None) -> None:
        import numpy as np

        self._check_keys(keys, vals)
        if not keys_out.is_cuda or not keys_out.is_contiguous() or keys_out.element_size() != keys.element_size():
            raise ValueError("keys_out must be a contiguous device tensor of the key width")
        if not counts.is_cuda or counts.element_size() != 4 or not counts.is_contiguous():
            raise ValueError("counts must be a contiguous 32-bit device tensor")
        n = self._check_n(n, keys, vals, keys_out, vals_out)
        sp = np.ascontiguousarray(np.asarray(splitters, dtype=np.uint32 if self.key_bits == 32
                                             else np.uint64))
        if counts.numel() < sp.size + 1:
            raise ValueError("counts needs len(splitters) + 1 entries")
        if self.pairs and (vals_out is None or not vals_out.is_cuda or not vals_out.is_contiguous()
                           or vals_out.element_size() != 4):
            raise ValueError("pairs partition needs a contiguous 32-bit device vals_out")
        vp = _ptr(vals) if vals is not None else ctypes.c_void_p(0)
        vo = _ptr(vals_out) if vals_out is not None else ctypes.c_void_p(0)
        check(lib().grs_partition(self._h, _ptr(keys), vp, _ptr(keys_out), vo, n,
                                  ctypes.c_void_p(sp.ctypes.data), int(sp.size), _ptr(counts),
                                  _stream_ptr(stream)), "grs_partition")

    def partition_regions(self, keys: torch.Tensor, keys_out: torch.Tensor, splitters, counts: torch.Tensor,
                          region: int, thresholds=None, vals: Optional[torch.Tensor] = None,
                          vals_out: Optional[torch.Tensor] = None, n: Optional[int] = None,
                          stream: Optional[torch.cuda.Stream] = None) -> None:
        import numpy as np

        self._check_keys(keys, vals)
        n = keys.numel() if n is None else int(n)
        sp = np.ascontiguousarray(np.asarray(splitters, dtype=np.uint32 if self.key_bits == 32
                                             else np.uint64))
        th = np.ascontiguousarray(np.zeros(sp.size, np.uint32) if thresholds is None
                                  else np.asarray(thresholds, dtype=np.uint32))
        need = sp.size * int(region) + n
        if (not keys_out.is_cuda or not keys_out.is_contiguous() or keys_out.numel() < need
                or keys_out.element_size() != keys.element_size()):
            raise ValueError(f"keys_out must be a contiguous device tensor of >= {need} keys")
        if self.pairs and (vals_out is None or vals_out.numel() < need or not vals_out.is_contiguous()):
            raise ValueError(f"pairs partition needs a contiguous vals_out of >= {need} items")
        if counts.numel() < sp.size + 1 or counts.element_size() != 4:
            raise ValueError("counts needs len(splitters) + 1 32-bit entries")
        vp = _ptr(vals) if vals is not None else ctypes.c_void_p(0)
        vo = _ptr(vals_out) if vals_out is not None else ctypes.c_void_p(0)
        check(lib().grs_partition_regions(self._h, _ptr(keys), vp, _ptr(keys_out), vo, n,
                                          ctypes.c_void_p(sp.ctypes.data), ctypes.c_void_p(th.ctypes.data),
                                          int(sp.size), int(region), _ptr(counts), _stream_ptr(stream)),
              "grs_partition_regions")

    def sort_host(self, keys, vals=None, stream: Optional[torch.cuda.Stream] = None) -> None:
        import numpy as np

        if not isinstance(keys, np.ndarray) or not keys.flags.c_contiguous \
                or keys.dtype.itemsize * 8 != self.key_bits:
            raise ValueError(f"keys must be a contiguous {self.key_bits}-bit numpy array")
        if (vals is not None) != self.pairs:
            raise ValueError("payload presence must match the sorter")
        if vals is not None and (vals.dtype.itemsize != 4 or vals.size < keys.size
                                 or not vals.flags.c_contiguous):
            raise ValueError("vals must be a contiguous 32-bit numpy array")
        kp = ctypes.c_void_p(keys.ctypes.data)
        vp = ctypes.c_void_p(vals.ctypes.data) if vals is not None else ctypes.c_void_p(0)
        check(lib().grs_sort_host(self._h, kp, kp, vp, vp, keys.size, _stream_ptr(stream)),
              "grs_sort_host")

    def sort_segmented(self, keys: torch.Tensor, offsets: torch.Tensor,
                       vals: Optional[torch.Tensor] = None, n: Optional[int] = None,
                       stream: Optional[torch.cuda.Stream] = None) -> None:
        if not self.pairs:
            raise ValueError("sort_segmented needs a sorter created with pairs=True")
        if not keys.is_cuda or not keys.is_contiguous() or keys.element_size() * 8 != self.key_bits:
            raise ValueError(f"keys must be a contiguous {self.key_bits}-bit device tensor")
        if not offsets.is_cuda or not offsets.is_contiguous() or offsets.element_size() != 4:
            raise ValueError("offsets must be a contiguous 32-bit device tensor")
        if vals is not None and (not vals.is_cuda or not vals.is_contiguous()
                                 or vals.element_size() != 4):
            raise ValueError("vals must be a contiguous 32-bit device tensor")
        n = self._check_n(n, keys, vals)
        if offsets.numel() < 2:
            raise ValueError("offsets needs num_segments + 1 >= 2 entries")
        vp = _ptr(vals) if vals is not None else ctypes.c_void_p(0)
        check(lib().grs_sort_segmented(self._h, _ptr(keys), vp, n, _ptr(offsets),
                                       offsets.numel() - 1, _stream_ptr(stream)),
              "grs_sort_segmented")

    def set_profiling(self, ring: int) -> None:
        check(lib().grs_set_profiling(self._h, int(ring)), "grs_set_profiling")

    def timing(self, k: int = 0) -> dict:
        t = grs_timing()
        check(lib().grs_timing_history(self._h, int(k), ctypes.byref(t)), "grs_timing_history")
        return {"passes": t.passes, "total_ms": t.total_ms, "hist_ms": t.hist_ms,
                "pass_ms": list(t.pass_ms)[: t.passes], "copy_ms": t.copy_ms,
                "kind": {1: "msd", 2: "fused"}.get(t.kind, "lsd")}

    def check_error(self, stream: Optional[torch.cuda.Stream] = None, device_wide: bool = False) -> None:
        if device_wide:
            check(lib().grs_check_error(self._h), "grs_check_error")
        else:
            check(lib().grs_stream_check_error(self._h, _stream_ptr(stream)), "grs_stream_check_error")

# ... 68 lines not shown
```

### include/grs.h

```cpp
#ifndef GRS_H_
#define GRS_H_

#include <stddef.h>
#include <stdint.h>

#ifdef __cplusplus
extern "C" {
#endif

#define GRS_VERSION 410

typedef enum grs_status {
  GRS_OK = 0,
  GRS_EINVAL = 1,
  GRS_ENOMEM = 2,
  GRS_EHIP = 3,
  GRS_ECAPACITY = 4,
  GRS_ENODEV = 5,
  GRS_ETIMEOUT = 6,
  GRS_ERCCL = 7
} grs_status;

#define GRS_MAX_N 0xFFFF0000ull

typedef enum grs_key_type { GRS_KEY_U32 = 0, GRS_KEY_U64 = 1 } grs_key_type;

typedef struct grs_sorter grs_sorter;

typedef struct grs_timing {
  int passes;
  float total_ms;
  float hist_ms;
  float pass_ms[16];
  float copy_ms;
  int kind;
} grs_timing;

int grs_version(void);
const char* grs_status_string(grs_status s);
const char* grs_last_error(void);

grs_status grs_create(grs_sorter** out, size_t capacity, grs_key_type key_type,
                      int with_u32_payload, int radix_bits, int device);
void grs_destroy(grs_sorter* s);

size_t grs_scratch_bytes(const grs_sorter* s);

grs_status grs_debug_check_guards(grs_sorter* s, uint64_t* bad_words);

grs_status grs_debug_msd_flags(grs_sorter* s, uint32_t flags[3]);

const char* grs_debug_p3_kernel(grs_key_type key_type, int pairs, size_t n, int p3_mode, int p3_shape);

int grs_rank_mode(const grs_sorter* s);

grs_status grs_lds_order_check(int device, int blocks, int items, unsigned long long* mismatches);

typedef enum grs_option {
  GRS_OPT_TILE = 1,
  GRS_OPT_XL = 2,
  GRS_OPT_PASS = 3,
  GRS_OPT_RECORDS = 4,
  GRS_OPT_RANK = 5,
  GRS_OPT_SHARDED_PATH = 6,
  GRS_OPT_SHARDED_SEND = 7,
  GRS_OPT_EXCHANGE = 8,
  GRS_OPT_MERGE = 9,
  GRS_OPT_FAULT_TILE = 10,
  GRS_OPT_MSD = 11,
  GRS_OPT_SEG_ROUTE = 12,
  GRS_OPT_H2_CHUNK = 13,
  GRS_OPT_H2_PIECE = 14,
  GRS_OPT_P3 = 15,
  GRS_OPT_X_CHUNKS = 16,
  GRS_OPT_P3_SHAPE = 17
} grs_option;
grs_status grs_set_option(grs_sorter* s, grs_option opt, int value);
grs_status grs_get_option(const grs_sorter* s, grs_option opt, int* value);

const char* grs_pass_kernel(const grs_sorter* s, size_t n);

grs_status grs_sort(grs_sorter* s, void* d_keys, uint32_t* d_vals, size_t n, void* stream);

grs_status grs_sort_bits(grs_sorter* s, void* d_keys, uint32_t* d_vals, size_t n,
                         int begin_bit, int end_bit, void* stream);

grs_status grs_set_profiling(grs_sorter* s, int ring);
grs_status grs_last_timing(grs_sorter* s, grs_timing* out);
grs_status grs_timing_history(grs_sorter* s, int k, grs_timing* out);
grs_status grs_check_error(grs_sorter* s);
grs_status grs_stream_check_error(grs_sorter* s, void* stream);

grs_status grs_partition(grs_sorter* s, const void* d_keys, const uint32_t* d_vals,
                         void* d_keys_out, uint32_t* d_vals_out, size_t n,
                         const void* splitters, int n_splitters, uint32_t* d_counts,
                         void* stream);

grs_status grs_partition_ranges(grs_sorter* s, const void* d_keys, const uint32_t* d_vals,
                                void* d_keys_out, uint32_t* d_vals_out, size_t n,
                                const void* splitters, const uint32_t* thresholds,
                                int n_splitters, uint32_t* d_counts, void* stream);

grs_status grs_partition_regions(grs_sorter* s, const void* d_keys, const uint32_t* d_vals,
                                 void* d_keys_out, uint32_t* d_vals_out, size_t n,
                                 const void* splitters, const uint32_t* thresholds,
                                 int n_splitters, size_t region, uint32_t* d_counts, void* stream);

grs_status grs_sort_sharded(grs_sorter* s, const void* d_keys_in, const uint32_t* d_vals_in,
                            size_t n_local, void* d_keys_out, uint32_t* d_vals_out,
                            size_t out_capacity, size_t* n_out, void* nccl_comm, void* stream);

typedef struct grs_sharded_timing {
  float total_ms, before_ms, exchange_ms, after_ms;
  uint64_t bytes_sent, bytes_received;
  int presorted;
} grs_sharded_timing;
grs_status grs_sharded_last_timing(grs_sorter* s, grs_sharded_timing* out);
grs_status grs_sharded_redo_count(const grs_sorter* s, uint64_t* count);

#define GRS_RCCL_ID_BYTES 128
grs_status grs_rccl_unique_id(void* id_out);
grs_status grs_rccl_comm_init(void** comm_out, const void* id, int nranks, int rank, int device);
void grs_rccl_comm_destroy(void* comm);

grs_status grs_shard_splitters_host(const void* sorted_keys, const uint32_t* sorted_idx,
                                    const uint32_t* gathered_pos, int key_bytes, int nranks,
                                    int samples_per_rank, int rank, void* splitters_out,
                                    uint32_t* thresholds_out);
grs_status grs_shard_plan_host(const uint32_t* count_matrix, int nranks, int rank,
                               uint64_t* send_off, uint64_t* recv_off, uint64_t* n_out);
grs_status grs_shard_bounds_host(const void* sorted_keys, size_t n, int key_bytes,
                                 const void* splitters, const uint32_t* thresholds, int nranks,
                                 uint64_t* bounds_out);
grs_status grs_shard_chunk_plan_host(const uint32_t* count_matrices, int nchunks, int nranks, int rank,
                                     uint64_t chunk_len, uint64_t* send_off, uint64_t* recv_off,
                                     uint64_t* n_out);
int grs_shard_samples_per_rank(int nranks);

grs_status grs_shard_sample(const void* d_keys, size_t n, int key_bytes, int samples,
                            void* d_sample_keys, uint32_t* d_sample_pos, void* stream);
size_t grs_shard_encode_words_max(size_t n, int nranks);
grs_status grs_shard_encode(grs_sorter* s, const uint32_t* d_sorted, size_t n,
                            const uint32_t* d_gathered_keys, const uint32_t* d_gathered_pos,
                            int nranks, int rank, uint32_t* d_send, size_t send_capacity_words,
                            uint32_t* d_sizes, void* stream);
grs_status grs_shard_decode_merge(grs_sorter* s, const uint32_t* d_recv, int nranks,
                                  const uint64_t* recv_word_offsets, const uint32_t* recv_keys,
                                  uint32_t* d_keys_out, size_t out_capacity, void* stream);


grs_status grs_iota_u32(uint32_t* d_out, size_t n, uint32_t start, void* stream);

grs_status grs_gather_records(const void* d_src, void* d_dst, const uint32_t* d_idx, size_t n,
                              size_t record_bytes, void* stream);

grs_status grs_copy_u32(const uint32_t* d_src, uint32_t* d_dst, size_t n, void* stream);

grs_status grs_fill_splitmix(void* d_keys, size_t n, int key_bytes, uint64_t seed,
                             uint64_t first_index, void* stream);

grs_status grs_fill_permutation(void* d_keys, size_t n, int key_bytes, uint64_t total, uint64_t seed,
                                uint64_t first_index, void* stream);

grs_status grs_count_inversions(const void* d_keys, size_t n, int key_bytes,
                                uint64_t* out_count, void* stream);

grs_status grs_sort_host(grs_sorter* s, const void* h_keys_in, void* h_keys_out,
                         const uint32_t* h_vals_in, uint32_t* h_vals_out, size_t n, void* stream);


#define GRS_KEYS_UNSIGNED 0
#define GRS_KEYS_SIGNED 1
#define GRS_KEYS_FLOAT 2
grs_status grs_key_transform(void* d_keys, size_t n, int key_bytes, int kind, int inverse,
                             void* stream);

#define GRS_EXTRACT_FIELD 0
#define GRS_EXTRACT_MORTON3 1
typedef struct grs_key_extract {
  int kind;
  uint32_t offset;
  int transform;
  float lo[3];
  float hi[3];
} grs_key_extract;
grs_status grs_sort_records(grs_sorter* s, void* d_records, size_t n, size_t record_bytes,
                            const grs_key_extract* key, void* stream);

grs_status grs_records_key_buffers(grs_sorter* s, size_t n, size_t record_bytes, void** d_keys,
                                   uint32_t** d_idx);
grs_status grs_sort_records_by_keys(grs_sorter* s, void* d_records, size_t n, size_t record_bytes,
                                    void* d_keys, uint32_t* d_idx, void* stream);

#define GRS_SCAN_MAX_N 0xFFFFF000u
size_t grs_scan_scratch_bytes(size_t n);
grs_status grs_exclusive_scan_u32(const uint32_t* d_in, uint32_t* d_out, size_t n,
                                  uint32_t* d_total, void* d_scratch, size_t scratch_bytes,
                                  void* stream);
grs_status grs_scan_check_error(const void* d_scratch, void* stream);

grs_status grs_sort_segmented(grs_sorter* s, void* d_keys, uint32_t* d_vals, size_t n,
                              const uint32_t* d_offsets, int num_segments, void* stream);

#ifdef __cplusplus
}
#endif

#endif
```

Before: 170.1 Gkeys/s.

## Store only low 16-bit key halves between MSD pass 2 and local sort

In the MSD path for u32 keys without payload, the second region pass now writes only the low 16 bits of each key into the scratch buffer. The high 16 bits are rebuilt in pass 3 from the segment index and the OR of the key span, through a new helper, and passed along the mid/big work lists. This halves the write traffic of pass 2 and the read traffic of pass 3, at the cost of wider work-list entries, an extra hi array, and more branches in the local-sort and copy kernels. It is on by default and can be turned off with a new option.

```diff
diff --git a/gpuradixsort_amd/_lib.py b/gpuradixsort_amd/_lib.py
--- a/gpuradixsort_amd/_lib.py
+++ b/gpuradixsort_amd/_lib.py
@@ -57,6 +57,7 @@
     "h2_piece": (14, {"default": 0}),
     "p3": (15, {"per_segment": 0, "persistent": 1, "whole_keys": 2}),
     "x_chunks": (16, {"default": 0}),
+    "p2_half": (18, {"auto": 0, "never": 1}),
     "p3_shape": (17, {"size": 0, "S": 4, "M": 5, "A": 1, "W": 1, "B": 2, "C2": 7, "C": 3, "D": 6}),
 }
 
@@ -69,6 +70,7 @@
     ("grs_scratch_bytes", c_size_t, [c_void_p]),
     ("grs_debug_check_guards", c_int, [c_void_p, POINTER(c_uint64)]),
     ("grs_debug_msd_flags", c_int, [c_void_p, POINTER(c_uint32)]),
+    ("grs_debug_p2_half_hi", c_uint32, [c_uint32, c_int, c_uint32]),
     ("grs_debug_p3_kernel", c_char_p, [c_int, c_int, c_size_t, c_int, c_int]),
     ("grs_rank_mode", c_int, [c_void_p]),
     ("grs_lds_order_check", c_int, [c_int, c_int, c_int, POINTER(c_ulonglong)]),
diff --git a/gpuradixsort_amd/csrc/grs_capi.hip b/gpuradixsort_amd/csrc/grs_capi.hip
--- a/gpuradixsort_amd/csrc/grs_capi.hip
+++ b/gpuradixsort_amd/csrc/grs_capi.hip
@@ -252,6 +252,7 @@
   uint32_t h2_piece = 0;
   int p3_shape = 0;
   int p3_mode = 0;
+  int p2_half = 0;
   int seg_route = 0;
   int msd_mode = -1;
   void* msd_buf = nullptr;
@@ -267,6 +268,7 @@
   std::vector<ScratchBuf> bufs;
   int last_msd_cb = -1;
   uint32_t* last_msd_spill2 = nullptr;
+  bool last_msd_half = false;
   size_t alt_inner_band = 0;
   bool alt_band_dirty = false;
 };
@@ -435,7 +437,7 @@
 
 struct MsdLayout {
   size_t h2, h2x, h2s, big, spill2, mid, clear, dstart, reg, room, len2, in2, out2, tab, hdr2, rec2, hdr2r, rec2r,
-      hdrf, recf, bin, bstart, blen, brow, rows, spill, words;
+      hdrf, recf, bin, bstart, blen, brow, bhi, rows, spill, words;
   size_t r2, rf, bl, mr;
   std::vector<size_t> bands;
   static MsdLayout of(size_t cap, size_t nd) {
@@ -455,7 +457,7 @@
       o += (w + 63) & ~static_cast<size_t>(63);
       return at;
     };
-    L.h2 = take(3 * 65536 + 64 + 2 + 3 * 65536);
+    L.h2 = take(3 * 65536 + 64 + 2 + 4 * 65536);
     L.h2x = L.h2 + 65536;
     L.h2s = L.h2 + 2 * 65536;
     L.big = L.h2 + 3 * 65536;
@@ -479,6 +481,7 @@
     L.bstart = take(L.bl);
     L.blen = take(L.bl);
     L.brow = take(L.bl);
+    L.bhi = take(L.bl);
     L.rows = take(L.mr * nd * 256);
     L.spill = take(6 * (L.bl + 1));
     L.words = o;
@@ -669,6 +672,10 @@
       if (value < 0 || value > 2) return bad();
       s->p3_mode = value;
       break;
+    case GRS_OPT_P2_HALF:
+      if (value < 0 || value > 1) return bad();
+      s->p2_half = value;
+      break;
     case GRS_OPT_P3_SHAPE: {
       const auto none = [](auto) {};
       const bool ok = value == 0 || (s->key_type == GRS_KEY_U32
@@ -723,6 +730,7 @@
     case GRS_OPT_H2_PIECE: *value = static_cast<int>(s->h2_piece); break;
     case GRS_OPT_P3: *value = s->p3_mode; break;
     case GRS_OPT_P3_SHAPE: *value = s->p3_shape; break;
+    case GRS_OPT_P2_HALF: *value = s->p2_half; break;
     default: return set_err(GRS_EINVAL, "grs_get_option: unknown option");
   }
   return GRS_OK;
@@ -823,6 +831,7 @@
   grs_status r = GRS_OK;
   const uint32_t* hist = s->last_msd_cb == 0 ? s->ctrl : s->ctrl2;
   uint32_t w[3] = {};
+  const bool half = s->last_msd_half;
   if (hipDeviceSynchronize() != hipSuccess ||
       hipMemcpy(&w[0], hist + 512 + 256, 4, hipMemcpyDeviceToHost) != hipSuccess ||
       hipMemcpy(&w[1], s->last_msd_spill2, 4, hipMemcpyDeviceToHost) != hipSuccess ||
@@ -831,6 +840,7 @@
   flags[0] = w[0] != 0u;
   flags[1] = w[1] != 0u;
   flags[2] = w[2];
+  flags[3] = half && w[1] == 0u;
   (void)hipSetDevice(prev);
   return r;
 }
@@ -1246,6 +1256,7 @@
   if ((r = mark()) != GRS_OK) return r;
   s->last_msd_cb = s->cb_i;
   s->last_msd_spill2 = mb + L.spill2;
+  s->last_msd_half = false;
   if (s->cb_dirty && s->cb_i == 0) GRS_HIP(hipMemsetAsync(hist, 0, GRS_CTRL_ERROR * 4, stream));
   s->cb_dirty = false;
   if (s->alt_band_dirty) {
@@ -1330,18 +1341,31 @@
     }
   }
   if ((r = mark()) != GRS_OK) return r;
+  const MsdP3Kernel pk = msd_p3_kernel<K, PAIRS, P3C>(n, s->p3_mode);
+  const bool half = sizeof(K) == 4 && !PAIRS && shift != 0 && pk.family == MsdP3Kernel::kLocal16 && s->p2_half == 0;
+  s->last_msd_half = half;
   {
     const Dig d2{-8, 255u};
     const dim3 grid(static_cast<uint32_t>(t2));
-    constexpr uint32_t RG = 131072;
+    constexpr uint32_t RG = 131072, HALF = 524288;
     auto go = [&](auto tshape) -> grs_status {
       using T = decltype(tshape);
       if (shift) {
         GRS_DIAG_CHECK("plans");
         GRS_DIAG_SET(cap2, region_len);
-        hipLaunchKernelGGL((grs::grs_onesweep_seg<K, PAIRS, 8, T::BLOCK, T::ITEMS, T::MINW, T::OPT | RG, false>),
-                           grid, dim3(T::BLOCK), 0, stream, alt, rk, valt, rv, d2, rec2r, hdr2r, reg, 256u,
-                           tickets + GRS_XCDS, st[1], st[0], err, dstart, h2, spill2, (const uint32_t*)nullptr, top);
+        bool launched_half = false;
+        if constexpr (sizeof(K) == 4 && !PAIRS) {
+          if (half) {
+            hipLaunchKernelGGL((grs::grs_onesweep_seg<K, PAIRS, 8, T::BLOCK, T::ITEMS, T::MINW, T::OPT | RG | HALF, false>),
+                               grid, dim3(T::BLOCK), 0, stream, alt, rk, valt, rv, d2, rec2r, hdr2r, reg, 256u,
+                               tickets + GRS_XCDS, st[1], st[0], err, dstart, h2, spill2, (const uint32_t*)nullptr, top);
+            launched_half = true;
+          }
+        }
+        if (!launched_half)
+          hipLaunchKernelGGL((grs::grs_onesweep_seg<K, PAIRS, 8, T::BLOCK, T::ITEMS, T::MINW, T::OPT | RG, false>),
+                             grid, dim3(T::BLOCK), 0, stream, alt, rk, valt, rv, d2, rec2r, hdr2r, reg, 256u,
+                             tickets + GRS_XCDS, st[1], st[0], err, dstart, h2, spill2, (const uint32_t*)nullptr, top);
         GRS_HIP(hipGetLastError());
         GRS_DIAG_CHECK("P2region");
         GRS_DIAG_SET(n, region_len);
@@ -1371,8 +1395,9 @@
   }
   if ((r = mark()) != GRS_OK) return r;
   using P3L = std::conditional_t<sizeof(K) == 4 && !PAIRS, MsdLocalC, MsdLocalB>;
-  const MsdP3Kernel pk = msd_p3_kernel<K, PAIRS, P3C>(n, s->p3_mode);
   const uint32_t mid_max = pk.mid_max;
+  const uint32_t* const span_or = half ? span : nullptr;
+  uint32_t* const bhi = half ? mb + L.bhi : nullptr;
   bool launched = false;
   if constexpr (sizeof(K) == 4) {
     if (pk.family == MsdP3Kernel::kLocalPf) {
@@ -1388,12 +1413,14 @@
     } else if (pk.family == MsdP3Kernel::kLocal16 && pk.block == 512) {
       hipLaunchKernelGGL((grs::grs_msd_local16<512, 34, 6, FT::TILE>), dim3(65536), dim3(512), 0, stream,
                          (uint32_t*)keys, vals, (const uint32_t*)rk, rv, spill2, mb + L.len2, mb + L.in2, mb + L.out2,
-                         mid_max, mb + L.mid, bigc, mb + L.bin, mb + L.bstart, mb + L.blen, mb + L.brow, rows, top);
+                         mid_max, mb + L.mid, bigc, mb + L.bin, mb + L.bstart, mb + L.blen, mb + L.brow, rows, top,
+                         span_or, bhi);
       launched = true;
     } else if (pk.family == MsdP3Kernel::kLocal16) {
       hipLaunchKernelGGL((grs::grs_msd_local16<1024, 34, 8, FT::TILE>), dim3(65536), dim3(1024), 0, stream,
                          (uint32_t*)keys, vals, (const uint32_t*)rk, rv, spill2, mb + L.len2, mb + L.in2, mb + L.out2,
-                         mid_max, mb + L.mid, bigc, mb + L.bin, mb + L.bstart, mb + L.blen, mb + L.brow, rows, top);
+                         mid_max, mb + L.mid, bigc, mb + L.bin, mb + L.bstart, mb + L.blen, mb + L.brow, rows, top,
+                         span_or, bhi);
       launched = true;
     }
   }
@@ -1410,11 +1437,11 @@
     hipLaunchKernelGGL((grs::grs_msd_local_list<K, PAIRS, P3L::BLOCK, P3L::I, P3L::C16, minw>),
                        dim3(per_cu * s->cus), dim3(P3L::BLOCK), 0, stream, keys, vals, rk, rv, spill2, mb + L.mid,
                        top, (const uint32_t*)bigc, (const uint32_t*)(mb + L.bin), (const uint32_t*)(mb + L.bstart),
-                       (const uint32_t*)(mb + L.blen));
+                       (const uint32_t*)(mb + L.blen), (const uint32_t*)bhi);
     GRS_HIP(hipGetLastError());
   } else {
     hipLaunchKernelGGL((grs::grs_msd_copy_big<K, PAIRS>), dim3(4 * s->cus), dim3(256), 0, stream, rk, rv, keys, vals,
-                       spill2, bigc, mb + L.bin, mb + L.bstart, mb + L.blen);
+                       spill2, bigc, mb + L.bin, mb + L.bstart, mb + L.blen, (const uint32_t*)bhi);
     GRS_HIP(hipGetLastError());
   }
   GRS_DIAG_CHECK("P3");
@@ -3369,6 +3396,11 @@
   return name;
 }
 
+uint32_t grs_debug_p2_half_hi(uint32_t or_keys, int top_shift, uint32_t segment) {
+  if (top_shift < 8 || top_shift > 24 || segment > 0xFFFFu) return 0xFFFFFFFFu;
+  return grs::msd_half_hi(or_keys, static_cast<uint32_t>(top_shift), segment);
+}
+
 const char* grs_pass_kernel(const grs_sorter* s, size_t n) {
   if (!s || n == 0) return "";
   if (use_msd(s, n, 0, s->key_type == GRS_KEY_U64 ? 64 : 32)) return "grs_onesweep_region";
diff --git a/gpuradixsort_amd/csrc/grs_msd.hpp b/gpuradixsort_amd/csrc/grs_msd.hpp
--- a/gpuradixsort_amd/csrc/grs_msd.hpp
+++ b/gpuradixsort_amd/csrc/grs_msd.hpp
@@ -198,6 +198,10 @@
   if constexpr (sizeof(K) == 8) return (static_cast<K>(hi) << 32) | lo;
   else return static_cast<K>(lo);
 }
+__host__ __device__ inline uint32_t msd_half_hi(uint32_t or_keys, uint32_t s, uint32_t b) {
+  const uint32_t low_mask = s + 8 >= 32 ? 0xFFFFFFFFu : (1u << (s + 8)) - 1u;
+  return ((or_keys & ~low_mask) | (b << (s - 8))) & 0xFFFF0000u;
+}
 template <int RMAX>
 __device__ __forceinline__ int msd_p3_rounds(uint32_t s) {
   const int r = (static_cast<int>(s) - 8 + 7) / 8;
@@ -575,11 +579,20 @@
                                                         const uint32_t* __restrict__ big,
                                                         const uint32_t* __restrict__ big_in,
                                                         const uint32_t* __restrict__ big_out,
-                                                        const uint32_t* __restrict__ big_len) {
+                                                        const uint32_t* __restrict__ big_len,
+                                                        const uint32_t* __restrict__ big_hi = nullptr) {
   if (*spill != 0u) return;
   const uint32_t count = big[0];
   for (uint32_t e = 0; e < count; ++e) {
     const uint32_t a = big_in[e], o = big_out[e], n = big_len[e];
+    if constexpr (sizeof(K) == 4 && !PAIRS) {
+      if (big_hi != nullptr) {
+        const uint32_t hi = big_hi[e];
+        const uint16_t* const rh = reinterpret_cast<const uint16_t*>(rk);
+        for (uint32_t i = blockIdx.x * 256 + threadIdx.x; i < n; i += gridDim.x * 256) keys[o + i] = hi | rh[a + i];
+        continue;
+      }
+    }
     for (uint32_t i = blockIdx.x * 256 + threadIdx.x; i < n; i += gridDim.x * 256) {
       keys[o + i] = rk[a + i];
       if constexpr (PAIRS) vals[o + i] = rv[a + i];
@@ -651,6 +664,15 @@
       if constexpr (PAIRS) v[j] = i < len ? vin[lo + i] : 0u;
     }
   }
+  __device__ __forceinline__ static void load_half(K (&k)[I], const uint16_t* hin, uint32_t len, uint32_t hi) {
+    static_assert(sizeof(K) == 4 && !PAIRS, "low halves: u32 keys without payload");
+    const uint32_t lane = threadIdx.x & (GRS_WAVE - 1), w = threadIdx.x >> 6;
+#pragma unroll
+    for (uint32_t j = 0; j < I; ++j) {
+      const uint32_t i = w * GRS_WAVE * I + j * GRS_WAVE + lane;
+      k[j] = i < len ? hi | hin[i] : K(0);
+    }
+  }
   __device__ __forceinline__ static void sort_rounds(Smem& sm, K (&k)[I], Vals& v, uint32_t len, int rounds,
                                                      uint32_t ak = 0, uint32_t av = 0, int shift0 = 0,
                                                      uint32_t t = threadIdx.x) {
@@ -835,19 +857,20 @@
   __device__ __forceinline__ static uint32_t half(const uint32_t (&p)[IP], uint32_t j) {
     return (p[j >> 1] >> (16 * (j & 1))) & 0xFFFFu;
   }
-  __device__ __forceinline__ static void run(Smem& sm, const uint32_t* kin, uint32_t* kout, uint32_t len,
-                                             int rounds) {
+  __device__ __forceinline__ static void run(Smem& sm, const void* kin, uint32_t esz, uint32_t hi, uint32_t* kout,
+                                             uint32_t len, int rounds) {
     const uint32_t t = threadIdx.x, lane = t & (GRS_WAVE - 1), w = t >> 6;
-    const uint32_t hi = __builtin_amdgcn_readfirstlane(kin[0]) & 0xFFFF0000u;
-    const auto rsrc = __builtin_amdgcn_make_buffer_rsrc(const_cast<uint32_t*>(kin), 0, static_cast<int>(4u * len),
+    if (esz == 4u) hi = __builtin_amdgcn_readfirstlane(*static_cast<const uint32_t*>(kin)) & 0xFFFF0000u;
+    const auto rsrc = __builtin_amdgcn_make_buffer_rsrc(const_cast<void*>(kin), 0, static_cast<int>(esz * len),
                                                         0x00020000);
     const uint32_t ws = __builtin_amdgcn_readfirstlane(w), wbase = ws * GRS_WAVE * I;
     const uint32_t wlen = len > wbase ? len - wbase : 0u;
+    const uint32_t voff = esz * lane;
     uint32_t kp[IP];
 #pragma unroll
     for (uint32_t j = 0; j < IP; ++j) {
-      const uint32_t a = __builtin_amdgcn_raw_buffer_load_b16(rsrc, 4u * lane, 4u * (wbase + 2u * j * GRS_WAVE), 0);
-      const uint32_t b = __builtin_amdgcn_raw_buffer_load_b16(rsrc, 4u * lane, 4u * (wbase + (2u * j + 1u) * GRS_WAVE), 0);
+      const uint32_t a = __builtin_amdgcn_raw_buffer_load_b16(rsrc, voff, esz * (wbase + 2u * j * GRS_WAVE), 0);
+      const uint32_t b = __builtin_amdgcn_raw_buffer_load_b16(rsrc, voff, esz * (wbase + (2u * j + 1u) * GRS_WAVE), 0);
       kp[j] = (a & 0xFFFFu) | (b << 16);
     }
     const uint32_t ak = static_cast<uint32_t>(reinterpret_cast<uintptr_t>(kout) / 4u) % 4u;
@@ -931,12 +954,17 @@
                                                 const uint32_t* vin, K* keys, uint32_t* vals, uint32_t mid_max,
                                                 uint32_t* mid, uint32_t* big, uint32_t* big_in,
                                                 uint32_t* big_start, uint32_t* big_len, uint32_t* big_row,
-                                                uint32_t* rows, uint32_t& slot) {
+                                                uint32_t* rows, uint32_t& slot, bool half = false, uint32_t hi = 0,
+                                                uint32_t* big_hi = nullptr) {
   const uint32_t t = threadIdx.x;
   if (len == 1u) {
     if (!inplace && t == 0) {
-      keys[o] = kin[lo];
-      if constexpr (PAIRS) vals[o] = vin[lo];
+      if constexpr (sizeof(K) == 4 && !PAIRS) {
+        keys[o] = half ? hi | reinterpret_cast<const uint16_t*>(kin)[lo] : kin[lo];
+      } else {
+        keys[o] = kin[lo];
+        if constexpr (PAIRS) vals[o] = vin[lo];
+      }
     }
     return;
   }
@@ -944,15 +972,17 @@
   if (len <= mid_max) {
     if (t == 0) {
       const uint32_t e = atomicAdd(&mid[0], 1u);
-      mid[2 + 3 * e] = lo;
-      mid[3 + 3 * e] = o;
-      mid[4 + 3 * e] = len;
+      mid[2 + 4 * e] = lo;
+      mid[3 + 4 * e] = o;
+      mid[4 + 4 * e] = len;
+      mid[5 + 4 * e] = hi;
     }
     return;
   }
   if (t == 0) {
     const uint32_t e = atomicAdd(&big[0], 1u);
     const uint32_t row = len > TILEF ? atomicAdd(&big[1], 1u) : 0xFFFFFFFFu;
+    if (big_hi != nullptr) big_hi[e] = hi;
     big_in[e] = lo;
     big_start[e] = o;
     big_len[e] = len;
@@ -1006,7 +1036,8 @@
     const uint32_t* __restrict__ in2, const uint32_t* __restrict__ out2, uint32_t mid_max, uint32_t* __restrict__ mid,
     uint32_t* __restrict__ big, uint32_t* __restrict__ big_in, uint32_t* __restrict__ big_start,
     uint32_t* __restrict__ big_len, uint32_t* __restrict__ big_row, uint32_t* __restrict__ rows,
-    const uint32_t* __restrict__ top_shift) {
+    const uint32_t* __restrict__ top_shift, const uint32_t* __restrict__ span_or = nullptr,
+    uint32_t* __restrict__ big_hi = nullptr) {
   using LS = LocalSort16<BLOCK, I>;
   __shared__ typename LS::Smem sm;
   const uint32_t len = len2[blockIdx.x];
@@ -1014,13 +1045,18 @@
   const bool inplace = __builtin_amdgcn_readfirstlane(*spill) != 0u;
   const uint32_t lo = in2[blockIdx.x], o = out2[blockIdx.x];
   const uint32_t* const kin = inplace ? keys : rk;
+  const uint32_t top = __builtin_amdgcn_readfirstlane(*top_shift);
+  const bool half = span_or != nullptr && !inplace;
+  const uint32_t hi = half ? msd_half_hi(__builtin_amdgcn_readfirstlane(*span_or), top, blockIdx.x) : 0u;
   if (len == 1u || len > LS::SMAX) {
     msd_local_other<uint32_t, false, BLOCK, LS::SMAX, 2, TILEF>(len, lo, o, inplace, kin, nullptr, keys, vals, mid_max,
                                                                 mid, big, big_in, big_start, big_len, big_row, rows,
-                                                                sm.slot);
+                                                                sm.slot, half, hi, big_hi);
     return;
   }
-  LS::run(sm, kin + lo, keys + o, len, msd_p3_rounds<2>(__builtin_amdgcn_readfirstlane(*top_shift)));
+  const void* const src = half ? static_cast<const void*>(reinterpret_cast<const uint16_t*>(kin) + lo)
+                               : static_cast<const void*>(kin + lo);
+  LS::run(sm, src, half ? 2u : 4u, hi, keys + o, len, msd_p3_rounds<2>(top));
 }
 
 template <typename K, bool PAIRS, int BLOCK, int I, bool C16, uint32_t TILEF, int MINW>
@@ -1094,14 +1130,25 @@
                                                             const uint32_t* __restrict__ big = nullptr,
                                                             const uint32_t* __restrict__ big_in = nullptr,
                                                             const uint32_t* __restrict__ big_out = nullptr,
-                                                            const uint32_t* __restrict__ big_len = nullptr) {
+                                                            const uint32_t* __restrict__ big_len = nullptr,
+                                                            const uint32_t* __restrict__ big_hi = nullptr) {
   using LS = LocalSort<K, PAIRS, BLOCK, I, C16>;
   __shared__ typename LS::Smem sm;
   const bool inplace = *spill != 0u;
+  bool half = false;
+  if constexpr (sizeof(K) == 4 && !PAIRS) half = big_hi != nullptr && !inplace;
+  const uint16_t* const rh = reinterpret_cast<const uint16_t*>(rk);
   if (big != nullptr && !inplace) {
     const uint32_t nb = big[0];
     for (uint32_t e = 0; e < nb; ++e) {
       const uint32_t a = big_in[e], o = big_out[e], n = big_len[e];
+      if constexpr (sizeof(K) == 4 && !PAIRS) {
+        if (half) {
+          const uint32_t hi = big_hi[e];
+          for (uint32_t i = blockIdx.x * BLOCK + threadIdx.x; i < n; i += gridDim.x * BLOCK) keys[o + i] = hi | rh[a + i];
+          continue;
+        }
+      }
       for (uint32_t i = blockIdx.x * BLOCK + threadIdx.x; i < n; i += gridDim.x * BLOCK) {
         keys[o + i] = rk[a + i];
         if constexpr (PAIRS) vals[o + i] = rv[a + i];
@@ -1114,7 +1161,18 @@
   const uint32_t* const vin = inplace ? vals : rv;
   const int rounds = msd_p3_rounds<LS::ROUNDS>(__builtin_amdgcn_readfirstlane(*top_shift));
   for (uint32_t e = blockIdx.x; e < count; e += gridDim.x) {
-    const uint32_t lo = mid[2 + 3 * e], o = mid[3 + 3 * e], len = mid[4 + 3 * e];
+    const uint32_t lo = mid[2 + 4 * e], o = mid[3 + 4 * e], len = mid[4 + 4 * e];
+    if constexpr (sizeof(K) == 4 && !PAIRS) {
+      if (half) {
+        K k[I];
+        typename LS::Vals v;
+        LS::load_half(k, rh + lo, len, mid[5 + 4 * e]);
+        LS::sort_rounds(sm, k, v, len, rounds, LS::template mis<K, LS::KV>(keys + o), 0u);
+        LS::template copy_out<K, LS::KV>(keys + o, sm.sk, len);
+        __syncthreads();
+        continue;
+      }
+    }
     LS::template run_vec<>(sm, kin + lo, PAIRS ? vin + lo : nullptr, keys + o, PAIRS ? vals + o : nullptr,
                            len, rounds);
     __syncthreads();
diff --git a/gpuradixsort_amd/csrc/grs_pass.hpp b/gpuradixsort_amd/csrc/grs_pass.hpp
--- a/gpuradixsort_amd/csrc/grs_pass.hpp
+++ b/gpuradixsort_amd/csrc/grs_pass.hpp
@@ -501,6 +501,9 @@
       } else {
         reinterpret_cast<unsigned long long*>(keys_out)[dst] = x;
       }
+    } else if constexpr ((OPT & 524288) != 0) {
+      static_assert(sizeof(K) == 4 && !PAIRS && (OPT & 131072) != 0, "low halves: u32 keys, a region pass");
+      reinterpret_cast<uint16_t*>(keys_out)[dst] = static_cast<uint16_t>(kk);
     } else {
       keys_out[dst] = kk;
       if constexpr (PAIRS) vals_out[dst] = sm.vals[i];
diff --git a/gpuradixsort_amd/sorter.py b/gpuradixsort_amd/sorter.py
--- a/gpuradixsort_amd/sorter.py
+++ b/gpuradixsort_amd/sorter.py
@@ -73,10 +73,13 @@
         check(lib().grs_debug_check_guards(self._h, ctypes.byref(bad)), "grs_debug_check_guards")
         return int(bad.value)
 
-    def msd_flags(self) -> dict:
-        f = (ctypes.c_uint32 * 3)()
+    def msd_flags(self, p2_half: bool = False) -> dict:
+        f = (ctypes.c_uint32 * 4)()
         check(lib().grs_debug_msd_flags(self._h, f), "grs_debug_msd_flags")
-        return {"p1_redo": bool(f[0]), "p2_exact": bool(f[1]), "top_shift": int(f[2])}
+        flags = {"p1_redo": bool(f[0]), "p2_exact": bool(f[1]), "top_shift": int(f[2])}
+        if p2_half:
+            flags["p2_half"] = bool(f[3])
+        return flags
 
     def p3_kernel(self, n: int) -> Optional[str]:
         kt = GRS_KEY_U32 if self.key_bits == 32 else GRS_KEY_U64
diff --git a/include/grs.h b/include/grs.h
--- a/include/grs.h
+++ b/include/grs.h
@@ -48,7 +48,9 @@
 
 grs_status grs_debug_check_guards(grs_sorter* s, uint64_t* bad_words);
 
-grs_status grs_debug_msd_flags(grs_sorter* s, uint32_t flags[3]);
+grs_status grs_debug_msd_flags(grs_sorter* s, uint32_t flags[4]);
+
+uint32_t grs_debug_p2_half_hi(uint32_t or_keys, int top_shift, uint32_t segment);
 
 const char* grs_debug_p3_kernel(grs_key_type key_type, int pairs, size_t n, int p3_mode, int p3_shape);
 
@@ -73,6 +75,7 @@
   GRS_OPT_H2_PIECE = 14,
   GRS_OPT_P3 = 15,
   GRS_OPT_X_CHUNKS = 16,
+  GRS_OPT_P2_HALF = 18,
   GRS_OPT_P3_SHAPE = 17
 } grs_option;
 grs_status grs_set_option(grs_sorter* s, grs_option opt, int value);
```

After: 177.5 Gkeys/s, median of 6. 1.04x the previous value.
